# johannes-graeter/limo

Measured on AMD Instinct MI355X. Metric: keyframe-BA window solves/sec (5 KF, ~2k landmarks), higher is better.
Workload: dtype f64; 1 GPU; C2: KITTI-00-shaped windows, 5 keyframes x 2000 landmarks, LiDAR depth + ground plane, solveTrimmed schedule {2, trim 5%, <=100 LM iterations}; batch_windows_per_gpu=16384, distinct_windows_per_gpu=4096, observations_per_batch=144288124, depth_observations_per_batch=68405568, parallelism=single, converged=16328

## Files before the change

include/limo_hip.h:

```cpp
#ifndef LIMO_HIP_H_
#define LIMO_HIP_H_

#include <stddef.h>
#include <stdint.h>

#ifdef __cplusplus
extern "C" {
#endif

#define LIMO_ABI_VERSION 6

enum limo_fixation { LIMO_FIX_POSE = 0, LIMO_FIX_SCALE = 1, LIMO_FIX_NONE = 2 };

enum limo_status {
    LIMO_OK = 0,
    LIMO_ERR_INVALID = -1,
    LIMO_ERR_NOT_ENOUGH_KF = -2,
    LIMO_ERR_RUNTIME = -3,
    LIMO_ERR_NO_DEVICE = -4,
    LIMO_ERR_UNSUPPORTED = -5
};

enum limo_termination { LIMO_CONVERGENCE = 0, LIMO_NO_CONVERGENCE = 1, LIMO_FAILURE = 2 };

// ... 20 lines not shown
    const float* obs_u;
    const float* obs_v;
    const float* obs_d;
} limo_ba_window;

typedef struct limo_ba_options {
    double depth_thres;
    double reprojection_thres;
    double depth_quantile;
    double reprojection_quantile;
    int32_t num_trim_rounds;
    int32_t trim_solver_iterations;
    int32_t min_landmarks_for_trimming;
    int32_t minimum_number_residual_groups;
    int32_t max_num_iterations;
    double max_solver_time_sec;
    double function_tolerance;
    double gradient_tolerance;
    double parameter_tolerance;
    double initial_trust_region_radius;
    double max_trust_region_radius;
    double min_trust_region_radius;
    double min_lm_diagonal;
    double max_lm_diagonal;
    double min_relative_decrease;
    int32_t max_num_consecutive_invalid_steps;
    int32_t jacobi_scaling;
} limo_ba_options;

typedef struct limo_ba_report {
    int32_t termination;
    int32_t num_solves;
    int32_t iterations_total;
    int32_t iterations_final;
    int32_t successful_steps;
    int32_t n_depth_blocks;
    int32_t n_repr_blocks;
    int32_t n_gp_blocks;
    int32_t n_trimmed_landmarks;
    int32_t num_linearizations;
    double initial_cost;
    double final_cost;
    double time_sec;
} limo_ba_report;

typedef struct limo_ctx limo_ctx;
typedef struct limo_ba_batch limo_ba_batch;

int limo_abi_version(void);
int limo_ctx_create(int device, limo_ctx** out);
void limo_ctx_destroy(limo_ctx* ctx);
int limo_ctx_set_stream(limo_ctx* ctx, void* hip_stream);
const char* limo_last_error(const limo_ctx* ctx);
void* limo_host_alloc(size_t bytes);
void limo_host_free(void* p);

void limo_ba_default_options(limo_ba_options* out);

int limo_ba_solve(limo_ctx* ctx, limo_ba_window* window, const limo_ba_options* opts, limo_ba_report* report);

int limo_ba_batch_create(limo_ctx* ctx, int32_t n_windows, const limo_ba_window* windows, limo_ba_batch** out);
int limo_ba_batch_solve(limo_ba_batch* batch, const limo_ba_options* opts);
int limo_ba_batch_reset(limo_ba_batch* batch);
int limo_ba_batch_download(limo_ba_batch* batch, limo_ba_window* windows_out, limo_ba_report* reports);
void limo_ba_batch_destroy(limo_ba_batch* batch);
int limo_ba_batch_trimmed(limo_ba_batch* batch, int32_t window, uint8_t* removed);
int limo_ba_batch_kernel_stats(limo_ba_batch* batch, int reset, double* linearize_ms, int64_t* linearize_launches,
                               double* total_ms);
#define LIMO_KERNEL_LINEARIZE 0
#define LIMO_KERNEL_SCHUR 1
int limo_ba_batch_kernel_time(limo_ba_batch* batch, int kernel, double* ms, int64_t* launches);

#define LIMO_COMM_ID_BYTES 128
int limo_comm_unique_id(unsigned char id[LIMO_COMM_ID_BYTES]);
int limo_ctx_comm_init(limo_ctx* ctx, const unsigned char id[LIMO_COMM_ID_BYTES], int rank, int world);
typedef void (*limo_exchange_fn)(const double* send, double* recv, long long count, int kind, void* user);
int limo_ctx_comm_init_host(limo_ctx* ctx, limo_exchange_fn fn, void* user, int rank, int world);
int limo_ba_solve_sharded(limo_ctx* ctx, limo_ba_window* window, const limo_ba_options* opts, int n_shards,
                          limo_ba_report* report);
int limo_ctx_exchange_stats(limo_ctx* ctx, int64_t* stats3);
int64_t limo_ctx_coop_fallbacks(const limo_ctx* ctx);
int limo_ctx_last_solve_info(const limo_ctx* ctx, int64_t info[8]);
int limo_ctx_last_schur_gp_info(const limo_ctx* ctx, int64_t info[4]);

typedef struct limo_ba_iteration {
    int32_t solve;
    int32_t solve_kind;
    int32_t iteration;
    uint8_t step_is_valid, step_is_successful, pad[2];
    double cost;
    double cost_change, gradient_max_norm, step_norm, relative_decrease, trust_region_radius;
} limo_ba_iteration;
int limo_ctx_set_iteration_log(limo_ctx* ctx, int32_t on);
int limo_ba_batch_iteration_log(limo_ba_batch* batch, int32_t window, int32_t cap, limo_ba_iteration* out, int32_t* n);
int limo_ctx_last_iteration_log(limo_ctx* ctx, int32_t window, int32_t cap, limo_ba_iteration* out, int32_t* n);

int limo_ba_evaluate(limo_ctx* ctx, const limo_ba_window* window, const limo_ba_options* opts, int apply_loss,
                     double* cost, double* residuals, double* jac_pose, double* jac_lm, uint8_t* valid);

int limo_ba_evaluate_batch_time(limo_ctx* ctx, int32_t n_windows, const limo_ba_window* windows, const limo_ba_options* opts,
                                int32_t reps, double* device_ms);

typedef struct limo_speed_prior {
    double speed_weight;
    double dt_cur;
    double vel_prev[3];
    double pose_before[7];
} limo_speed_prior;
int limo_ba_adjust_pose_only(limo_ctx* ctx, limo_ba_window* window, const limo_speed_prior* prior,
                             const limo_ba_options* opts, limo_ba_report* report);

int limo_ba_batch_create_pose_only(limo_ctx* ctx, int32_t n_windows, const limo_ba_window* windows,
                                   const limo_speed_prior* priors, limo_ba_batch** out);
int limo_ba_adjust_pose_only_batch(limo_ctx* ctx, int32_t n_windows, limo_ba_window* windows, const limo_speed_prior* priors,
                                   const limo_ba_options* opts, limo_ba_report* reports);

int limo_ba_solve_fixed_landmarks(limo_ctx* ctx, limo_ba_window* window, const uint8_t* lm_fixed, const limo_ba_options* opts,
                                  limo_ba_report* report);
int limo_ba_batch_create_fixed_landmarks(limo_ctx* ctx, int32_t n_windows, const limo_ba_window* windows, const uint8_t* const* lm_fixed,
                                         limo_ba_batch** out);

enum limo_row_kind {
    LIMO_ROW_GROUND_HEIGHT = 0,
    LIMO_ROW_SCALE = 1,
    LIMO_ROW_NORMAL_DIFF = 2,
    LIMO_ROW_DIST_DIFF = 3,
    LIMO_ROW_PLANE_MOTION = 4,
    LIMO_ROW_GLOBAL_NORMAL = 5,
    LIMO_ROW_SPEED = 6
};
typedef struct limo_ba_row {
    int32_t kind;
    int32_t sub;
    int32_t kf[2];
    int32_t lm;
    int32_t fixed;
    double r;
    double cost;
    double jac_kf[2][10];
    double jac_lm[3];
} limo_ba_row;
int limo_ba_evaluate_rows(limo_ctx* ctx, const limo_ba_window* window, const limo_speed_prior* prior, int pose_only,
                          const limo_ba_options* opts, int32_t cap, limo_ba_row* rows, int32_t* n_rows);

typedef struct limo_ray {
    double pose_cam_origin[7];
    double f, cx, cy;
    float u, v, d;
    float pad;
} limo_ray;
int limo_landmark_init(limo_ctx* ctx, int32_t n, const int32_t* ray_off , const limo_ray* rays,
                       const uint8_t* use_depth , double* pos_out , uint8_t* ok );

int limo_trim_quantile(int32_t n, const int64_t* ids, const double* values, double quantile, int64_t* outliers_out);

typedef struct limo_depth_params {
    int32_t pixelarea_search_width;
    int32_t pixelarea_search_height;
    int32_t pixelarea_search_offset_x;
    int32_t pixelarea_search_offset_y;
    int32_t neighbors_count_min;
    int32_t do_use_histogram_segmentation;
    double histogram_segmentation_bin_width;
    int32_t histogram_segmentation_min_pointcount;
    int32_t treshold_depth_enabled;
    double treshold_depth_max;
// ... 149 lines not shown
```

limo_amd/_ffi.py:

```python
import ctypes as C
import os

_HERE = os.path.dirname(os.path.abspath(__file__))
LIB_PATH = os.environ.get("LIMO_HIP_LIB") or os.path.join(_HERE, "lib", "liblimo_hip.so")

LIMO_FIX_POSE, LIMO_FIX_SCALE, LIMO_FIX_NONE = 0, 1, 2
LIMO_OK, LIMO_ERR_INVALID, LIMO_ERR_NOT_ENOUGH_KF, LIMO_ERR_RUNTIME, LIMO_ERR_NO_DEVICE, LIMO_ERR_UNSUPPORTED = 0, -1, -2, -3, -4, -5
LIMO_CONVERGENCE, LIMO_NO_CONVERGENCE, LIMO_FAILURE = 0, 1, 2

c_double_p = C.POINTER(C.c_double)
c_float_p = C.POINTER(C.c_float)
c_int32_p = C.POINTER(C.c_int32)
c_int64_p = C.POINTER(C.c_int64)
c_uint8_p = C.POINTER(C.c_uint8)


class BaWindow(C.Structure):
    _fields_ = [
        ("n_kf", C.c_int32),
        ("n_cam", C.c_int32),
        ("n_lm", C.c_int32),
        ("n_obs", C.c_int32),
        ("kf_pose", c_double_p),
        ("kf_plane_dir", c_double_p),
# ... 259 lines not shown
        ("do_use_triangle_size_maximation", C.c_int32),
        ("do_check_triangleplanar_condition", C.c_int32),
        ("triangleplanar_crossnorm_treshold", C.c_double),
        ("viewray_plane_orthoganality_treshold", C.c_double),
        ("do_use_ransac_plane", C.c_int32),
        ("ransac_plane_distance_treshold", C.c_double),
        ("ransac_plane_min_z", C.c_double),
        ("ransac_plane_max_z", C.c_double),
        ("ransac_plane_max_iterations", C.c_int32),
        ("ransac_plane_probability", C.c_double),
        ("ransac_plane_use_refinement", C.c_int32),
        ("ransac_plane_refinement_treshold", C.c_double),
        ("ransac_plane_point_distance_treshold", C.c_double),
        ("plane_estimator_use_mestimator", C.c_int32),
        ("ransac_seed", C.c_uint64),
        ("neighbor_search_mode", C.c_int32),
        ("do_use_nearestNeighborSearch", C.c_int32),
        ("nnSearch_count", C.c_int32),
        ("do_use_radiusSearch", C.c_int32),
        ("radiusSearch_radius", C.c_double),
        ("radiusSearch_count_min", C.c_int32),
        ("do_use_depth_segmentation", C.c_int32),
        ("depth_segmentation_max_treshold_gradient", C.c_double),
        ("depth_segmentation_max_neighbor_distance", C.c_double),
        ("depth_segmentation_max_neighbor_distance_gradient", C.c_double),
        ("depth_segmentation_max_seedpoint_to_seedpoint_distance", C.c_double),
        ("depth_segmentation_max_seedpoint_to_seedpoint_distance_gradient", C.c_double),
        ("depth_segmentation_max_neighbor_to_seedpoint_distance", C.c_double),
        ("depth_segmentation_max_neighbor_to_seedpoint_distance_gradient", C.c_double),
        ("depth_segmentation_max_pointcount", C.c_int32),
        ("treshold_depth_mode", C.c_int32),
        ("treshold_depth_local_mode", C.c_int32),
        ("do_use_PCA", C.c_int32),
        ("pca_debug", C.c_double),
        ("pca_treshold_3_abs_min", C.c_double),
        ("pca_treshold_3_2_rel_max", C.c_double),
        ("pca_treshold_2_1_rel_min", C.c_double),
        ("ransac_plane_use_camx_treshold", C.c_int32),
        ("ransac_plane_treshold_camx", C.c_double),
        ("plane_estimator_use_triangle_maximation", C.c_int32),
        ("plane_estimator_use_leastsquares", C.c_int32),
        ("plane_estimator_z_x_min_relation", C.c_double),
        ("do_debug_singleFeatures", C.c_int32),
        ("do_publish_points", C.c_int32),
        ("do_depth_calc_statistics", C.c_int32),
    ]


(DEPTH_OK, DEPTH_NEIGHBOURS, DEPTH_HISTOGRAM, DEPTH_SEGMENT3, DEPTH_PLANAR, DEPTH_PARALLEL, DEPTH_GLOBAL, DEPTH_LOCAL, DEPTH_PCA,
 DEPTH_DEGENERATE) = range(10)
DEPTH_REASON_NAMES = ["OK", "NEIGHBOURS", "HISTOGRAM", "SEGMENT3", "PLANAR", "PARALLEL", "GLOBAL", "LOCAL", "PCA", "DEGENERATE"]


EXCHANGE_FN = C.CFUNCTYPE(None, C.POINTER(C.c_double), C.POINTER(C.c_double), C.c_longlong, C.c_int, C.c_void_p)

ABI_VERSION = 6

ABI_SYMBOLS = [
    "limo_abi_version",
    "limo_ctx_create",
    "limo_ctx_destroy",
    "limo_ctx_set_stream",
    "limo_last_error",
    "limo_host_alloc",
    "limo_host_free",
    "limo_ba_default_options",
    "limo_ba_solve",
    "limo_ba_batch_create",
    "limo_ba_batch_solve",
    "limo_ba_batch_reset",
    "limo_ba_batch_download",
    "limo_ba_batch_destroy",
    "limo_ba_batch_trimmed",
    "limo_ba_batch_kernel_stats",
    "limo_ba_batch_kernel_time",
    "limo_comm_unique_id",
    "limo_ctx_comm_init",
    "limo_ctx_comm_init_host",
    "limo_ba_solve_sharded",
    "limo_ctx_exchange_stats",
    "limo_ctx_coop_fallbacks",
    "limo_ctx_last_solve_info",
    "limo_ctx_last_schur_gp_info",
    "limo_ctx_set_iteration_log",
    "limo_ba_batch_iteration_log",
    "limo_ctx_last_iteration_log",
    "limo_ba_evaluate",
    "limo_ba_evaluate_batch_time",
    "limo_ba_evaluate_rows",
    "limo_ba_adjust_pose_only",
    "limo_ba_batch_create_pose_only",
    "limo_ba_adjust_pose_only_batch",
    "limo_ba_solve_fixed_landmarks",
    "limo_ba_batch_create_fixed_landmarks",
    "limo_landmark_init",
    "limo_trim_quantile",
    "limo_depth_default_params",
    "limo_depth_estimate",
    "limo_depth_estimate_begin",
    "limo_depth_estimate_end",
    "limo_depth_estimate_batch",
    "limo_depth_last_ground_plane",
    "limo_depth_last_reasons",
    "limo_depth_set_timing",
    "limo_depth_last_kernel_ms",
    "limo_five_point_default_params",
    "limo_five_point",
    "limo_five_point_batch",
    "limo_select_default_params",
    "limo_landmark_select",
    "limo_landmark_select_batch",
    "limo_select_set_timing",
    "limo_select_last_kernel_ms",
]

_lib = None


def load():
    global _lib
    if _lib is not None:
        return _lib
    if not os.path.exists(LIB_PATH):
        raise RuntimeError(
            "limo_amd: %s not found - run `python -c 'import __graft_entry__ as g; g.build()'` first. "
            "There is no CPU fallback for the product path." % LIB_PATH
        )
    try:
        import torch
    except ImportError:
        pass
    lib = C.CDLL(LIB_PATH, mode=C.RTLD_GLOBAL)
    vp = C.c_void_p
    lib.limo_abi_version.restype = C.c_int
    older = os.environ.get("LIMO_ALLOW_OLDER_ABI") == "1" and lib.limo_abi_version() < ABI_VERSION
    if lib.limo_abi_version() != ABI_VERSION and not older:
        raise RuntimeError("limo_amd: %s has ABI version %d, this binding needs %d - rebuild it (__graft_entry__.build())" % (LIB_PATH, lib.limo_abi_version(), ABI_VERSION))
    lib.limo_ctx_create.argtypes = [C.c_int, C.POINTER(vp)]
    lib.limo_ctx_destroy.argtypes = [vp]
    lib.limo_ctx_destroy.restype = None
    lib.limo_ctx_set_stream.argtypes = [vp, vp]
    lib.limo_last_error.argtypes = [vp]
    lib.limo_last_error.restype = C.c_char_p
    lib.limo_ba_default_options.argtypes = [C.POINTER(BaOptions)]
    lib.limo_ba_default_options.restype = None
    lib.limo_ba_solve.argtypes = [vp, C.POINTER(BaWindow), C.POINTER(BaOptions), C.POINTER(BaReport)]
    lib.limo_ba_batch_create.argtypes = [vp, C.c_int32, C.POINTER(BaWindow), C.POINTER(vp)]
    lib.limo_ba_batch_solve.argtypes = [vp, C.POINTER(BaOptions)]
    lib.limo_ba_batch_reset.argtypes = [vp]
    lib.limo_ba_batch_download.argtypes = [vp, C.POINTER(BaWindow), C.POINTER(BaReport)]
    lib.limo_ba_batch_destroy.argtypes = [vp]
    lib.limo_ba_batch_destroy.restype = None
    lib.limo_ba_batch_trimmed.argtypes = [vp, C.c_int32, c_uint8_p]
    lib.limo_ba_batch_kernel_stats.argtypes = [vp, C.c_int, c_double_p, c_int64_p, c_double_p]
    lib.limo_ba_batch_kernel_time.argtypes = [vp, C.c_int, c_double_p, c_int64_p]
    lib.limo_comm_unique_id.argtypes = [C.c_char_p]
    lib.limo_ctx_comm_init.argtypes = [vp, C.c_char_p, C.c_int, C.c_int]
    if not older:
        lib.limo_ctx_comm_init_host.argtypes = [vp, EXCHANGE_FN, C.c_void_p, C.c_int, C.c_int]
    lib.limo_ba_solve_sharded.argtypes = [vp, C.POINTER(BaWindow), C.POINTER(BaOptions), C.c_int, C.POINTER(BaReport)]
    lib.limo_ba_evaluate_batch_time.argtypes = [vp, C.c_int32, C.POINTER(BaWindow), C.POINTER(BaOptions), C.c_int32, C.POINTER(C.c_double)]
    lib.limo_ba_evaluate.argtypes = [
        vp,
        C.POINTER(BaWindow),
        C.POINTER(BaOptions),
        C.c_int,
        c_double_p,
        c_double_p,
        c_double_p,
        c_double_p,
        c_uint8_p,
    ]
    lib.limo_ba_evaluate_rows.argtypes = [vp, C.POINTER(BaWindow), C.POINTER(SpeedPrior), C.c_int, C.POINTER(BaOptions), C.c_int32, C.POINTER(BaRow), c_int32_p]
    lib.limo_ba_adjust_pose_only.argtypes = [
        vp,
        C.POINTER(BaWindow),
        C.POINTER(SpeedPrior),
        C.POINTER(BaOptions),
        C.POINTER(BaReport),
    ]
    if hasattr(lib, "limo_ba_batch_create_pose_only"):
        lib.limo_ba_batch_create_pose_only.argtypes = [vp, C.c_int32, C.POINTER(BaWindow), C.POINTER(SpeedPrior), C.POINTER(vp)]
        lib.limo_ba_adjust_pose_only_batch.argtypes = [vp, C.c_int32, C.POINTER(BaWindow), C.POINTER(SpeedPrior), C.POINTER(BaOptions), C.POINTER(BaReport)]
    if hasattr(lib, "limo_ba_solve_fixed_landmarks"):
        lib.limo_ba_solve_fixed_landmarks.argtypes = [vp, C.POINTER(BaWindow), c_uint8_p, C.POINTER(BaOptions), C.POINTER(BaReport)]
        lib.limo_ba_batch_create_fixed_landmarks.argtypes = [vp, C.c_int32, C.POINTER(BaWindow), C.POINTER(c_uint8_p), C.POINTER(vp)]
    lib.limo_landmark_init.argtypes = [vp, C.c_int32, c_int32_p, C.POINTER(Ray), c_uint8_p, c_double_p, c_uint8_p]
    lib.limo_trim_quantile.argtypes = [C.c_int32, c_int64_p, c_double_p, C.c_double, c_int64_p]
    lib.limo_depth_default_params.argtypes = [C.POINTER(DepthParams)]
    lib.limo_depth_default_params.restype = None
    lib.limo_depth_estimate.argtypes = [
        vp,
        c_float_p,
        C.c_size_t,
        c_double_p,
        C.c_double,
        C.c_double,
        C.c_double,
        C.c_int32,
        C.c_int32,
        c_float_p,
        C.c_size_t,
        c_uint8_p,
        C.POINTER(DepthParams),
        c_float_p,
    ]
    lib.limo_depth_estimate_begin.argtypes = lib.limo_depth_estimate.argtypes[:-1]
    lib.limo_depth_estimate_end.argtypes = [vp, c_float_p, C.c_size_t]
    lib.limo_host_alloc.argtypes = [C.c_size_t]
    lib.limo_host_alloc.restype = C.c_void_p
    lib.limo_host_free.argtypes = [C.c_void_p]
    lib.limo_host_free.restype = None
    lib.limo_depth_estimate_batch.argtypes = [vp, C.c_int32, C.POINTER(DepthFrame), c_double_p, C.c_double, C.c_double, C.c_double, C.c_int32, C.c_int32,
                                              C.POINTER(DepthParams), C.c_uint32]
    lib.limo_ctx_exchange_stats.argtypes = [vp, c_int64_p]
    lib.limo_ctx_coop_fallbacks.argtypes = [vp]
    lib.limo_ctx_coop_fallbacks.restype = C.c_int64
    if hasattr(lib, "limo_ctx_last_solve_info"):
        lib.limo_ctx_last_solve_info.argtypes = [vp, c_int64_p]
    if hasattr(lib, "limo_ctx_last_schur_gp_info"):
        lib.limo_ctx_last_schur_gp_info.argtypes = [vp, c_int64_p]
    if hasattr(lib, "limo_ctx_set_iteration_log"):
        lib.limo_ctx_set_iteration_log.argtypes = [vp, C.c_int32]
        lib.limo_ba_batch_iteration_log.argtypes = [vp, C.c_int32, C.c_int32, C.POINTER(BaIteration), c_int32_p]
        lib.limo_ctx_last_iteration_log.argtypes = [vp, C.c_int32, C.c_int32, C.POINTER(BaIteration), c_int32_p]
    lib.limo_depth_set_timing.argtypes = [vp, C.c_int32]
    lib.limo_depth_last_kernel_ms.argtypes = [vp, c_double_p]
    lib.limo_depth_last_ground_plane.argtypes = [vp, C.c_int32, c_double_p, c_int32_p]
    if not older:
        lib.limo_depth_last_reasons.argtypes = [vp, C.c_int32, c_uint8_p, C.c_size_t]
    if hasattr(lib, "limo_five_point"):
        lib.limo_five_point_default_params.argtypes = [C.POINTER(FivePointParams)]
        lib.limo_five_point_default_params.restype = None
        lib.limo_five_point.argtypes = [vp, C.POINTER(FivePointFrame), C.c_double, C.c_double, C.c_double, C.POINTER(FivePointParams),
                                        C.POINTER(FivePointMotion), c_uint8_p]
        lib.limo_five_point_batch.argtypes = [vp, C.c_int32, C.POINTER(FivePointFrame), C.c_double, C.c_double, C.c_double, C.POINTER(FivePointParams),
                                              C.POINTER(FivePointMotion)]
    if hasattr(lib, "limo_landmark_select"):
        lib.limo_select_default_params.argtypes = [C.POINTER(SelectParams)]
        lib.limo_select_default_params.restype = None
        lib.limo_landmark_select.argtypes = [vp, C.POINTER(SelectPool), C.POINTER(SelectParams), c_uint8_p]
        lib.limo_landmark_select_batch.argtypes = [vp, C.c_int32, C.POINTER(SelectPool), C.POINTER(SelectParams), C.POINTER(c_uint8_p)]
        lib.limo_select_set_timing.argtypes = [vp, C.c_int32]
        lib.limo_select_last_kernel_ms.argtypes = [vp, c_double_p]
    _lib = lib
    return lib
```

limo_amd/ba.py:

```python
import ctypes as C

import numpy as np

from . import _ffi
from .window import struct_array


class LimoError(RuntimeError):
    pass


class NotEnoughKeyframes(LimoError):
    """BundleAdjusterKeyframes::NotEnoughKeyframesException (bundle_adjuster_keyframes.hpp:59-68)."""


def _check(rc, ctx=None, what=""):
    if rc == _ffi.LIMO_OK:
        return
    msg = ""
    if ctx is not None:
        msg = _ffi.load().limo_last_error(ctx).decode(errors="replace")
    if rc == _ffi.LIMO_ERR_NOT_ENOUGH_KF:
        raise NotEnoughKeyframes(msg or what)
    raise LimoError("%s failed: rc=%d %s" % (what, rc, msg))


class Context:
    def __init__(self, device=0, stream=None):
        self.lib = _ffi.load()
        self.device = device
        self.ptr = C.c_void_p()
        rc = self.lib.limo_ctx_create(device, C.byref(self.ptr))
        if rc != 0:
            raise LimoError("limo_ctx_create(device=%d) failed rc=%d (no gfx950 device? the product path has no CPU fallback)" % (device, rc))
        if stream is not None:
            self.set_stream(stream)

    def set_stream(self, stream):
        _check(self.lib.limo_ctx_set_stream(self.ptr, C.c_void_p(stream)), self.ptr, "limo_ctx_set_stream")

    def close(self):
        if self.ptr:
            self.lib.limo_ctx_destroy(self.ptr)
            self.ptr = C.c_void_p()

    def __del__(self):
        try:
            self.close()
        except Exception:
            pass

    def solve(self, window, opts, lm_fixed=None):
        s = window.as_struct()
        rep = _ffi.BaReport()
        if lm_fixed is not None:
            flags = fixed_flags(lm_fixed, window.n_lm)
            rc = self.lib.limo_ba_solve_fixed_landmarks(self.ptr, C.byref(s), flags.ctypes.data_as(_ffi.c_uint8_p), C.byref(opts), C.byref(rep))
            _check(rc, self.ptr, "limo_ba_solve_fixed_landmarks")
            return rep.as_dict()
        _check(self.lib.limo_ba_solve(self.ptr, C.byref(s), C.byref(opts), C.byref(rep)), self.ptr, "limo_ba_solve")
        return rep.as_dict()

    def solve_sharded(self, window, opts, n_shards):
        s = window.as_struct()
        rep = _ffi.BaReport()
        _check(self.lib.limo_ba_solve_sharded(self.ptr, C.byref(s), C.byref(opts), int(n_shards), C.byref(rep)), self.ptr, "limo_ba_solve_sharded")
        return rep.as_dict()

    def exchange_stats(self):
        st = (C.c_int64 * 3)()
        _check(self.lib.limo_ctx_exchange_stats(self.ptr, st), self.ptr, "limo_ctx_exchange_stats")
        return {"exchanges": int(st[0]), "bytes": int(st[1]), "iterations": int(st[2])}

    def coop_fallbacks(self):
        return int(self.lib.limo_ctx_coop_fallbacks(self.ptr))

    SOLVE_PATHS = {1: "WG", 2: "COOP", 3: "STREAMING", 4: "LOCKSTEP"}

    def last_solve_info(self):
        v = (C.c_int64 * 8)()
        _check(self.lib.limo_ctx_last_solve_info(self.ptr, v), self.ptr, "limo_ctx_last_solve_info")
        keys = ("recovered", "coop_G", "groups", "slots", "rounds", "pair_launches", "lin_variant")
        return dict({"path": self.SOLVE_PATHS.get(int(v[0]), "NONE")}, **{k: int(v[1 + i]) for i, k in enumerate(keys)})

    def last_schur_gp_info(self):
        v = (C.c_int64 * 4)()
        _check(self.lib.limo_ctx_last_schur_gp_info(self.ptr, v), self.ptr, "limo_ctx_last_schur_gp_info")
        return dict(zip(("narrow_groups", "wide_groups", "narrow_launches", "wide_launches"), (int(x) for x in v)))

    def set_iteration_log(self, on):
        _check(self.lib.limo_ctx_set_iteration_log(self.ptr, int(bool(on))), self.ptr, "limo_ctx_set_iteration_log")

    def last_iteration_log(self, window=0):
        return _read_iteration_log(lambda cap, out, n: self.lib.limo_ctx_last_iteration_log(self.ptr, int(window), cap, out, n), self.ptr,
                                   "limo_ctx_last_iteration_log")

    def comm_init(self, unique_id, rank, world):
        _check(self.lib.limo_ctx_comm_init(self.ptr, unique_id, int(rank), int(world)), self.ptr, "limo_ctx_comm_init")

    def comm_init_host(self, rank, world, allgather, allreduce):
        import numpy as np

        def _cb(send, recv, count, kind, _user):
            s = np.ctypeslib.as_array(send, shape=(count,))
            if kind == 0:
                allgather(s, np.ctypeslib.as_array(recv, shape=(world, count)))
            else:
                allreduce(s, np.ctypeslib.as_array(recv, shape=(count,)))

        self._xfn = _ffi.EXCHANGE_FN(_cb)
        _check(self.lib.limo_ctx_comm_init_host(self.ptr, self._xfn, None, int(rank), int(world)), self.ptr, "limo_ctx_comm_init_host")

    def comm_unique_id(self):
        buf = C.create_string_buffer(128)
        _check(self.lib.limo_comm_unique_id(buf), self.ptr, "limo_comm_unique_id")
        return buf.raw

    def landmark_init(self, ray_off, rays, use_depth):
        ray_off = np.ascontiguousarray(ray_off, np.int32)
        use_depth = np.ascontiguousarray(use_depth, np.uint8)
        n = len(use_depth)
        pos = np.zeros((n, 3))
        ok = np.zeros(n, np.uint8)
        rc = self.lib.limo_landmark_init(self.ptr, n, ray_off.ctypes.data_as(_ffi.c_int32_p), rays, use_depth.ctypes.data_as(_ffi.c_uint8_p),
                                         pos.ctypes.data_as(_ffi.c_double_p), ok.ctypes.data_as(_ffi.c_uint8_p))
        _check(rc, self.ptr, "limo_landmark_init")
        return pos, ok

    def five_point_params(self, probability=None, threshold_px=None, max_samples=None, chunk=None):
        p = _ffi.FivePointParams()
        self.lib.limo_five_point_default_params(C.byref(p))
        for name, v in (("probability", probability), ("threshold_px", threshold_px), ("max_samples", max_samples), ("chunk", chunk)):
            if v is not None:
                setattr(p, name, v)
        return p

    def five_point(self, pts_a, pts_b, focal, cx, cy, seed=1, params=None, with_mask=False):
        a = np.ascontiguousarray(pts_a, np.float64).reshape(-1, 2)
        b = np.ascontiguousarray(pts_b, np.float64).reshape(-1, 2)
        if len(a) != len(b):
            raise ValueError("five_point: %d points in a, %d in b" % (len(a), len(b)))
        fr = _ffi.FivePointFrame(len(a), a.ctypes.data_as(_ffi.c_double_p), b.ctypes.data_as(_ffi.c_double_p), int(seed))
        p = params if params is not None else self.five_point_params()
        m = _ffi.FivePointMotion()
        mask = np.zeros(max(1, len(a)), np.uint8) if with_mask else None
        rc = self.lib.limo_five_point(self.ptr, C.byref(fr), float(focal), float(cx), float(cy), C.byref(p), C.byref(m),
                                      mask.ctypes.data_as(_ffi.c_uint8_p) if with_mask else None)
        _check(rc, self.ptr, "limo_five_point")
        out = m.as_dict()
        out["raw"] = bytes(m)
        if with_mask:
            out["inlier"] = mask[: len(a)]
        return out

    def five_point_batch(self, frames, focal, cx, cy, params=None):
        keep = [(np.ascontiguousarray(a, np.float64).reshape(-1, 2), np.ascontiguousarray(b, np.float64).reshape(-1, 2), int(s)) for a, b, s in frames]
        n = len(keep)
        arr = (_ffi.FivePointFrame * max(1, n))()
        for i, (a, b, s) in enumerate(keep):
            if len(a) != len(b):
                raise ValueError("five_point_batch: frame %d: %d points in a, %d in b" % (i, len(a), len(b)))
            arr[i] = _ffi.FivePointFrame(len(a), a.ctypes.data_as(_ffi.c_double_p), b.ctypes.data_as(_ffi.c_double_p), s)
        p = params if params is not None else self.five_point_params()
        ms = (_ffi.FivePointMotion * max(1, n))()
        _check(self.lib.limo_five_point_batch(self.ptr, n, arr, float(focal), float(cx), float(cy), C.byref(p), ms), self.ptr, "limo_five_point_batch")
        out = []
        for i in range(n):
            d = ms[i].as_dict()
            d["raw"] = bytes(ms[i])
            out.append(d)
        return out
# ... 318 lines not shown
```

limo_amd/csrc/kba_batch_plan.hpp:

```cpp
#pragma once
#include <algorithm>
#include <cstdint>
#include <cstdlib>
#include <vector>

#include "kba_items.hpp"
#include "kba_pack.hpp"

namespace kba {

struct PlanKernelSizes {
    int (*lean_lds)(int ncol);
    int (*wide_lds)(int nfp, int nc, int n_view);
    int lin_lds;
    int wide_waves;
    int trim_max_sort;
};

struct BatchPlan {
    bool any_fast = false, any_gen = false;
    int plain_tm = 1, plain_wpe = 4, gp_tm = 1, gp_wpe = 3;
    bool pair_ok = false;
    int wide_npw = 0;
    int plain_lds = 0, leangp_lds = 0, wide_lds = 0;
// ... 11 lines not shown
        p.max_nc = std::max(p.max_nc, (int)d.nc);
        if (d.schur_fast) {
            p.any_fast = true;
            max_nfq = std::max(max_nfq, (int)d.nfq);
            max_nf = std::max(max_nf, (int)d.nf);
        } else if (d.n_sblk > 0) {
            p.any_gen = true;
            t_gen = std::max(t_gen, d.nf_pad / 16);
            nfp_gen = std::max(nfp_gen, (int)d.nf_pad);
            nc_gen = std::max(nc_gen, (int)d.nc);
            nv_gen = std::max(nv_gen, (int)d.n_view);
        }
    }
    if (p.any_fast) {
        p.plain_tm = (max_nfq + 16) / 16 <= 1 ? 1 : 2;
        p.plain_wpe = p.plain_tm == 1 ? 4 : 3;
        p.plain_lds = ks.lean_lds(max_nfq + 1);
        p.gp_tm = std::min(3, (max_nf + 16) / 16);
        p.gp_wpe = p.gp_tm == 1 ? 3 : 2;
        p.leangp_lds = ks.lean_lds(max_nf + 1);
        p.pair_ok = p.plain_tm == 2 && p.gp_tm == 3;
        p.narrow = p.gp_tm == 3 && P.n_sgrp_narrow > 0;
    }
    if (p.any_gen) {
        const int tiles = t_gen * (t_gen + 1) / 2, npw = (tiles + ks.wide_waves - 1) / ks.wide_waves;
        p.wide_npw = npw <= 1 ? 1 : npw <= 3 ? 3 : npw <= 6 ? 6 : npw <= 12 ? 12 : -1;
        p.wide_lds = ks.wide_lds(nfp_gen, nc_gen, nv_gen);
    }
    {
        int nc_lds = kCamSlots, nf_lds = 1, nv_lds = 1;
        for (const WinDesc& d : P.win)
            if (d.cam_scr_off < 0) {
                nc_lds = std::max(nc_lds, (int)d.nc);
                nf_lds = std::max(nf_lds, (int)d.nf);
                nv_lds = std::max(nv_lds, (int)d.n_view);
            }
        p.asm_bytes = cam_assemble_scratch(nc_lds, kBlock, nv_lds) * (int)sizeof(double);
        p.solve_bytes = cam_solve_scratch(nc_lds, kBlock, nf_lds) * (int)sizeof(double);
    }
    int max_lm = 1, np2 = 1;
    for (const WinDesc& d : P.win) max_lm = std::max(max_lm, (int)d.n_lm);
    while (np2 < max_lm) np2 <<= 1;
    p.trim_bytes = np2 <= ks.trim_max_sort ? np2 * 12 + max_lm + 16 : 16;
    p.schur_wave_lds = (std::max(p.plain_lds, p.leangp_lds) + 15) / 16 * 16;
    p.onelaunch_lds = std::max(std::max(p.asm_bytes, p.solve_bytes), std::max(p.trim_bytes, ks.lin_lds));
    return p;
}

inline void build_sblk_list(const PackedBatch& P, const std::vector<int32_t>* windows, int span, int span_gp, int owner, std::vector<int32_t>& v,
                            int& n_plain, int& n_fgp) {
    v.clear();
    n_plain = n_fgp = 0;
    const int nw = windows ? (int)windows->size() : P.n_win;
    for (int cls = 0; cls < 3; ++cls) {
        for (int q = 0; q < nw; ++q) {
            const int w = windows ? (*windows)[q] : q;
            const WinDesc& d = P.win[w];
            if ((cls < 2) != (d.schur_fast != 0)) continue;
            auto groups = [&](int i0, int i1, int sp) {
                for (int i = i0; i < i1; i += sp)
                    if (owner < 0 || P.sblk_owner[d.sblk0 + i] == owner) v.push_back(d.sblk0 + i);
            };
            if (cls != 1) groups(0, d.n_sblk_plain, span);
            if (cls != 0) groups(d.n_sblk_plain, d.n_sblk, span_gp);
        }
        if (cls == 0) n_plain = (int)v.size();
        if (cls == 1) n_fgp = (int)v.size() - n_plain;
    }
}

constexpr int kCoopMaxWg = 256, kCoopMaxWin = 64;
constexpr int kWgMaxLblk = 8;
constexpr int kCoopRetryAfter = 64;

struct SolveSwitches {
    bool stream_min_set = false;
    int stream_min = 16;
    int coop_max_win = kCoopMaxWin;
    bool no_wg = false;
    bool no_coop = false;
    double coop_timeout_ms = 50.0;
    bool groups_set = false;
    int groups = 0;
    bool gp_wide = false;
};

inline SolveSwitches read_solve_switches() {
    SolveSwitches s;
    auto on = [](const char* name) {
        const char* e = std::getenv(name);
        return e && std::atoi(e) != 0;
    };
    if (const char* e = std::getenv("KBA_STREAM_MIN")) {
        s.stream_min_set = true;
        s.stream_min = std::atoi(e);
    }
    if (const char* e = std::getenv("KBA_COOP_MAX_WIN")) s.coop_max_win = std::min(std::atoi(e), kCoopMaxWg);
    s.no_wg = on("KBA_NO_WG_SOLVE");
    s.no_coop = on("KBA_NO_COOP_SOLVE");
    if (const char* e = std::getenv("KBA_COOP_TIMEOUT_MS")) s.coop_timeout_ms = std::atof(e);
    if (const char* e = std::getenv("KBA_GROUPS")) {
        s.groups_set = true;
        s.groups = std::atoi(e);
    }
    s.gp_wide = on("KBA_SCHUR_GP_WIDE");
    return s;
}

enum SolvePath { PATH_NONE = 0, PATH_WG = 1, PATH_COOP = 2, PATH_STREAMING = 3, PATH_LOCKSTEP = 4 };

struct SolveFacts {
    double max_solver_time_sec = -1.0;
    int shard_P = 1;
    bool pose_batch = false;
    bool pristine = true;
    int coop_strikes = 0, coop_benched = 0;
};
struct CoopGeometry {
    int G = 0, grid = 0;
};
struct SolveChoice {
    SolvePath path = PATH_LOCKSTEP;
    SolvePath fallback = PATH_LOCKSTEP;
    bool benched = false;
    CoopGeometry coop;
};

inline int plain_groups(const WinDesc& d, int span) { return (d.n_sblk_plain + span - 1) / span; }
inline int gp_groups(const WinDesc& d, int span_gp) { return (d.n_sblk - d.n_sblk_plain + span_gp - 1) / span_gp; }

inline bool wg_solve_applies(const PackedBatch& P, const BatchPlan& plan, const SolveSwitches& sw, int shard_P) {
    if (shard_P != 1 || P.evaluate_only || P.n_sblk != 0 || P.n_win < 1 || sw.no_wg) return false;
    for (const WinDesc& d : P.win)
        if (d.n_lblk > kWgMaxLblk) return false;
    return plan.onelaunch_lds <= kCamLdsCapBytes;
}

inline int coop_lds_bytes(const BatchPlan& plan) { return std::max(plan.onelaunch_lds, (kBlock / 64) * plan.schur_wave_lds); }

inline bool coop_solve_applies(const PackedBatch& P, const BatchPlan& plan, const SolveSwitches& sw, int shard_P, CoopGeometry& geo) {
    if (shard_P != 1 || P.evaluate_only || P.n_win < 1 || sw.no_coop) return false;
    int G = 1;
    for (const WinDesc& d : P.win) {
        if (!d.schur_fast || d.cam_scr_off >= 0 || d.nf_pad * d.nf_pad > kCoopRedStride) return false;
        const int tasks = plain_groups(d, kSchurSpan) + gp_groups(d, kSchurSpanGp);
        G = std::max(G, std::max((int)d.n_lblk, tasks ? 1 + (tasks + kBlock / 64 - 1) / (kBlock / 64) : 1));
    }
    G = std::min(G, 32);
    if (P.n_win > kCoopMaxWg || coop_lds_bytes(plan) > kCamLdsCapBytes) return false;
    const int per8 = ((int)P.n_win + 7) / 8;
    geo.G = std::max(1, std::min(G, kCoopMaxWg / (8 * per8)));
    geo.grid = 8 * geo.G * per8;
    return true;
}

inline SolveChoice choose_solve_path(const PackedBatch& P, const BatchPlan& plan, const SolveSwitches& sw, const SolveFacts& f) {
    SolveChoice ch;
    const bool pose_multi = f.pose_batch && P.n_win > 1;
    const bool can_stream = f.shard_P == 1 && f.max_solver_time_sec <= 0.0 && P.n_win >= sw.stream_min && !P.evaluate_only && !pose_multi;
    const bool one_launch = pose_multi || (!(sw.stream_min_set && can_stream) && P.n_win <= sw.coop_max_win);
    ch.path = ch.fallback = can_stream ? PATH_STREAMING : PATH_LOCKSTEP;
    if (!one_launch) return ch;
    if (wg_solve_applies(P, plan, sw, f.shard_P)) {
        ch.path = PATH_WG;
    } else if (!pose_multi && f.pristine && coop_solve_applies(P, plan, sw, f.shard_P, ch.coop)) {
        ch.benched = f.coop_strikes >= 3;
        if (!ch.benched || f.coop_benched + 1 >= kCoopRetryAfter) ch.path = PATH_COOP;
    }
    return ch;
}

struct SchurSpans {
    int plain = kSchurSpan, gp = kSchurSpanGp;
};
struct StreamGeometry {
    int n_slots = 0, n_groups = 0;
    int group_slots[4] = {0, 0, 0, 0};
    int mx[SL_COUNT] = {0};
};
inline StreamGeometry stream_geometry(const PackedBatch& P, const SchurSpans& spans, const SolveSwitches& sw) {
    StreamGeometry g;
    g.n_slots = std::min((int)P.n_win, std::max(1024, std::min(kSchedMaxSlots, (int)P.n_win / 4)));
    g.n_groups = sw.groups_set ? std::max(1, std::min(4, sw.groups)) : g.n_slots >= 4096 ? 3 : P.n_win >= 512 ? 2 : 1;
    for (int gi = 0; gi < g.n_groups; ++gi) g.group_slots[gi] = g.n_slots / g.n_groups + (gi < g.n_slots % g.n_groups ? 1 : 0);
    for (const WinDesc& d : P.win) {
        const int plg = plain_groups(d, spans.plain), gpg = gp_groups(d, spans.gp);
        g.mx[SL_LBLK] = std::max(g.mx[SL_LBLK], (int)d.n_lblk);
        g.mx[SL_TBLK] = std::max(g.mx[SL_TBLK], (int)d.n_blk);
        g.mx[SL_SPLAIN] = std::max(g.mx[SL_SPLAIN], d.schur_fast ? plg : 0);
// ... 11 lines not shown
```

limo_amd/csrc/kba_items.hpp:

```cpp
#pragma once
#include "kba_layout.hpp"
#include "kba_lm.hpp"
#include "kba_math.hpp"

#ifndef KBA_SYNC
#define KBA_SYNC() ((void)0)
#endif
#if defined(KBA_PROFILE_TICKS) && defined(__HIPCC__)
__device__ long long kba_ticks[2][24];
#endif
#if defined(KBA_PROFILE_TICKS) && defined(__HIP_DEVICE_COMPILE__)
#define KBA_TICK(n)                                                                   \
    do {                                                                              \
        if (w == 0 && (tid == 0 || tid == nt - 1)) kba_ticks[tid != 0][n] = clock64(); \
    } while (0)
#else
#define KBA_TICK(n) ((void)0)
#endif

namespace kba {

struct LinLane {
    double e[kLinPartial];
    int fail;
// ... 938 lines not shown
                rel_translation(pose + 7 * (int64_t)(wd.kf0 + k0), pose + 7 * (int64_t)(wd.kf0 + k1), d, Ja, Jb, want_jac);
                const double z = d[0] * d[0] + d[1] * d[1] + d[2] * d[2];
                double dn[3] = {d[0], d[1], d[2]};
                double inv = 1.0;
                if (z > 0.0) {
                    inv = 1.0 / sqrt(z);
                    for (int k = 0; k < 3; ++k) dn[k] *= inv;
                }
                row.r = sw * (n0[0] * dn[0] + n0[1] * dn[1] + n0[2] * dn[2]);
                all_const = !blk_free(k0, 0) && !blk_free(k1, 0) && !blk_free(k0, 6);
                if (want_jac) {
                    double e[3];
                    if (z > 0.0) {
                        const double ndn = n0[0] * dn[0] + n0[1] * dn[1] + n0[2] * dn[2];
                        for (int k = 0; k < 3; ++k) e[k] = (n0[k] - ndn * dn[k]) * inv;
                    } else {
                        for (int k = 0; k < 3; ++k) e[k] = n0[k];
                    }
                    double P0[9];
                    unitvec_plus_jac(n0, P0);
                    for (int k = 0; k < 6; ++k) push(k0, k, sw * (e[0] * Ja[k] + e[1] * Ja[6 + k] + e[2] * Ja[12 + k]));
                    for (int k = 0; k < 6; ++k) push(k1, k, sw * (e[0] * Jb[k] + e[1] * Jb[6 + k] + e[2] * Jb[12 + k]));
                    for (int k = 0; k < 3; ++k)
                        push(k0, 6 + k, sw * (dn[0] * P0[0 + k] + dn[1] * P0[3 + k] + dn[2] * P0[6 + k]));
                }
            }
            return;
        }
        i -= npair * 5;
        if (i < wd.n_kf * 3) {
            const int k = i / 3, sub = i % 3;
            const double sw = sqrt(10.0);
            const double* n = pdir + 3 * (int64_t)(wd.kf0 + k);
            const double tgt[3] = {0.0, 0.0, 1.0};
            row.r = sw * (tgt[sub] - n[sub]);
            all_const = !blk_free(k, 6);
            if (want_jac) {
                double P[9];
                unitvec_plus_jac(n, P);
                for (int kk = 0; kk < 3; ++kk) push(k, 6 + kk, -sw * sel_row3(P, sub, kk));
            }
            return;
        }
        i -= wd.n_kf * 3;
    }
    if (wd.pose_only && wd.speed_w > 0.0 && i < 3) {
        const double sw = sqrt(wd.speed_w);
        const double* p = pose + 7 * (int64_t)wd.kf0;
        double u[3], R[9], Ru[3];
        for (int k = 0; k < 3; ++k)
            u[k] = -(wd.speed_Rb[0 + k] * wd.speed_tb[0] + wd.speed_Rb[3 + k] * wd.speed_tb[1] + wd.speed_Rb[6 + k] * wd.speed_tb[2]);
        quat_R(p, R);
        mat3_vec(R, u, Ru);
        const double Rui = i == 0 ? Ru[0] : (i == 1 ? Ru[1] : Ru[2]);
        row.r = sw * ((Rui + p[4 + i]) / wd.speed_dt - wd.speed_vel[i]);
        all_const = !blk_free(0, 0);
        if (want_jac) {
            double M[9];
            rot_tangent_jac(p, u, M);
            for (int k = 0; k < 3; ++k) push(0, k, sw * sel_row3(M, i, k) / wd.speed_dt);
            for (int k = 0; k < 3; ++k) push(0, 3 + k, sw * ((i == k) ? 1.0 : 0.0) / wd.speed_dt);
        }
        return;
    }
}

KBA_HD double block_grad_inf(int kind, const double* x, const double* g) {
    double out[7], d[6], m = 0.0;
    if (kind == 0) {
        for (int i = 0; i < 6; ++i) d[i] = -g[i];
        pose_plus(x, d, out);
        for (int i = 0; i < 7; ++i) m = fmax(m, fabs(x[i] - out[i]));
    } else if (kind == 1) {
        for (int i = 0; i < 3; ++i) d[i] = -g[i];
        unitvec_plus(x, d, out);
        for (int i = 0; i < 3; ++i) m = fmax(m, fabs(x[i] - out[i]));
    } else {
        m = fabs(g[0]);
    }
    return m;
}

template <int N, int NSUM>
KBA_HD void coop_reduce(double* v, int tid, int nt, double* red) {
#if defined(__HIP_DEVICE_COMPILE__)
    if (nt >= 64 && (nt & 63) == 0) {
        const int wave = tid >> 6, nw = nt >> 6;
        for (int q = 0; q < N; ++q) {
            double x = v[q];
            for (int off = 32; off > 0; off >>= 1) {
                const double o = __shfl_xor(x, off, 64);
                x = q < NSUM ? x + o : fmax(x, o);
            }
            if ((tid & 63) == 0) red[wave * N + q] = x;
        }
        KBA_SYNC();
        for (int q = 0; q < N; ++q) {
            double x = red[q];
            for (int u = 1; u < nw; ++u) x = q < NSUM ? x + red[u * N + q] : fmax(x, red[u * N + q]);
            v[q] = x;
        }
        KBA_SYNC();
        return;
    }
#endif
    for (int q = 0; q < N; ++q) red[q * nt + tid] = v[q];
    KBA_SYNC();
    for (int s = nt >> 1; s > 0; s >>= 1) {
        if (tid < s) {
            for (int q = 0; q < NSUM; ++q) red[q * nt + tid] += red[q * nt + tid + s];
            for (int q = NSUM; q < N; ++q) red[q * nt + tid] = fmax(red[q * nt + tid], red[q * nt + tid + s]);
        }
        KBA_SYNC();
    }
    for (int q = 0; q < N; ++q) v[q] = red[q * nt];
    KBA_SYNC();
}

KBA_HD int coop_red_doubles(int n, int nt) { return n * ((nt >= 64 && (nt & 63) == 0) ? nt >> 6 : nt); }

constexpr int kGpChunk = 128;
constexpr int kRegDense = 2 + 2 * kCamSlots;
KBA_HD int cam_max_reg_rows(int nc) {
    const int nkf = nc / kCamSlots;
    return 1 + (nkf > 0 ? (nkf - 1) * 5 + 3 * nkf : 0) + 3;
}
constexpr int kCamDiag = kCamSlots * (kCamSlots + 1) / 2, kCamOff = kCamSlots * kCamSlots;
KBA_HD int cam_bt_count(int nc) {
    const int nkf = nc / kCamSlots;
    return nkf > 0 ? kCamDiag * nkf + kCamOff * (nkf - 1) : 0;
}
KBA_HD int cam_bt_index(int nc, int a, int b) {
    if (a > b) {
        const int t = a;
        a = b;
        b = t;
    }
    const int ka = a / kCamSlots, kb = b / kCamSlots, ia = a - ka * kCamSlots, ib = b - kb * kCamSlots;
    if (ka == kb) return ka * kCamDiag + ia * kCamSlots - ia * (ia - 1) / 2 + (ib - ia);
    if (kb == ka + 1) return (nc / kCamSlots) * kCamDiag + ka * kCamOff + ia * kCamSlots + ib;
    return -1;
}
KBA_HD int cam_assemble_head(int nc) { return cam_bt_count(nc) + 2 * nc + (nc + 1) / 2; }
KBA_HD int cam_assemble_union(int nc) {
    const int rows = (int)((sizeof(RegRow) * cam_max_reg_rows(nc) + 7) / 8);
    const int gp = kGpChunk * 12;
    return rows > gp ? rows : gp;
}
KBA_HD int cam_assemble_scratch(int nc, int nt, int n_view) {
    const int dense = cam_max_reg_rows(nc) * kRegDense;
    const int red = coop_red_doubles(6, nt);
    const int raw = n_view * kLinPartial;
    const int third = red > dense ? red : dense;
    return cam_assemble_head(nc) + cam_assemble_union(nc) + (raw > third ? raw : third);
}
constexpr int kCamLdsCapBytes = 150 * 1024;
KBA_HD int cam_solve_scratch(int nc, int nt, int nf = -1) {
    if (nf < 0) nf = nc;
    return nf * (nf + 1) + nf + nc + coop_red_doubles(3, nt) + nf * (nf + 1) / 2 + nf;
}

KBA_HD void cam_assemble(const BatchView& bv, const SolveConsts& c, int w, int tid, int nt, double* scratch) {
    const WinDesc& wd = bv.win[w];
    const int nc = wd.nc, nbt = cam_bt_count(nc);
    double* H = scratch;
    double* gc = H + nbt;
    double* sc = gc + nc;
    int* fl = reinterpret_cast<int*>(sc + nc);
    double* gps = scratch + cam_assemble_head(nc);
    RegRow* rows = reinterpret_cast<RegRow*>(gps);
    double* dense = gps + cam_assemble_union(nc);
    double* red = dense;
    const uint8_t* cm = bv.cmask + (int64_t)wd.cam0;
    const bool compute_scale = bv.st[w].compute_scale != 0;
    KBA_TICK(0);
    for (int i = tid; i < nbt; i += nt) H[i] = 0.0;
    for (int i = tid; i < nc; i += nt) gc[i] = 0.0;
    auto gp_stage = [&](int g0) {
        const int ng = (wd.gp0 + wd.n_gp - g0) < kGpChunk ? (wd.gp0 + wd.n_gp - g0) : kGpChunk;
        for (int i = tid; i < ng * 12; i += nt) {
            const int q = i / ng, g = g0 + i % ng;
            double v;
            if (q < 10)
                v = bv.gp_F[q * bv.SG + g];
            else if (q == 10)
                v = bv.gp_r[g];
            else
                v = (double)(bv.gp_kf[g] - wd.kf0);
            gps[(i % ng) * 12 + q] = v;
        }
    };
    if (wd.n_gp > 0 && !bv.gp_red) gp_stage(wd.gp0);
    KBA_SYNC();
    double* raw = dense;
    const bool slots_once = nc <= nt;
    int ci0 = -1;
    double sc0 = 1.0;
    if (slots_once && tid < nc) {
        ci0 = bv.cslot[wd.cam0 + tid];
        if (!compute_scale) sc0 = bv.scale_c[wd.cam0 + tid];
    }
    for (int e = tid; e < wd.n_view * kLinPartial; e += nt) {
        const double* lp = bv.lv_part + wd.lvpart_off + e;
        const int64_t stride = (int64_t)wd.n_view * kLinPartial;
        double acc = 0.0;
        int b = 0;
        for (; b + 4 <= wd.n_lblk; b += 4) {
            const double v0 = lp[b * stride], v1 = lp[(b + 1) * stride], v2 = lp[(b + 2) * stride], v3 = lp[(b + 3) * stride];
            acc += v0;
            acc += v1;
            acc += v2;
            acc += v3;
        }
        for (; b < wd.n_lblk; ++b) acc += lp[b * stride];
        raw[e] = acc;
    }
    if (slots_once) {
        if (tid < nc) {
            if (ci0 >= 0) fl[ci0] = tid;
            if (!compute_scale) sc[tid] = sc0;
        }
    } else {
        for (int i = tid; i < nc; i += nt) {
            const int ci = bv.cslot[wd.cam0 + i];
            if (ci >= 0) fl[ci] = i;
            if (!compute_scale) sc[i] = bv.scale_c[wd.cam0 + i];
        }
    }
    KBA_SYNC();
    for (int e = tid; e < wd.n_kf * 27; e += nt) {
        const int kl = e / 27, q = e % 27;
        double acc = 0.0;
        for (int j = 0; j < wd.n_view; ++j) {
            if (bv.view_kf[wd.view0 + j] - wd.kf0 != kl) continue;
            acc += cam_raw_entry(q, raw + j * kLinPartial, bv.view_cam + 16 * (int64_t)(wd.view0 + j) + 4);
        }
        if (q < 21) {
            int a = 0, rem = q;
            while (rem >= 6 - a) {
                rem -= 6 - a;
                ++a;
            }
            const int bb = a + rem;
            H[cam_bt_index(nc, kl * kCamSlots + a, kl * kCamSlots + bb)] += acc;
        } else {
            gc[kl * kCamSlots + (q - 21)] += acc;
        }
    }
    KBA_SYNC();
    KBA_TICK(1);
    if (bv.gp_red) {
        for (int e = tid; e < wd.n_kf * 110; e += nt) {
            const int kl = e / 110, q = e % 110;
            const int a = q < 100 ? q / 10 : q - 100, bb = q < 100 ? q % 10 : 10;
            if (a > bb) continue;
            const int lo = a, hi = bb;
            const int idx = hi == 10 ? 55 + lo : lo * 10 - lo * (lo - 1) / 2 + (hi - lo);
            double acc = 0.0;
            for (int sh = 0; sh < bv.gp_red_P; ++sh) acc += bv.gp_red[((int64_t)sh * bv.TK + wd.kf0 + kl) * kGpRed + idx];
            if (bb < 10)
                H[cam_bt_index(nc, kl * kCamSlots + a, kl * kCamSlots + bb)] += acc;
            else
                gc[kl * kCamSlots + a] += acc;
        }
        KBA_SYNC();
    }
    for (int g0 = wd.gp0; !bv.gp_red && g0 < wd.gp0 + wd.n_gp; g0 += kGpChunk) {
        const int ng = (wd.gp0 + wd.n_gp - g0) < kGpChunk ? (wd.gp0 + wd.n_gp - g0) : kGpChunk;
        if (g0 != wd.gp0) {
            gp_stage(g0);
            KBA_SYNC();
        }
#if defined(__HIP_DEVICE_COMPILE__)
        if (nt == 256) {
            typedef double v4d_t __attribute__((ext_vector_type(4)));
            const int lane = tid & 63, li = lane & 15, kq = lane >> 4;
            for (int kl = tid >> 6; kl < wd.n_kf; kl += 4) {
                int lo = bv.kf_gp0[wd.kf0 + kl] - g0, hi = lo + bv.kf_ngp[wd.kf0 + kl];
                lo = lo < 0 ? 0 : lo;
                hi = hi > ng ? ng : hi;
                if (hi <= lo) continue;
                v4d_t acc = {0.0, 0.0, 0.0, 0.0};
                for (int g = lo; g < hi; g += 8) {
                    const int r0 = g + kq, r1 = g + 4 + kq;
                    const double z0 = (r0 < hi && li < 11) ? gps[r0 * 12 + li] : 0.0;
                    const double z1 = (r1 < hi && li < 11) ? gps[r1 * 12 + li] : 0.0;
                    acc = __builtin_amdgcn_mfma_f64_16x16x4f64(z0, z0, acc, 0, 0, 0);
                    acc = __builtin_amdgcn_mfma_f64_16x16x4f64(z1, z1, acc, 0, 0, 0);
                }
#pragma unroll
                for (int r = 0; r < 4; ++r) {
                    const int a = kq + 4 * r;
                    if (a < 10 && li < 10) {
                        if (a <= li) H[cam_bt_index(nc, kl * kCamSlots + a, kl * kCamSlots + li)] += acc[r];
                    } else if (a < 10 && li == 10)
                        gc[kl * kCamSlots + a] += acc[r];
                }
            }
        } else
#endif
        for (int e = tid; e < wd.n_kf * 110; e += nt) {
            const int kl = e / 110, q = e % 110;
            const int a = q < 100 ? q / 10 : q - 100, bb = q < 100 ? q % 10 : 10;
            if (a > bb) continue;
            int lo = bv.kf_gp0[wd.kf0 + kl] - g0, hi = lo + bv.kf_ngp[wd.kf0 + kl];
            lo = lo < 0 ? 0 : lo;
            hi = hi > ng ? ng : hi;
            double acc = 0.0;
            for (int g = lo; g < hi; ++g) acc += gps[g * 12 + a] * gps[g * 12 + bb];
            if (bb < 10)
                H[cam_bt_index(nc, kl * kCamSlots + a, kl * kCamSlots + bb)] += acc;
            else
                gc[kl * kCamSlots + a] += acc;
        }
        KBA_SYNC();
    }
    KBA_TICK(2);
    const int nrows = reg_row_count(wd);
    const int reg_base = wd.has_scale_reg ? 1 : 0, reg_npair = wd.has_gp_reg ? wd.n_kf - 1 : 0;
    for (int i0 = tid; i0 < (nt >= 256 ? nt : nrows); i0 += nt) {
        int i = i0;
        if (nt >= 256) {
            const int wv = tid >> 6, ln = tid & 63;
            i = -1;
            if (wv == 0) {
                if (ln < reg_npair) i = reg_base + ln * 5 + 4;
            } else if (wv == 1) {
                if (ln < reg_npair * 3) i = reg_base + (ln / 3) * 5 + ln % 3;
            } else if (wv == 2) {
                if (ln < reg_npair)
                    i = reg_base + ln * 5 + 3;
                else if (ln == 63 && wd.has_scale_reg)
                    i = 0;
            } else if (wv == 3) {
                if (reg_base + reg_npair * 5 + ln < nrows) i = reg_base + reg_npair * 5 + ln;
            }
            if (i < 0) continue;
        }
        int all_const;
        reg_row_eval(wd, bv.cmask, bv.pose, bv.pdir, bv.pdist, i, true, rows[i], all_const);
        if (all_const) rows[i].n = -1;
        const RegRow& row = rows[i];
        double* dd = dense + i * kRegDense;
        int klo = 1 << 20;
        for (int p = 0; p < row.n; ++p) klo = row.col[p] / kCamSlots < klo ? row.col[p] / kCamSlots : klo;
        if (row.n <= 0) klo = -(1 << 20);
        for (int q = 0; q < 2 * kCamSlots; ++q) dd[2 + q] = 0.0;
        for (int p = 0; p < row.n; ++p) dd[2 + row.col[p] - klo * kCamSlots] = row.val[p];
        dd[0] = row.r;
        dd[1] = (double)klo;
    }
    KBA_SYNC();
    KBA_TICK(3);
    for (int e = tid; e < (2 * wd.n_kf - 1) * kCamSlots * kCamSlots; e += nt) {
        const int blk = e / (kCamSlots * kCamSlots), q = e % (kCamSlots * kCamSlots);
        const int ka = blk < wd.n_kf ? blk : blk - wd.n_kf, kb = blk < wd.n_kf ? blk : ka + 1;
        const int a = ka * kCamSlots + q / kCamSlots, b = kb * kCamSlots + q % kCamSlots;
        if (a > b) continue;
        const int at = cam_bt_index(nc, a, b);
        double acc = H[at];
        reg_rows_of_block(wd, ka, kb, [&](int lo, int cnt, int base) {
            const double* da = dense + lo * kRegDense + 2 + a - base * kCamSlots;
            const double* db = dense + lo * kRegDense + 2 + b - base * kCamSlots;
            for (int i = 0; i < cnt; ++i) acc += da[i * kRegDense] * db[i * kRegDense];
        });
        H[at] = acc;
    }
    for (int a = tid; a < nc; a += nt) {
        double acc = gc[a];
        reg_rows_of_block(wd, a / kCamSlots, a / kCamSlots, [&](int lo, int cnt, int base) {
            const double* da = dense + lo * kRegDense + 2 + a - base * kCamSlots;
            const double* dr = dense + lo * kRegDense;
            for (int i = 0; i < cnt; ++i) acc += da[i * kRegDense] * dr[i * kRegDense];
        });
        gc[a] = acc;
    }
    KBA_SYNC();
    KBA_TICK(4);
    for (int i = tid; i < nc; i += nt) {
        const double g = cm[i] ? gc[i] : 0.0;
        gc[i] = g;
        bv.gc[wd.cam0 + i] = g;
        if (compute_scale) {
            const double s = (cm[i] && c.jacobi_scaling) ? 1.0 / (1.0 + sqrt(H[cam_bt_index(nc, i, i)])) : 1.0;
            sc[i] = s;
            bv.scale_c[wd.cam0 + i] = s;
        }
    }
    KBA_SYNC();
    {
        double* Hg = bv.Hcc + wd.hcc_off;
        const int nf = wd.nf, n_need = schur_need_count(nf);
        for (int i = tid; i < n_need; i += nt) {
            int ca, cb;
            schur_need_decode(i, nf, ca, cb);
            const int a = fl[ca];
            double v;
            if (cb < nf) {
                const int b = fl[cb], e = cam_bt_index(nc, a, b);
                v = e >= 0 ? sc[a] * sc[b] * H[e] : 0.0;
            } else {
                v = sc[a] * gc[a];
            }
            Hg[i] = v;
        }
    }
    KBA_TICK(5);
    double cost = 0.0, failf = 0.0, gmax = 0.0, xn2 = 0.0, reg_free = 0.0, reg_fixed = 0.0;
    for (int i = tid; i < wd.n_lblk * wd.n_view; i += nt) cost += bv.lv_part[wd.lvpart_off + (int64_t)i * kLinPartial];
    for (int b = wd.lblk0 + tid; b < wd.lblk0 + wd.n_lblk; b += nt)
        if (bv.lblk_linfail[b] != 0.0) failf = 1.0;
    if (wd.n_lm_const) {
        for (int i = tid; i < wd.n_lblk * wd.n_view_fixed0; i += nt)
            reg_fixed += bv.lv_part[wd.lvpart_off + ((int64_t)(i / wd.n_view_fixed0) * wd.n_view + i % wd.n_view_fixed0) * kLinPartial + kLinFixedCost];
        for (int g = wd.gp0 + tid; g < wd.gp0 + wd.n_gp; g += nt) {
            const double v = bv.gp_cost[g];
            const bool fixed = gp_row_fixed(bv, g);
            cost += fixed ? 0.0 : v;
            reg_fixed += fixed ? v : 0.0;
        }
    } else {
        for (int g = wd.gp0 + tid; g < wd.gp0 + wd.n_gp; g += nt) cost += bv.gp_cost[g];
    }
    for (int i = tid; i < nrows; i += nt) {
        if (rows[i].n < 0)
            reg_fixed += 0.5 * rows[i].r * rows[i].r;
        else
            reg_free += 0.5 * rows[i].r * rows[i].r;
    }
    for (int b = wd.lblk0 + tid; b < wd.lblk0 + wd.n_lblk; b += nt) {
        gmax = fmax(gmax, bv.lblk_part[(int64_t)b * 8 + 0]);
        xn2 += bv.lblk_part[(int64_t)b * 8 + 1];
    }
    for (int k = tid; k < wd.n_kf; k += nt) {
        const int gk = wd.kf0 + k;
        if (cm[k * kCamSlots + 0]) {
            const double* x = bv.pose + 7 * (int64_t)gk;
            gmax = fmax(gmax, block_grad_inf(0, x, gc + k * kCamSlots));
            for (int i = 0; i < 7; ++i) xn2 += x[i] * x[i];
        }
        if (cm[k * kCamSlots + 6]) {
            const double* x = bv.pdir + 3 * (int64_t)gk;
            gmax = fmax(gmax, block_grad_inf(1, x, gc + k * kCamSlots + 6));
            for (int i = 0; i < 3; ++i) xn2 += x[i] * x[i];
        }
        if (cm[k * kCamSlots + 9]) {
            gmax = fmax(gmax, block_grad_inf(2, bv.pdist + gk, gc + k * kCamSlots + 9));
            xn2 += bv.pdist[gk] * bv.pdist[gk];
        }
    }
    {
        double v[6] = {reg_free, reg_fixed, cost, xn2, failf, gmax};
        coop_reduce<6, 4>(v, tid, nt, red);
        reg_free = v[0];
        reg_fixed = v[1];
        cost = v[2] + reg_free;
        xn2 = v[3];
        failf = v[4];
        gmax = v[5];
    }
    if (tid == 0) {
        WinRed& r = bv.red[w];
        r.lin_cost = cost;
        r.lin_fail = failf != 0.0;
        r.gmax = gmax;
        r.xnorm2 = xn2;
        r.no_variable = wd.nf == 0 && wd.n_lm_const > 0 && wd.n_lm_const == wd.n_lm;
        bv.reg_cost[2 * w] = reg_free;
        bv.reg_cost[2 * w + 1] = reg_fixed;
    }
    KBA_TICK(6);
}

KBA_HD void cam_solve(const BatchView& bv, const SolveConsts& c, int w, int tid, int nt, double* scratch, int* flag) {
    const WinDesc& wd = bv.win[w];
    const int nc = wd.nc, nf = wd.nf, nfp = wd.nf_pad, lda = nf + 1;
    double* A = scratch;
    double* y = A + nf * lda;
    double* dl = y + nf;
    double* red = dl + nc;
    double* Hs = red + coop_red_doubles(3, nt);
    const double radius = bv.st[w].radius;
    const double* Hg = bv.Hcc + wd.hcc_off;
    const double* sc = bv.scale_c + wd.cam0;
    const int32_t* cs = bv.cslot + wd.cam0;
    double* yc = bv.yc + wd.cam0;
    double* dc = bv.delta_c + wd.cam0;
    const int slab = c.schur_packed ? schur_need_pad(nf) : nfp * nfp;
    const int nfq = wd.nfq;
    KBA_TICK(8);
    const double* sp = c.schur_nslab > 0 ? bv.S_red + wd.sred_off : bv.S_part + wd.spart_off;
    const int n_need = nf * (nf + 1) / 2 + nf;
    const int n_slab = c.schur_nslab > 0 ? c.schur_nslab : schur_slabs(wd, c.schur_span, c.schur_span_gp);
    const int q_gp = c.schur_nslab > 0 ? 0 : (schur_plain_slabs(wd, c.schur_span) & ~3);
    const bool pk = c.slab_packed && wd.schur_fast && c.schur_nslab == 0;
    const int n_pk = pk ? schur_plain_slabs(wd, c.schur_span) : 0;
    const int64_t stride_pl = pk ? schur_need_pad(nfq) : 0, stride_gp = pk ? schur_need_pad(nf) : slab;
    const int64_t skip_base = pk ? (n_slab > n_pk ? slab_packed_base(n_slab - 1, n_pk, nf, nfq) : 0) : (int64_t)(n_slab - 1) * slab;
    constexpr int kE = 4;
    for (int i0 = tid; i0 < n_need; i0 += kE * nt) {
        double acc[kE][4];
        int off[kE], off_pl[kE];
        int dst[kE], qs[kE];
        for (int e = 0; e < kE; ++e) {
            const int i = i0 + e * nt;
            dst[e] = -1;
            off[e] = 0;
            off_pl[e] = -1;
            qs[e] = n_slab;
            for (int r = 0; r < 4; ++r) acc[e][r] = 0.0;
            if (i >= n_need) continue;
            int ca, cb;
            schur_need_decode(i, nf, ca, cb);
            double s_e = Hg[i];
            Hs[i] = s_e;
            if (ca == cb) s_e += fmin(fmax(s_e, c.min_lm_diagonal), c.max_lm_diagonal) / radius;
            off[e] = (c.schur_packed || pk) ? i : (int)schur_need_offset(ca, cb, nf, nfq, nfp);
            if (pk) off_pl[e] = slab_packed_read(false, ca, cb, nf, nfq);
            dst[e] = ca * lda + cb;
            A[dst[e]] = s_e;
            qs[e] = (ca >= nfq || (cb >= nfq && cb < nf)) ? q_gp : 0;
        }
        int q = 0;
        for (; q + 4 <= n_slab; q += 4)
            for (int e = 0; e < kE; ++e)
                for (int r = 0; r < 4; ++r) {
                    const bool plain = q + r < n_pk;
                    const int64_t base = plain ? (int64_t)(q + r) * stride_pl : n_pk * stride_pl + (int64_t)(q + r - n_pk) * stride_gp;
                    const int o = plain ? off_pl[e] : off[e];
                    const bool on = q >= qs[e] && o >= 0;
                    const double v = sp[on ? base + o : skip_base + off[e]];
                    acc[e][r] += on ? v : 0.0;
                }
        for (; q < n_slab; ++q)
            for (int e = 0; e < kE; ++e) {
                const bool plain = q < n_pk;
                const int64_t base = plain ? (int64_t)q * stride_pl : n_pk * stride_pl + (int64_t)(q - n_pk) * stride_gp;
                const int o = plain ? off_pl[e] : off[e];
                const bool on = q >= qs[e] && o >= 0;
                const double v = sp[on ? base + o : skip_base + off[e]];
                acc[e][0] += on ? v : 0.0;
            }
        for (int e = 0; e < kE; ++e)
            if (dst[e] >= 0) A[dst[e]] = A[dst[e]] - ((acc[e][0] + acc[e][1]) + (acc[e][2] + acc[e][3]));
    }
    KBA_SYNC();
    KBA_TICK(9);
    bool failed = false;
    (void)flag;
    const int tw = nt >= 16 ? 16 : 1, th = nt / tw, tx = tid % tw;
    const int ty = nt == 256 ? ((tid >> 4) & 3) * 4 + (tid >> 6) : tid / tw;
#if defined(__HIP_DEVICE_COMPILE__)
    if (nt == 256) {
        typedef double v4d_t __attribute__((ext_vector_type(4)));
        const int lane = tid & 63, wave = tid >> 6, li = lane & 15, kq = lane >> 4;
        double* invd = y;
        if (tid == 0) *flag = 0;
        KBA_SYNC();
        for (int kb = 0; kb < nf; kb += 4) {
            const int kbe = kb + 4 < nf ? kb + 4 : nf;
            if (wave == 0 && nf < 64) {
                auto bcast = [](double v, int from) {
                    return __hiloint2double(__builtin_amdgcn_readlane(__double2hiint(v), from), __builtin_amdgcn_readlane(__double2loint(v), from));
                };
                double rw[4];
#pragma unroll
                for (int q = 0; q < 4; ++q) rw[q] = (kb + q < kbe && lane <= nf) ? A[(kb + q) * lda + lane] : 0.0;
                bool bad = false;
#pragma unroll
                for (int q = 0; q < 4; ++q) {
                    if (kb + q < kbe && !bad) {
                        const double d = bcast(rw[q], kb + q);
                        if (!(d > 0.0)) {
                            bad = true;
                        } else {
                            const double inv_d = 1.0 / d;
                            if (lane == 0) invd[q] = inv_d;
#pragma unroll
                            for (int pr = q + 1; pr < 4; ++pr) {
                                if (kb + pr < kbe) {
                                    const double aki = bcast(rw[q], kb + pr) * inv_d;
                                    if (lane >= kb + pr) rw[pr] -= aki * rw[q];
                                }
                            }
                        }
                    }
                }
                if (bad && lane == 0) *flag = 1;
#pragma unroll
                for (int q = 1; q < 4; ++q)
                    if (kb + q < kbe && lane >= kb + q && lane <= nf) A[(kb + q) * lda + lane] = rw[q];
            } else if (wave == 0) {
                for (int k = kb; k < kbe; ++k) {
                    const double d = A[k * lda + k];
                    if (!(d > 0.0)) {
                        if (lane == 0) *flag = 1;
                        break;
                    }
                    const double inv_d = 1.0 / d;
                    if (lane == 0) invd[k - kb] = inv_d;
                    for (int i = k + 1; i < kbe; ++i) {
                        const double aki = A[k * lda + i] * inv_d;
                        for (int j = i + lane; j <= nf; j += 64) A[i * lda + j] -= aki * A[k * lda + j];
                    }
                    __builtin_amdgcn_fence(__ATOMIC_RELEASE, "workgroup");
                    __builtin_amdgcn_wave_barrier();
                    __builtin_amdgcn_fence(__ATOMIC_ACQUIRE, "workgroup");
                }
            }
            KBA_SYNC();
            if (*flag) break;
            const int n_tr = nf - kbe;
            if (n_tr > 0) {
                const int Ti = (n_tr + 15) / 16, Tj = (n_tr + 1 + 15) / 16;
                const int kp = kb + kq;
                const bool kin = kp < kbe;
                const double ivd = kin ? invd[kq] : 0.0;
                int t = 0;
                for (int ti = 0; ti < Ti; ++ti)
                    for (int tj = ti; tj < Tj; ++tj, ++t) {
                        if ((t & 3) != wave) continue;
                        const int i_op = kbe + 16 * ti + li, j_op = kbe + 16 * tj + li;
                        const double wv = kin && i_op < nf ? -(A[kp * lda + i_op] * ivd) : 0.0;
                        const double pv = kin && j_op <= nf ? A[kp * lda + j_op] : 0.0;
                        v4d_t cacc;
                        const int jc = kbe + 16 * tj + li;
#pragma unroll
                        for (int r = 0; r < 4; ++r) {
                            const int ic = kbe + 16 * ti + kq + 4 * r;
                            cacc[r] = (ic < nf && jc <= nf && jc >= ic) ? A[ic * lda + jc] : 0.0;
                        }
                        cacc = __builtin_amdgcn_mfma_f64_16x16x4f64(wv, pv, cacc, 0, 0, 0);
#pragma unroll
                        for (int r = 0; r < 4; ++r) {
                            const int ic = kbe + 16 * ti + kq + 4 * r;
                            if (ic < nf && jc <= nf && jc >= ic) A[ic * lda + jc] = cacc[r];
                        }
                    }
            }
            KBA_SYNC();
        }
        failed = *flag != 0;
    } else
#endif
    for (int k = 0; k < nf; ++k) {
        const double d = A[k * lda + k];
        if (!(d > 0.0)) {
            failed = true;
            break;
        }
        const double inv_d = 1.0 / d;
        for (int i = k + 1 + ty; i < nf; i += th) {
            const double aki = A[k * lda + i] * inv_d;
            for (int j = i + tx; j <= nf; j += tw) A[i * lda + j] -= aki * A[k * lda + j];
        }
        KBA_SYNC();
    }
    if (failed) {
        if (tid == 0) {
            WinRed& r = bv.red[w];
            r.chol_fail = 1;
            r.mcc = 0.0;
            r.step2 = 0.0;
            r.cand2 = 0.0;
        }
        for (int a = tid; a < nc; a += nt) dc[a] = 0.0;
        return;
    }
    for (int k = tid; k < nf; k += nt) y[k] = sqrt(A[k * lda + k]);
    KBA_SYNC();
    for (int k = ty; k < nf; k += th) {
        const double dp = y[k];
        for (int j = k + tx; j <= nf; j += tw) A[k * lda + j] = j == k ? dp : A[k * lda + j] / dp;
    }
    KBA_SYNC();
    KBA_TICK(10);
#if defined(__HIP_DEVICE_COMPILE__)
    if (nt >= 64 && nf <= 64) {
        if (tid < 64) {
            const bool mine = tid < nf;
            double yv = mine ? A[tid * lda + nf] : 0.0;
            const double diag = mine ? A[tid * lda + tid] : 1.0;
            for (int i = nf - 1; i >= 0; --i) {
                const double xi = __hiloint2double(__builtin_amdgcn_readlane(__double2hiint(yv), i), __builtin_amdgcn_readlane(__double2loint(yv), i)) /
                                  __hiloint2double(__builtin_amdgcn_readlane(__double2hiint(diag), i), __builtin_amdgcn_readlane(__double2loint(diag), i));
                if (tid < i)
                    yv -= A[tid * lda + i] * xi;
                else if (tid == i)
                    yv = xi;
            }
            if (mine) y[tid] = yv;
        }
    } else
#endif
    {
        for (int i = tid; i < nf; i += nt) y[i] = A[i * lda + nf];
        KBA_SYNC();
        for (int i = nf - 1; i >= 0; --i) {
            const double xi = y[i] / A[i * lda + i];
            for (int j = tid; j < i; j += nt) y[j] -= A[j * lda + i] * xi;
            KBA_SYNC();
            if (tid == 0) y[i] = xi;
        }
    }
    KBA_SYNC();
    KBA_TICK(11);
    for (int a = tid; a < nc; a += nt) {
        const int ca = cs[a];
        const double yv = ca >= 0 ? y[ca] : 0.0;
        yc[a] = yv;
        const double d = ca >= 0 ? -sc[a] * yv : 0.0;
        dc[a] = d;
        dl[a] = d;
    }
    KBA_SYNC();
    double part = 0.0;
    for (int i = tid; i < n_need; i += nt) {
        int ca, cb;
        schur_need_decode(i, nf, ca, cb);
        if (cb < nf)
            part -= (ca == cb ? 0.5 : 1.0) * (Hs[i] * y[ca] * y[cb]);
        else
            part += Hs[i] * y[ca];
    }
    KBA_TICK(14);
    const uint8_t* cm = bv.cmask + (int64_t)wd.cam0;
    double step2 = 0.0, cand2 = 0.0;
    for (int k = tid; k < wd.n_kf; k += nt) {
        const int gk = wd.kf0 + k;
        const double* d = dl + k * kCamSlots;
        const double* x = bv.pose + 7 * (int64_t)gk;
        double* xc = bv.pose_c + 7 * (int64_t)gk;
        double pc[7];
        if (cm[k * kCamSlots + 0]) {
            pose_plus(x, d, pc);
            for (int i = 0; i < 7; ++i) {
                step2 += (x[i] - pc[i]) * (x[i] - pc[i]);
                cand2 += pc[i] * pc[i];
            }
        } else {
            for (int i = 0; i < 7; ++i) pc[i] = x[i];
        }
        for (int i = 0; i < 7; ++i) xc[i] = pc[i];
        const double* n = bv.pdir + 3 * (int64_t)gk;
        double* ncand = bv.pdir_c + 3 * (int64_t)gk;
        if (cm[k * kCamSlots + 6]) {
            unitvec_plus(n, d + 6, ncand);
            for (int i = 0; i < 3; ++i) {
                step2 += (n[i] - ncand[i]) * (n[i] - ncand[i]);
                cand2 += ncand[i] * ncand[i];
            }
        } else {
            for (int i = 0; i < 3; ++i) ncand[i] = n[i];
        }
        if (cm[k * kCamSlots + 9]) {
            bv.pdist_c[gk] = bv.pdist[gk] + d[9];
            step2 += d[9] * d[9];
            cand2 += bv.pdist_c[gk] * bv.pdist_c[gk];
        } else {
            bv.pdist_c[gk] = bv.pdist[gk];
        }
    }
    for (int j = nt - 1 - tid; j < wd.n_view; j += nt) {
        const int view = wd.view0 + j, gk = bv.view_kf[view], k = gk - wd.kf0;
        const double* cam = bv.view_cam + 16 * (int64_t)view;
        const double* x = bv.pose + 7 * (int64_t)gk;
        double pc[7];
        if (cm[k * kCamSlots + 0]) {
            pose_plus(x, dl + k * kCamSlots, pc);
        } else {
            for (int i = 0; i < 7; ++i) pc[i] = x[i];
        }
        double Rk[9];
        quat_R(pc, Rk);
        double* vl = bv.view_lin_c + (int64_t)kViewLin * view;
        mat3_mul(cam + 4, Rk, vl);
        for (int i = 0; i < 3; ++i)
            vl[9 + i] = cam[4 + 3 * i] * pc[4] + cam[4 + 3 * i + 1] * pc[5] + cam[4 + 3 * i + 2] * pc[6] + cam[13 + i];
        vl[25] = cam[0];
        vl[26] = cam[1];
        vl[27] = cam[2];
        {
            const bool fr = cm[k * kCamSlots] != 0;
            const double* dk = dl + k * kCamSlots;
            const double dz[6] = {fr ? dk[0] : 0.0, fr ? dk[1] : 0.0, fr ? dk[2] : 0.0, fr ? dk[3] : 0.0, fr ? dk[4] : 0.0, fr ? dk[5] : 0.0};
            double dR[9];
            quat_dR(x, dz, dR);
            mat3_mul(cam + 4, dR, vl + 28);
            mat3_vec(cam + 4, dz + 3, vl + 37);
        }
    }
    KBA_TICK(12);
    double v3[3] = {part, step2, cand2};
    coop_reduce<3, 3>(v3, tid, nt, red);
    if (tid == 0) {
        WinRed& r = bv.red[w];
        r.chol_fail = 0;
        r.mcc = v3[0];
        r.step2 = v3[1];
        r.cand2 = v3[2];
    }
    KBA_TICK(13);
}


KBA_HD void reduce_step(const BatchView& bv, int w, int tid, int nt, double* red, int n_work = -1) {
    const WinDesc& wd = bv.win[w];
    if (n_work < 0) n_work = nt;
    double mcc = 0.0, s2 = 0.0, c2 = 0.0, lfail = 0.0, cost = 0.0, cfail = 0.0;
    const int t0 = tid < n_work ? tid : (1 << 28);
    for (int b = wd.lblk0 + t0; b < wd.lblk0 + wd.n_lblk; b += n_work) {
        mcc += bv.lblk_part[(int64_t)b * 8 + 2];
        s2 += bv.lblk_part[(int64_t)b * 8 + 3];
        c2 += bv.lblk_part[(int64_t)b * 8 + 4];
        if (bv.lblk_part[(int64_t)b * 8 + 5] != 0.0) lfail = 1.0;
    }
    for (int b = wd.lblk0 + t0; b < wd.lblk0 + wd.n_lblk; b += n_work) {
        cost += bv.lblk_part[(int64_t)b * 8 + 6];
        if (bv.lblk_part[(int64_t)b * 8 + 7] != 0.0) cfail = 1.0;
    }
    {
        int g = wd.gp0 + t0;
        const int g_end = wd.gp0 + wd.n_gp;
        for (; g + 3 * n_work < g_end; g += 4 * n_work) {
            const double v0 = bv.gp_cost_c[g], v1 = bv.gp_cost_c[g + n_work], v2 = bv.gp_cost_c[g + 2 * n_work], v3 = bv.gp_cost_c[g + 3 * n_work];
            cost += v0;
            cost += v1;
            cost += v2;
            cost += v3;
        }
        for (; g < g_end; g += n_work) cost += bv.gp_cost_c[g];
    }
    const int nrows = reg_row_count(wd);
    for (int i = t0; i < nrows; i += n_work) {
        RegRow row;
        int all_const;
        reg_row_eval(wd, bv.cmask, bv.pose_c, bv.pdir_c, bv.pdist_c, i, false, row, all_const);
        if (!all_const) cost += 0.5 * row.r * row.r;
    }
    double v[6] = {mcc, s2, c2, cost, lfail, cfail};
    coop_reduce<6, 4>(v, tid, nt, red);
    mcc = v[0];
    s2 = v[1];
    c2 = v[2];
    cost = v[3];
    lfail = v[4];
    cfail = v[5];
    if (tid == 0) {
        WinRed& r = bv.red[w];
        r.mcc += mcc;
        r.step2 += s2;
        r.cand2 += c2;
        if (lfail != 0.0) r.chol_fail = 1;
        r.cand_cost = cost;
        r.cand_fail = cfail != 0.0;
    }
}

KBA_HD void shard_reduce_lin(const BatchView& bv, int w, int shard, int tid, int nt) {
    const WinDesc& wd = bv.win[w];
    const int n_e = wd.n_view * kLinPartial;
    for (int e = tid; e < n_e; e += nt) {
        double acc = 0.0;
        for (int b = 0; b < wd.n_lblk; ++b)
            if (bv.lblk_owner[wd.lblk0 + b] == shard) acc += bv.lv_part[wd.lvpart_off + (int64_t)b * n_e + e];
        bv.x_lv[wd.xlv_off + e] = acc;
    }
    for (int e = tid; e < wd.n_kf * kGpRed; e += nt) {
        const int kl = e / kGpRed, idx = e % kGpRed;
        int a, bb;
        if (idx >= 55) {
            a = idx - 55;
            bb = 10;
        } else {
            a = 0;
            int rem = idx;
            while (rem >= 10 - a) {
// ... 123 lines not shown
```

limo_amd/csrc/kba_kernels.hip:

```cpp
#include <hip/hip_runtime.h>

#include <type_traits>

#define KBA_SYNC() __syncthreads()
#include "kba_items.hpp"

namespace kba {

__device__ __forceinline__ double wave_sum(double v) {
#pragma unroll
    for (int off = 32; off > 0; off >>= 1) v += __shfl_down(v, off, 64);
    return v;
}
__device__ __forceinline__ double wave_max(double v) {
#pragma unroll
    for (int off = 32; off > 0; off >>= 1) v = fmax(v, __shfl_down(v, off, 64));
    return v;
}

template <int N>
__device__ __forceinline__ void block_sum(const double* vals, double* lds , double* out_global) {
    const int lane = threadIdx.x & 63, wave = threadIdx.x >> 6;
#pragma unroll
    for (int i = 0; i < N; ++i) {
// ... 987 lines not shown
#pragma unroll
                for (int r = 0; r < 4; ++r) {
                    const int row = tr * 16 + kq + 4 * r, col = tc * 16 + li;
                    out[row * nfp + col] = St[row * 32 + col];
                }
            }
        return;
    }
    if constexpr (kTT) {
#pragma unroll
        for (int r = 0; r < 4; ++r) {
            const int row = kq + 4 * r, col = li;
            if (packed) {
                const int k = slab_packed_write(false, row, col, g.nf, nfq);
                if (k >= 0) out[k] = acc[0][r];
            } else {
                out[row * nfp + col] = (row < ncol && col < ncol) ? acc[0][r] : 0.0;
            }
        }
    } else {
        int idx = 0;
#pragma unroll
        for (int tr = 0; tr < TM; ++tr)
#pragma unroll
            for (int tc = tr; tc < TM; ++tc) {
                if (tc < T) {
#pragma unroll
                    for (int r = 0; r < 4; ++r) {
                        const int row = tr * 16 + kq + 4 * r, col = tc * 16 + li;
                        if (packed) {
                            const int k = slab_packed_write(GP, row, col, g.nf, nfq);
                            if (k >= 0) out[k] = acc[idx][r];
                        } else {
                            out[row * nfp + col] = (row < ncol && col < ncol) ? acc[idx][r] : 0.0;
                        }
                    }
                }
                ++idx;
            }
        if constexpr (GP) {
            if (!packed)
                for (int tc = TM; tc < T; ++tc)
                    for (int tr = 0; tr <= tc; ++tr) {
#pragma unroll
                        for (int r = 0; r < 4; ++r) out[(tr * 16 + kq + 4 * r) * nfp + tc * 16 + li] = 0.0;
                    }
        }
    }
}
template <int TM, bool GP, int WAVES>
__global__ __launch_bounds__(64) __attribute__((amdgpu_waves_per_eu(WAVES, WAVES))) void k_schur_lean(
    BatchView bv, const int32_t* wl, int span, int span_gp, int slab_packed) {
    const int sb = wl_at(bv, wl, blockIdx.x);
    if (sb < 0) return;
    extern __shared__ __attribute__((aligned(16))) double smem[];
    schur_lean_group<TM, GP, false>(bv, sb, span, span_gp, slab_packed, smem);
}
__global__ __launch_bounds__(64) __attribute__((amdgpu_waves_per_eu(2, 2))) void k_schur_lean_gp(BatchView bv, const int32_t* wl) {
    const int sb = wl_at(bv, wl, blockIdx.x);
    if (sb < 0) return;
    extern __shared__ __attribute__((aligned(16))) double smem[];
    if (bv.sgrp[sb].gp_class != kSchurGpWide)
        schur_lean_group<2, true, false, true>(bv, sb, kSchurSpan, kSchurSpanGp, 1, smem);
    else
        schur_lean_group<3, true, false>(bv, sb, kSchurSpan, kSchurSpanGp, 1, smem);
}

template <int TMP, int TMG, bool NARROW = false>
__global__ __launch_bounds__(64) void k_schur_lean_pair(BatchView bv, const int32_t* wl_plain, int n_plain_cap, const int32_t* wl_gp, int span, int span_gp, int slab_packed) {
    extern __shared__ __attribute__((aligned(16))) double smem[];
    if ((int)blockIdx.x < n_plain_cap) {
        const int sb = wl_at(bv, wl_plain, blockIdx.x);
        if (sb >= 0) schur_lean_group<TMP, false, false>(bv, sb, span, span_gp, slab_packed, smem);
    } else {
        const int sb = wl_at(bv, wl_gp, blockIdx.x - n_plain_cap);
        if (sb < 0) return;
        if (NARROW && bv.sgrp[sb].gp_class != kSchurGpWide)
            schur_lean_group<2, true, false, true>(bv, sb, span, span_gp, slab_packed, smem);
        else
            schur_lean_group<TMG, true, false>(bv, sb, span, span_gp, slab_packed, smem);
    }
}

__global__ __launch_bounds__(kBlock) __attribute__((amdgpu_waves_per_eu(3, 3))) void k_cam_assemble(BatchView bv, SolveConsts c, const int32_t* wl) {
    const int w = wl_at(bv, wl, blockIdx.x);
    if (w < 0) return;
    WinState& st = bv.st[w];
    extern __shared__ __attribute__((aligned(16))) double smem[];
    if (st.active && st.need_lin) {
        const int64_t so = bv.win[w].cam_scr_off;
        if (so >= 0)
            cam_assemble(bv, c, w, threadIdx.x, blockDim.x, bv.cam_scratch + so);
        else
            cam_assemble(bv, c, w, threadIdx.x, blockDim.x, smem);
        __syncthreads();
#ifdef KBA_PROFILE_TICKS
        if (w == 0 && threadIdx.x == 0)
            for (int l = 0; l < 2; ++l)
                printf("[ticks cam_assemble %s lane] observation blocks %lld, ground-plane rows %lld, regulariser rows %lld, their sums %lld, scale + hand-over %lld, reductions %lld\n",
                       l ? "last" : "first", kba_ticks[l][1] - kba_ticks[l][0], kba_ticks[l][2] - kba_ticks[l][1], kba_ticks[l][3] - kba_ticks[l][2],
                       kba_ticks[l][4] - kba_ticks[l][3], kba_ticks[l][5] - kba_ticks[l][4], kba_ticks[l][6] - kba_ticks[l][5]);
#endif
        if (threadIdx.x == 0) lm_decide_lin(st, bv.red[w], bv.reg_cost[2 * w + 1], c);
    }
    __syncthreads();
    if (threadIdx.x == 0 && !bv.counted) {
        if (st.active) atomicAdd(bv.n_active, 1);
        __threadfence();
        if (atomicAdd(bv.n_active + 1, 1) == (int)gridDim.x - 1) {
            __threadfence();
            const int total = atomicAdd(bv.n_active, 0);
            bv.n_active[0] = 0;
            bv.n_active[1] = 0;
            *(volatile int32_t*)bv.n_active_host = total;
            __threadfence_system();
        }
    }
}

__global__ __launch_bounds__(kBlock) void k_cam_solve(BatchView bv, SolveConsts c, const int32_t* wl) {
    const int w = wl_at(bv, wl, blockIdx.x);
    if (w < 0) return;
    if (!bv.st[w].active) return;
    extern __shared__ __attribute__((aligned(16))) double smem[];
    __shared__ int flag;
    const int64_t so = bv.win[w].cam_scr_off;
    if (so >= 0)
        cam_solve(bv, c, w, threadIdx.x, blockDim.x, bv.cam_scratch + so, &flag);
    else
        cam_solve(bv, c, w, threadIdx.x, blockDim.x, smem, &flag);
#ifdef KBA_PROFILE_TICKS
    __syncthreads();
    if (w == 0 && threadIdx.x == 0)
        for (int l = 0; l < 2; ++l)
            printf("[ticks cam_solve %s lane] slab sum %lld, cholesky %lld, back-substitution %lld, step %lld, reduction %lld\n", l ? "last" : "first",
                   kba_ticks[l][9] - kba_ticks[l][8], kba_ticks[l][10] - kba_ticks[l][9], kba_ticks[l][11] - kba_ticks[l][10],
                   kba_ticks[l][12] - kba_ticks[l][11], kba_ticks[l][13] - kba_ticks[l][12]);
#endif
}

__global__ __launch_bounds__(64) void k_step_decide(BatchView bv, SolveConsts c, const int32_t* wl) {
    const int w = wl_at(bv, wl, blockIdx.x);
    if (w < 0) return;
    if (!bv.st[w].active) return;
    __shared__ double red[64];
    reduce_step(bv, w, threadIdx.x, blockDim.x, red);
    __syncthreads();
    if (threadIdx.x == 0) lm_decide_step(bv.st[w], bv.red[w], c);
    __syncthreads();
    if (bv.st[w].accept) accept_keyframes(bv, bv.win[w], threadIdx.x, blockDim.x);
}

__global__ __launch_bounds__(kBlock) void k_after_step(BatchView bv, SolveConsts c, const int32_t* wl) {
    const int b = wl_at(bv, wl, blockIdx.x);
    if (b < 0) return;
    lm_damp_block(bv, c, b);
}

__global__ __launch_bounds__(kBlock) void k_trim_residual(BatchView bv, double* plane_rep, double* plane_dep, const int32_t* wl) {
    const int b = wl_at(bv, wl, blockIdx.x);
    if (b < 0) return;
    const int w = bv.view_win[bv.blk_view[b]];
    if (!bv.win[w].do_trim) return;
    for (int q = 0; q < kObsPerLane; ++q) trim_residual_lane(bv, b, threadIdx.x + q * kBlock, plane_rep, plane_dep);
}

__global__ void k_trim_max(BatchView bv, const double* plane_rep, const double* plane_dep, int shard, int n_shards) {
    int gl;
    if (bv.counted) {
        const int32_t* wl = bv.sched_lists + bv.sched_off[SL_TLBLK] + 1;
        if ((int)blockIdx.x >= wl[-1]) return;
        const int b = wl[blockIdx.x];
        if ((int)threadIdx.x >= bv.lblk_n[b]) return;
        gl = bv.lblk_lm0[b] + threadIdx.x;
    } else {
        gl = blockIdx.x * blockDim.x + threadIdx.x;
    }
    if (gl >= bv.TL) return;
    if (n_shards > 1 && bv.lm_id[gl] % n_shards != shard) return;
    if (!bv.win[bv.lm_win[gl]].do_trim) return;
    trim_max_lane(bv, gl, plane_rep, plane_dep);
}

constexpr int kTrimMaxSort = 8192;

__device__ __forceinline__ bool trim_less(double ka, int ia, double kb, int ib) {
    return ka < kb || (ka == kb && ia < ib);
}

__device__ __forceinline__ void trim_select_win(const BatchView& bv, const SolveConsts& c, int w) {
    const WinDesc& wd = bv.win[w];
    if (!wd.do_trim) return;
    const int n = wd.n_lm;
    extern __shared__ __attribute__((aligned(16))) double smem[];
    __shared__ int n_valid;
    int np2 = 1;
    while (np2 < n) np2 <<= 1;
    int removed = 0;
    if (np2 <= kTrimMaxSort) {
        unsigned long long* keys = reinterpret_cast<unsigned long long*>(smem);
        unsigned* ids = reinterpret_cast<unsigned*>(smem + np2);
        unsigned char* flags = reinterpret_cast<unsigned char*>(ids + np2);
        __shared__ int hist[256];
        __shared__ int s_bin, s_k, s_cnt;
        __shared__ unsigned long long s_thr_hi;
        __shared__ unsigned s_thr_lo;
        for (int i = threadIdx.x; i < n; i += kBlock) flags[i] = 0;
        for (int list = 0; list < 2; ++list) {
            const double* vals = (list == 0 ? bv.trim_dep : bv.trim_rep) + wd.lm0;
            const int32_t* lid = bv.lm_id + wd.lm0;
            const double q = list == 0 ? c.depth_quantile : c.reprojection_quantile;
            if (threadIdx.x == 0) n_valid = 0;
            __syncthreads();
// ... 634 lines not shown
```

limo_amd/csrc/kba_layout.hpp:

```cpp
#pragma once
#include <stddef.h>
#include <stdint.h>

#include "../../include/limo_hip.h"

namespace kba {

constexpr int kMaxKf = 20;
constexpr int kMaxViews = 64;
constexpr int kViewLin = 64;
constexpr int kCamSlots = 10;
constexpr int kMaxNc = kMaxKf * kCamSlots;
constexpr int kBlock = 256;
constexpr int kObsPerLane = 4;
constexpr int kObsBlock = kBlock * kObsPerLane;
constexpr int kSchurLm = 16;
constexpr int kSchurLmPerBlock = 64;
constexpr int kSchurSpan = 2, kSchurSpanGp = 1;
constexpr int kMaxRegRows = 1 + (kMaxKf - 1) * 5 + 3 * kMaxKf;

constexpr int kGpRed = 65;
constexpr int kLinPartial = 28;
constexpr int kLinFixedCost = 26;
constexpr int kLinWaves = 4;

struct EvalChunk {
    int32_t base, view, o0, o1, dep0, pad;
};

struct WinDesc {
    int32_t kf0, n_kf;
    int32_t lm0, n_lm;
    int32_t view0, n_view;
    int32_t obs0, n_obs;
    int32_t blk0, n_blk;
    int32_t lblk0, n_lblk;
    int32_t gp0, n_gp;
    int32_t sblk0, n_sblk;
    int32_t n_sblk_plain;
    int32_t schur_fast, n_fk;
    int32_t fk[4];
    int32_t fk_view[4];
    int32_t nc, nc_pad;
    int32_t nf, nf_pad;
    int32_t nfq;
    int32_t lm_gp0;
    int32_t cam0;
    int32_t reg0;
    int32_t has_scale_reg, has_gp_reg;
    int32_t n_depth, n_repr;
    int32_t do_trim;
    int32_t pose_only;
    int32_t n_view_fixed0;
    int32_t n_lm_const;
    double scale_w, scale_s0;
    double speed_w, speed_dt, speed_vel[3], speed_Rb[9], speed_tb[3];
    int64_t hcc_off;
    int64_t spart_off;
    int64_t sred_off;
    int64_t xlv_off;
    int64_t lvpart_off;
    int64_t cam_scr_off;
};

struct alignas(128) SchurGroup {
    int32_t w;
    int32_t lm_first, n_lm;
    int32_t n_fk;
    int32_t nf, nfq, nf_pad;
    int32_t kf0, view0, cam0;
    int32_t q_slab;
    int32_t gp_class;
    int32_t kl[4];
    int32_t view[4];
    int32_t col0[4];
    int64_t off_tile;
    int64_t off_packed;
    int32_t gp_ci0, gp_ns;
    int32_t pad2[2];
};
static_assert(sizeof(SchurGroup) == 128, "one cache line per record");
constexpr int kSchurGpNoPlane = -1, kSchurGpWide = -2;

struct WinState {
    int32_t active, need_lin, first, accept;
    int32_t iter, max_iter, term, invalid_run;
    int32_t in_phase;
    int32_t compute_scale;
    int32_t n_success, n_unsuccess;
    int32_t acc_solves, acc_iters, acc_success, last_iters;
    int32_t n_trimmed, acc_lin;
    int32_t phase, trim_round;
    int32_t redamp;
    int32_t log_kind;
    double radius, decrease_factor;
    double x_cost, x_norm, fixed_cost;
// ... 160 lines not shown
```

limo_amd/csrc/kba_pack.cpp:

```cpp
#include "kba_pack.hpp"

#include <algorithm>
#include <atomic>
#include <chrono>
#include <cmath>
#include <cstdio>
#include <cstdlib>
#include <cstring>
#include <condition_variable>
#include <functional>
#include <limits>
#include <mutex>
#include <numeric>
#include <thread>
#include <pthread.h>
#include <unistd.h>
#include <exception>

#include "kba_items.hpp"

namespace kba {

namespace {
thread_local PackArena* t_pack_arena = nullptr;
// ... 618 lines not shown
            }
        d.n_lblk = (int)L.lblk_win.size() - d.lblk0;
        d.sblk0 = (int)L.sblk_win.size();
        d.n_sblk_plain = 0;
        if (!po.pose_only && !po.evaluate_only && d.nf > 0) {
            const int per = kSchurLmPerBlock;
            const int n_plain = n_var - n_gp_var;
            std::vector<int> cuts;
            for (int v : seg)
                if (v < n_var) cuts.push_back(v);
            cuts.push_back(n_plain);
            cuts.push_back(n_var);
            std::sort(cuts.begin(), cuts.end());
            cuts.erase(std::unique(cuts.begin(), cuts.end()), cuts.end());
            for (size_t si = 0; si + 1 < cuts.size(); ++si)
                for (int l0 = cuts[si]; l0 < cuts[si + 1]; l0 += per) {
                    L.sblk_win.push_back(w);
                    L.sblk_lm0.push_back(d.lm0 + l0);
                    L.sblk_n.push_back(std::min(per, cuts[si + 1] - l0));
                    L.sblk_owner.push_back(P.lm_id[d.lm0 + l0] % NS);
                    if (l0 < n_plain) d.n_sblk_plain++;
                }
        }
        d.n_sblk = (int)L.sblk_win.size() - d.sblk0;
        d.schur_fast = 1;
        d.n_fk = 0;
        for (int q = 0; q < 4; ++q) d.fk[q] = d.fk_view[q] = -1;
        for (int k = 0; k < W.n_kf; ++k) {
            int nv = 0, view = -1;
            for (int v = 0; v < d.n_view; ++v)
                if (views[w][v].kf == k) {
                    ++nv;
                    view = d.view0 + v;
                }
            if (nv > 1) d.schur_fast = 0;
            if (freem[k * kCamSlots] || freem[k * kCamSlots + 6]) {
                if (d.n_fk < 4) {
                    d.fk[d.n_fk] = k;
                    d.fk_view[d.n_fk] = view;
                }
                d.n_fk++;
            }
        }
        if (d.n_fk > 4) d.schur_fast = 0;
        d.n_view_fixed0 = 0;
        while (d.n_view_fixed0 < d.n_view && !freem[views[w][d.n_view_fixed0].kf * kCamSlots]) d.n_view_fixed0++;
        if (po.evaluate_only) d.n_view_fixed0 = 0;
        };
    for_windows(pack_one);
    const auto t_p2 = std::chrono::steady_clock::now();
    struct Base {
        int blk, lblk, sblk, gp;
    };
    std::vector<Base> base(n);
    {
        Base run{0, 0, 0, 0};
        for (int w = 0; w < n; ++w) {
            Local& L = locals[w];
            if (L.rc != LIMO_OK) {
                err = po.per_window_prior ? "window " + std::to_string(w) + ": " + L.err : L.err;
                return L.rc;
            }
            base[w] = run;
            run.blk += (int)L.blk_view.size();
            run.lblk += (int)L.lblk_win.size();
            run.sblk += (int)L.sblk_win.size();
            run.gp += (int)L.gp_lm.size();
            WinDesc& d = P.win[w];
            d.blk0 += base[w].blk;
            d.lblk0 += base[w].lblk;
            d.sblk0 += base[w].sblk;
            d.gp0 += base[w].gp;
            d.hcc_off = P.hcc_total;
            P.hcc_total += (int64_t)d.nc * d.nc;
            d.spart_off = P.spart_total;
            P.spart_total += (int64_t)d.n_sblk * ((int64_t)d.nf_pad * d.nf_pad);
            d.sred_off = P.sred_total;
            if (P.n_shards > 1) P.sred_total += (int64_t)P.n_shards * schur_need_pad(d.nf);
            d.xlv_off = P.xlv_total;
            P.xlv_total += (int64_t)d.n_view * kLinPartial;
            d.lvpart_off = P.lvpart_total;
            P.lvpart_total += (int64_t)d.n_lblk * d.n_view * kLinPartial;
            {
                const int need = std::max(cam_assemble_scratch(d.nc, kBlock, d.n_view), cam_solve_scratch(d.nc, kBlock));
                d.cam_scr_off = -1;
                if (need * (int)sizeof(double) > kCamLdsCapBytes) {
                    d.cam_scr_off = P.camscr_total;
                    P.camscr_total += need;
                }
            }
        }
        for (auto* v : {&P.blk_view, &P.blk_obs0, &P.blk_n, &P.blk_owner}) v->resize(run.blk);
        for (auto* v : {&P.lblk_win, &P.lblk_lm0, &P.lblk_n, &P.lblk_owner}) v->resize(run.lblk);
        for (auto* v : {&P.sblk_win, &P.sblk_lm0, &P.sblk_n, &P.sblk_owner}) v->resize(run.sblk);
        for (auto* v : {&P.gp_lm, &P.gp_kf, &P.gp_owner}) v->resize(run.gp);
        P.gp_w.resize(run.gp);
    }
    for_windows([&](int w) {
        Local& L = locals[w];
        const WinDesc& d = P.win[w];
        const Base& bs = base[w];
        for (int k = d.kf0; k < d.kf0 + d.n_kf; ++k) {
            if (P.kf_nblk[k]) P.kf_blk0[k] += bs.blk;
            if (P.kf_ngp[k]) P.kf_gp0[k] += bs.gp;
        }
        for (int l = d.lm0; l < d.lm0 + d.n_lm; ++l)
            if (P.lm_gp[l] >= 0) P.lm_gp[l] += bs.gp;
        auto put = [](auto& dst, const auto& src, int at) { std::copy(src.begin(), src.end(), dst.begin() + at); };
        put(P.blk_view, L.blk_view, bs.blk);
        put(P.blk_obs0, L.blk_obs0, bs.blk);
        put(P.blk_n, L.blk_n, bs.blk);
        put(P.blk_owner, L.blk_owner, bs.blk);
        put(P.lblk_win, L.lblk_win, bs.lblk);
        put(P.lblk_lm0, L.lblk_lm0, bs.lblk);
        put(P.lblk_n, L.lblk_n, bs.lblk);
        put(P.lblk_owner, L.lblk_owner, bs.lblk);
        put(P.sblk_win, L.sblk_win, bs.sblk);
        put(P.sblk_lm0, L.sblk_lm0, bs.sblk);
        put(P.sblk_n, L.sblk_n, bs.sblk);
        put(P.sblk_owner, L.sblk_owner, bs.sblk);
        put(P.gp_lm, L.gp_lm, bs.gp);
        put(P.gp_kf, L.gp_kf, bs.gp);
        put(P.gp_w, L.gp_w, bs.gp);
        put(P.gp_owner, L.gp_owner, bs.gp);
        L = Local();
    });
    if (std::getenv("KBA_PACK_TRACE"))
        std::fprintf(stderr, "[kba] pack: views + sizes %.1f ms, arrays %.1f ms, fill %.1f ms, merge %.1f ms\n", std::chrono::duration<double, std::milli>(t_p0b - t_p0).count(),
                     std::chrono::duration<double, std::milli>(t_p1 - t_p0b).count(), std::chrono::duration<double, std::milli>(t_p2 - t_p1).count(),
                     std::chrono::duration<double, std::milli>(std::chrono::steady_clock::now() - t_p2).count());
    P.TG = (int)P.gp_lm.size();
    P.SG = pad64(std::max(1, P.TG));
    P.n_blk = (int)P.blk_view.size();
    P.n_lblk = (int)P.lblk_win.size();
    P.n_sblk = (int)P.sblk_win.size();
    P.sgrp.assign((size_t)P.n_sblk, SchurGroup{});
    const bool classify = schur_gp_panels(P.win) >= 3;
    for_windows([&](int w) {
        const WinDesc& d = P.win[w];
        if (!d.schur_fast) return;
        for (int sb = d.sblk0; sb < d.sblk0 + d.n_sblk; ++sb)
            P.sgrp[sb] = schur_group_make(d, w, sb, kSchurSpan, kSchurSpanGp, P.sblk_lm0.data(), P.sblk_n.data(), P.cslot.data(),
                                          classify ? P.lm_gp.data() : nullptr, classify ? P.gp_kf.data() : nullptr);
    });
    P.n_sgrp_narrow = P.n_sgrp_wide = 0;
    if (classify)
        for (const WinDesc& d : P.win) {
            if (!d.schur_fast) continue;
            for (int i = d.n_sblk_plain; i < d.n_sblk; i += kSchurSpanGp) (P.sgrp[d.sblk0 + i].gp_class == kSchurGpWide ? P.n_sgrp_wide : P.n_sgrp_narrow)++;
        }
    if (P.evaluate_only) {
        P.echunk.clear();
        P.obs_rank.assign((size_t)std::max(1, P.TO), -1);
        std::vector<int32_t> before((size_t)P.TO + 1, 0);
        for (int o = 0; o < P.TO; ++o) {
            const bool dep = P.obs_d[o] > 0.0f;
            if (dep) P.obs_rank[o] = before[o];
            before[o + 1] = before[o] + (dep ? 1 : 0);
        }
        P.TD = before[P.TO];
        P.SD = pad64(std::max(1, P.TD)) + 64;
        for (int b = 0; b < P.n_blk; ++b) {
            const int o0 = P.blk_obs0[b], o1 = o0 + P.blk_n[b];
            for (int a = o0; a < o1; a += 64) {
                EvalChunk ch;
                ch.base = a;
                ch.view = P.blk_view[b];
// ... 38 lines not shown
```

limo_amd/csrc/limo_ctx.hpp:

```cpp
#pragma once
#include <hip/hip_runtime.h>

#include <algorithm>
#include <cstdlib>
#include <map>
#include <string>
#include <vector>

#include "kba_pack.hpp"

struct PinnedBuf {
    void* p = nullptr;
    size_t cap = 0;
    hipError_t ensure(size_t bytes, size_t min_bytes = 0, size_t max_bytes = ~size_t(0)) {
        if (cap >= bytes) return hipSuccess;
        release();
        const size_t want = std::min(max_bytes, std::max(bytes, min_bytes));
        const hipError_t e = hipHostMalloc(&p, want);
        if (e == hipSuccess)
            cap = want;
        else
            p = nullptr;
        return e;
    }
    void release() {
        if (p) (void)hipHostFree(p);
        p = nullptr;
        cap = 0;
    }
};

struct limo_ctx {
    int device = 0;
    hipStream_t stream = nullptr;
    hipStream_t own = nullptr;
    std::string err;
    void* depth_ws = nullptr;
    void (*depth_ws_free)(void*) = nullptr;
    void* comm = nullptr;
    int comm_rank = 0, comm_world = 1;
    void (*xfn)(const double* send, double* recv, long long count, int kind, void* user) = nullptr;
    void* xuser = nullptr;
    PinnedBuf xhost;
    bool has_transport() const { return comm != nullptr || xfn != nullptr; }
    long long exchange_stats[3] = {0, 0, 0};
    long long coop_fallbacks = 0;
    int coop_strikes = 0;
    int coop_benched = 0;
    long long last_solve_info[8] = {0, 0, 0, 0, 0, 0, 0, 0};
    long long last_schur_gp_info[4] = {0, 0, 0, 0};
    bool iteration_log = false;
    std::vector<limo_ba_iteration> last_log;
    std::vector<int32_t> last_log_n;
    std::vector<size_t> last_log_off;
    bool select_timing = false;
    double select_last_ms = 0.;
    static constexpr int kPoolPerClass = 4;
    static constexpr size_t kPoolMaxBlock = 32u << 20;
    std::map<size_t, std::vector<void*>> pool, host_pool;
    PinnedBuf staging;
    PinnedBuf pack_arena;
    size_t pack_arena_wanted = 0;
    bool pack_arena_busy = false;
    static constexpr size_t kPackArenaMax = size_t(1) << 30;
    PinnedBuf staging_big;
    static constexpr size_t kBigStageMax = 512u << 20;

    static constexpr size_t kLargeStep = 64u << 20;
    static constexpr size_t kPoolLargeBytes = size_t(16) << 30;
    size_t pooled_large = 0;
    static size_t size_class(size_t bytes) {
        if (bytes > kPoolMaxBlock) return (bytes + kLargeStep - 1) / kLargeStep * kLargeStep;
        size_t c = 256;
        while (c < bytes) c <<= 1;
        return c;
    }
    hipError_t pool_alloc(void** p, size_t bytes) {
        const size_t c = size_class(bytes);
        static const bool no_reuse = std::getenv("KBA_NO_POOL") != nullptr;
        if (no_reuse) return hipMalloc(p, c);
        auto it = pool.find(c);
        if (it != pool.end() && !it->second.empty()) {
            *p = it->second.back();
            it->second.pop_back();
            if (bytes > kPoolMaxBlock) pooled_large -= c;
            return hipSuccess;
        }
        hipError_t e = hipMalloc(p, c);
        while (e == hipErrorOutOfMemory && trim_largest()) {
            (void)hipGetLastError();
            e = hipMalloc(p, c);
        }
        return e;
    }
    bool trim_largest() {
        for (auto it = pool.rbegin(); it != pool.rend(); ++it) {
            if (it->second.empty()) continue;
            (void)hipFree(it->second.back());
            it->second.pop_back();
            if (it->first > kPoolMaxBlock) pooled_large -= it->first;
            return true;
        }
        return false;
    }
    void pool_free(void* p, size_t bytes) {
        const size_t c = size_class(bytes);
        auto& v = pool[c];
        static const bool no_reuse = std::getenv("KBA_NO_POOL") != nullptr;
        const bool large = bytes > kPoolMaxBlock;
        if (!no_reuse && (large ? (v.empty() && pooled_large + c <= kPoolLargeBytes) : (int)v.size() < kPoolPerClass)) {
            v.push_back(p);
            if (large) pooled_large += c;
        } else {
            (void)hipFree(p);
        }
    }
    hipError_t host_alloc(void** p, size_t bytes) {
        const size_t c = size_class(bytes);
        auto it = host_pool.find(c);
        if (it != host_pool.end() && !it->second.empty()) {
            *p = it->second.back();
            it->second.pop_back();
            return hipSuccess;
        }
        return hipHostMalloc(p, c);
    }
    void host_free(void* p, size_t bytes) {
        auto& v = host_pool[size_class(bytes)];
        if ((int)v.size() < kPoolPerClass && bytes <= kPoolMaxBlock)
            v.push_back(p);
        else
            (void)hipHostFree(p);
    }
// ... 16 lines not shown
```

limo_amd/csrc/limo_hip.hip:

```cpp
#include <hip/hip_runtime.h>
#include <rccl/rccl.h>

#include <algorithm>
#include <chrono>
#include <cmath>
#include <cstdio>
#include <cstring>
#include <atomic>
#include <memory>
#include <new>
#include <string>
#include <thread>
#include <vector>

#include "kba_kernels.hip"

#include "kba_batch_plan.hpp"
#include "kba_buffers.hpp"
#include "kba_rows.hpp"

using namespace kba;

#include "limo_ctx.hpp"

// ... 1 lines not shown
    do {                                                                                         \
        hipError_t e__ = (expr);                                                                 \
        if (e__ != hipSuccess) {                                                                 \
            (ctx)->err = std::string(#expr) + ": " + hipGetErrorString(e__);                     \
            return LIMO_ERR_RUNTIME;                                                             \
        }                                                                                        \
    } while (0)

namespace {

inline int cdiv(int64_t a, int64_t b) {
    return (int)((a + b - 1) / b);
}

struct EventPair {
    hipEvent_t a, b;
    int kernel;
};

}

struct limo_ba_batch : Executor {
    limo_ctx* ctx = nullptr;
    PackedBatch P;
    bool holds_pack_arena = false;
    bool pose_batch = false;
    BatchView bv;
    SolveConsts c;
    limo_ba_options opts;
    std::vector<std::pair<void*, size_t>> allocs;
    double *d_plane_rep = nullptr, *d_plane_dep = nullptr;
    double *d_pose0 = nullptr, *d_pdir0 = nullptr, *d_pdist0 = nullptr, *d_lm0 = nullptr;
    uint8_t* d_lm_state0 = nullptr;
    std::vector<WinState> st0;
    int32_t* h_active = nullptr;
    int32_t* d_h_active = nullptr;
    size_t h_flags_bytes = 0;
    hipEvent_t act_ev[4] = {nullptr, nullptr, nullptr, nullptr};
    int it_no = 0;
    struct WorkLists {
        const int32_t *blk = nullptr, *lblk = nullptr, *sblk = nullptr, *win = nullptr;
        int n_blk = 0, n_lblk = 0, n_sblk_plain = 0, n_sblk_fgp = 0, n_sblk = 0, n_win = 0;
    };
    struct ViewLists {
        WorkLists full, cur;
        int owner = -1;
    };
    std::vector<ViewLists> wl;
    int32_t *d_act_blk = nullptr, *d_act_lblk = nullptr, *d_act_sblk = nullptr, *d_act_win = nullptr;
    int32_t* d_flags = nullptr;
    BatchPlan plan;
    const void *schur_fn_plain = nullptr, *schur_fn_leangp = nullptr, *schur_fn_gen = nullptr;
    const void* schur_fn_narrow = nullptr;
    bool gp_wide = false;
    bool schur_pair_ok = false;
    static constexpr int kSchurPairBound = 384;
    int32_t* h_flags = nullptr;
    int rc = LIMO_OK;
    int n_slots = 0;
    int32_t* d_sched_ctl = nullptr;
    int shard_P = 1, shard_rank = 0;
    bool shard_virtual = true;
    std::vector<int> local_shards;
    std::vector<BatchView> pv;
    ExchangeLayout xl;
    double* arena_c = nullptr;
    std::vector<double*> blocks;
    std::vector<double*> trims;
    double* d_gather = nullptr;
    WinDesc* d_win_orig = nullptr;
    bool first_lin = false, assemble_pending = false;
    int64_t n_exchanges = 0, exchange_bytes = 0;
    double* d_lm_tmp = nullptr;
    std::vector<EventPair> ev_pool;
    size_t ev_used = 0;
    double k_ms_acc[2] = {0.0, 0.0};
    int64_t k_launches[2] = {0, 0};
    hipEvent_t ev_total_a = nullptr, ev_total_b = nullptr;
    double total_ms_acc = 0.0;
    double last_solve_sec = 0.0;
    int64_t n_rounds = 0, n_pair_launches = 0;
    int64_t n_narrow_launches = 0, n_widegp_launches = 0;
    int lin_variant = 1;

    ~limo_ba_batch() override {
        if (holds_pack_arena) ctx->pack_arena_busy = false;
        for (auto& a : allocs) ctx->pool_free(a.first, a.second);
        if (h_active) ctx->host_free(h_active, 64);
        if (h_flags) ctx->host_free(h_flags, h_flags_bytes);
        stream_teardown();
        for (auto& e : ev_pool) {
            (void)hipEventDestroy(e.a);
            (void)hipEventDestroy(e.b);
        }
        for (auto& e : act_ev)
            if (e) (void)hipEventDestroy(e);
        if (ev_total_a) (void)hipEventDestroy(ev_total_a);
        if (ev_total_b) (void)hipEventDestroy(ev_total_b);
    }

    int dmalloc(void** p, size_t bytes) {
        bytes = bytes ? bytes : 8;
        HIP_TRY(ctx, ctx->pool_alloc(p, bytes));
        allocs.push_back({*p, bytes});
        static const bool poison = std::getenv("KBA_POISON") != nullptr;
        if (poison) {
            HIP_TRY(ctx, hipMemsetAsync(*p, 0xFF, bytes, ctx->stream));
            HIP_TRY(ctx, hipStreamSynchronize(ctx->stream));
        }
        return LIMO_OK;
    }

    static const void* schur_kernel(int cls, int a, int b) {
        switch (cls * 100 + a * 10 + b) {
            case 14: return (const void*)k_schur_lean<1, false, 4>;
            case 23: return (const void*)k_schur_lean<2, false, 3>;
            case 113: return (const void*)k_schur_lean<1, true, 3>;
            case 122: return (const void*)k_schur_lean<2, true, 2>;
            case 132: return (const void*)k_schur_lean<3, true, 2>;
            case 210: return (const void*)k_schur_wide<1>;
            case 230: return (const void*)k_schur_wide<3>;
            case 260: return (const void*)k_schur_wide<6>;
            case 320: return (const void*)k_schur_wide<12>;
        }
        return nullptr;
    }

    int upload_list(const std::vector<int32_t>& v, const int32_t** out) {
        int32_t* d = nullptr;
        if (dmalloc((void**)&d, sizeof(int32_t) * std::max<size_t>(1, v.size()))) return LIMO_ERR_RUNTIME;
        if (!v.empty()) HIP_TRY(ctx, hipMemcpy(d, v.data(), sizeof(int32_t) * v.size(), hipMemcpyHostToDevice));
        *out = d;
        return LIMO_OK;
    }
    int build_full_sblk(size_t i) {
        WorkLists& f = wl[i].full;
        std::vector<int32_t> v;
        build_sblk_list(P, nullptr, c.schur_span, c.schur_span_gp, wl[i].owner, v, f.n_sblk_plain, f.n_sblk_fgp);
        f.n_sblk = (int)v.size();
        return upload_list(v, &f.sblk);
    }

    int upload() {
        std::memset(&bv, 0, sizeof(bv));
        int status = LIMO_OK;
        struct Ent {
            void** slot;
            size_t bytes, off;
            const void* init;
        };
        std::vector<Ent> ents;
        for_each_buffer(P, bv, [&](void** slot, size_t bytes, const void* init) { ents.push_back({slot, bytes ? bytes : 8, 0, init}); });
        st0.assign(P.n_win, WinState());
        std::memset(st0.data(), 0, sizeof(WinState) * st0.size());
        for (auto& q : st0) q.term = -1;
        for (Ent& e : ents)
            if (e.slot == (void**)&bv.st) e.init = st0.data();
        ents.push_back({(void**)&d_pose0, sizeof(double) * 7 * std::max(1, P.TK), 0, P.pose.empty() ? nullptr : P.pose.data()});
        ents.push_back({(void**)&d_pdir0, sizeof(double) * 3 * std::max(1, P.TK), 0, P.pdir.empty() ? nullptr : P.pdir.data()});
        ents.push_back({(void**)&d_pdist0, sizeof(double) * std::max(1, P.TK), 0, P.pdist.empty() ? nullptr : P.pdist.data()});
        ents.push_back({(void**)&d_lm0, sizeof(double) * 3 * std::max(1, P.TL), 0, P.lm.empty() ? nullptr : P.lm.data()});
        ents.push_back({(void**)&d_lm_state0, (size_t)std::max(1, P.TL), 0, P.lm_state.empty() ? nullptr : P.lm_state.data()});
        auto align = [](size_t x) { return (x + 255) / 256 * 256; };
        size_t init_total = 0, zero_total = 0;
        for (Ent& e : ents)
            if (e.init) {
// ... 38 lines not shown
        pv.assign(1, bv);
        if (shard_P > 1) {
            xl = exchange_layout(P);
            d_win_orig = const_cast<WinDesc*>(bv.win);
            pv.assign(local_shards.size(), bv);
            auto zeros = [&](double** out, size_t n) -> int {
                if (dmalloc((void**)out, sizeof(double) * std::max<size_t>(1, n))) return LIMO_ERR_RUNTIME;
                HIP_TRY(ctx, hipMemsetAsync(*out, 0, sizeof(double) * std::max<size_t>(1, n), ctx->stream));
                return LIMO_OK;
            };
            if (zeros(&arena_c, xl.c_total)) return LIMO_ERR_RUNTIME;
            trims.assign(1 + local_shards.size(), nullptr);
            for (double*& t : trims)
                if (zeros(&t, xl.trim_count)) return LIMO_ERR_RUNTIME;
            blocks.assign(local_shards.size(), nullptr);
            if (!shard_virtual && zeros(&d_gather, (size_t)ctx->comm_world * xl.b_total)) return LIMO_ERR_RUNTIME;
            {
                std::vector<WinDesc> wc = exchange_consumer_windows(P);
                WinDesc* d_wc = nullptr;
                if (dmalloc((void**)&d_wc, sizeof(WinDesc) * wc.size())) return LIMO_ERR_RUNTIME;
                HIP_TRY(ctx, hipMemcpy(d_wc, wc.data(), sizeof(WinDesc) * wc.size(), hipMemcpyHostToDevice));
                exchange_bind_consumer(xl, bv, arena_c, trims[0], d_wc);
            }
            for (size_t i = 0; i < local_shards.size(); ++i) {
                if (zeros(&blocks[i], xl.b_total)) return LIMO_ERR_RUNTIME;
                exchange_bind_producer(xl, pv[i], blocks[i], trims[1 + i]);
                if (zeros(&pv[i].S_part, xl.spart_count)) return LIMO_ERR_RUNTIME;
            }
            if (!shard_virtual && dmalloc((void**)&d_lm_tmp, sizeof(double) * 3 * std::max(1, P.TL))) return LIMO_ERR_RUNTIME;
        }
        if (dmalloc((void**)&d_plane_rep, sizeof(double) * P.SO)) return LIMO_ERR_RUNTIME;
        if (dmalloc((void**)&d_plane_dep, sizeof(double) * P.SO)) return LIMO_ERR_RUNTIME;
        HIP_TRY(ctx, ctx->host_alloc((void**)&h_active, 64));
        HIP_TRY(ctx, hipHostGetDevicePointer((void**)&d_h_active, h_active, 0));
        bv.n_active_host = nullptr;
        h_flags_bytes = sizeof(int32_t) * std::max(1, P.n_win);
        HIP_TRY(ctx, ctx->host_alloc((void**)&h_flags, h_flags_bytes));
        if (dmalloc((void**)&d_act_blk, sizeof(int32_t) * std::max(1, P.n_blk))) return LIMO_ERR_RUNTIME;
        if (dmalloc((void**)&d_act_lblk, sizeof(int32_t) * std::max(1, P.n_lblk))) return LIMO_ERR_RUNTIME;
        if (dmalloc((void**)&d_act_sblk, sizeof(int32_t) * std::max(1, P.n_sblk))) return LIMO_ERR_RUNTIME;
        if (dmalloc((void**)&d_act_win, sizeof(int32_t) * std::max(1, P.n_win))) return LIMO_ERR_RUNTIME;
        if (dmalloc((void**)&d_flags, sizeof(int32_t) * std::max(1, P.n_win))) return LIMO_ERR_RUNTIME;
        wl.assign(pv.size(), ViewLists());
        for (size_t i = 0; i < wl.size(); ++i) {
            WorkLists& f = wl[i].full;
            f.n_blk = P.n_blk;
            f.n_lblk = P.n_lblk;
            f.n_win = P.n_win;
            if (shard_P == 1) continue;
            const int r = wl[i].owner = local_shards[i];
            auto owned = [&](const std::vector<int32_t>& owner, const int32_t** list, int* n) -> int {
                std::vector<int32_t> v;
                for (size_t k = 0; k < owner.size(); ++k)
                    if (owner[k] == r) v.push_back((int32_t)k);
                *n = (int)v.size();
                return upload_list(v, list);
            };
            if (owned(P.blk_owner, &f.blk, &f.n_blk) || owned(P.lblk_owner, &f.lblk, &f.n_lblk) || build_full_sblk(i)) return LIMO_ERR_RUNTIME;
        }
        plan = plan_batch(P, {schur_lean_lds_bytes, schur_wide_lds_bytes, lin_lm_lds_bytes(P.Vmax, true), kWideWaves, kTrimMaxSort});
        if (plan.wide_npw < 0) {
            ctx->err = "window with too many free camera slots for k_schur_wide";
            return LIMO_ERR_INVALID;
        }
        if (plan.any_fast) {
            schur_fn_plain = schur_kernel(0, plan.plain_tm, plan.plain_wpe);
            HIP_TRY(ctx, hipFuncSetAttribute(schur_fn_plain, hipFuncAttributeMaxDynamicSharedMemorySize, plan.plain_lds));
            schur_fn_leangp = schur_kernel(1, plan.gp_tm, plan.gp_wpe);
            HIP_TRY(ctx, hipFuncSetAttribute(schur_fn_leangp, hipFuncAttributeMaxDynamicSharedMemorySize, plan.leangp_lds));
            schur_pair_ok = plan.pair_ok && !(std::getenv("KBA_NO_SCHUR_PAIR") && std::atoi(std::getenv("KBA_NO_SCHUR_PAIR")) != 0);
            if (schur_pair_ok)
                HIP_TRY(ctx, hipFuncSetAttribute((const void*)k_schur_lean_pair<2, 3>, hipFuncAttributeMaxDynamicSharedMemorySize, std::max(plan.plain_lds, plan.leangp_lds)));
            if (plan.narrow) {
                schur_fn_narrow = (const void*)k_schur_lean_gp;
                HIP_TRY(ctx, hipFuncSetAttribute(schur_fn_narrow, hipFuncAttributeMaxDynamicSharedMemorySize, plan.leangp_lds));
                if (schur_pair_ok)
                    HIP_TRY(ctx, hipFuncSetAttribute((const void*)k_schur_lean_pair<2, 3, true>, hipFuncAttributeMaxDynamicSharedMemorySize, std::max(plan.plain_lds, plan.leangp_lds)));
            }
        }
        if (plan.any_gen) {
            schur_fn_gen = schur_kernel(2, plan.wide_npw, 0);
            HIP_TRY(ctx, hipFuncSetAttribute(schur_fn_gen, hipFuncAttributeMaxDynamicSharedMemorySize, plan.wide_lds));
        }
        HIP_TRY(ctx, hipFuncSetAttribute((const void*)k_cam_assemble, hipFuncAttributeMaxDynamicSharedMemorySize, plan.asm_bytes));
        HIP_TRY(ctx, hipFuncSetAttribute((const void*)k_cam_solve, hipFuncAttributeMaxDynamicSharedMemorySize, plan.solve_bytes));
        HIP_TRY(ctx, hipFuncSetAttribute((const void*)k_trim_select, hipFuncAttributeMaxDynamicSharedMemorySize, plan.trim_bytes));
        for (auto& e : act_ev) HIP_TRY(ctx, hipEventCreateWithFlags(&e, hipEventDisableTiming));
        HIP_TRY(ctx, hipEventCreate(&ev_total_a));
        HIP_TRY(ctx, hipEventCreate(&ev_total_b));
        return LIMO_OK;
    }

    bool spart_has_packed = false;
    bool pristine = true;
    int reset_state() {
        pristine = true;
        HIP_TRY(ctx, hipMemcpyAsync(bv.st, st0.data(), sizeof(WinState) * st0.size(), hipMemcpyHostToDevice, ctx->stream));
        HIP_TRY(ctx, hipMemcpyAsync(bv.pose, d_pose0, sizeof(double) * 7 * P.TK, hipMemcpyDeviceToDevice, ctx->stream));
        HIP_TRY(ctx, hipMemcpyAsync(bv.pdir, d_pdir0, sizeof(double) * 3 * P.TK, hipMemcpyDeviceToDevice, ctx->stream));
        HIP_TRY(ctx, hipMemcpyAsync(bv.pdist, d_pdist0, sizeof(double) * P.TK, hipMemcpyDeviceToDevice, ctx->stream));
        HIP_TRY(ctx, hipMemcpyAsync(bv.lm, d_lm0, sizeof(double) * 3 * P.TL, hipMemcpyDeviceToDevice, ctx->stream));
        HIP_TRY(ctx, hipMemcpyAsync(bv.lm_state, d_lm_state0, P.TL, hipMemcpyDeviceToDevice, ctx->stream));
        return LIMO_OK;
    }

    limo_ba_iteration* d_log = nullptr;
    int log_cap = 0;
    int log_alloc = 0;
    static int log_bound(const limo_ba_options& o) {
        const int64_t t = std::max(0, o.trim_solver_iterations), r = std::max(0, o.num_trim_rounds), m = std::max(0, o.max_num_iterations);
        return (int)std::min<int64_t>(r * ((t + 1) + (3 * t + 1)) + (m + 1), 1 << 24);
    }
    int bind_log(bool on) {
        const int cap = on ? log_bound(opts) : 0;
        if (!on && !log_cap) return LIMO_OK;
        if (cap > log_alloc) {
            if (dmalloc((void**)&d_log, sizeof(limo_ba_iteration) * (size_t)cap * (size_t)std::max(1, P.n_win))) return LIMO_ERR_RUNTIME;
            log_alloc = cap;
        }
        if (cap != log_cap) {
            HIP_TRY(ctx, hipStreamSynchronize(ctx->stream));
            for (int w = 0; w < P.n_win; ++w) {
                st0[w].log = on ? d_log + (size_t)w * cap : nullptr;
                st0[w].log_cap = cap;
            }
            log_cap = cap;
        }
        hipLaunchKernelGGL(k_log_bind, dim3(cdiv(P.n_win, 256)), dim3(256), 0, ctx->stream, bv, on ? d_log : (limo_ba_iteration*)nullptr, cap);
        HIP_TRY(ctx, hipGetLastError());
        return LIMO_OK;
    }
    int read_log(int w, int cap, limo_ba_iteration* out, int32_t* n) {
        *n = 0;
        if (!log_cap) return LIMO_OK;
        WinState s;
        HIP_TRY(ctx, hipMemcpyAsync(&s, bv.st + w, sizeof(WinState), hipMemcpyDeviceToHost, ctx->stream));
        HIP_TRY(ctx, hipStreamSynchronize(ctx->stream));
        const int have = std::max(0, std::min(s.log_n, log_cap)), m = std::min(have, cap);
        *n = have;
        if (m > 0) {
            HIP_TRY(ctx, hipMemcpyAsync(out, d_log + (size_t)w * log_cap, sizeof(limo_ba_iteration) * m, hipMemcpyDeviceToHost, ctx->stream));
            HIP_TRY(ctx, hipStreamSynchronize(ctx->stream));
        }
        return LIMO_OK;
    }
    int export_log() {
        ctx->last_log.clear();
        ctx->last_log_n.clear();
        ctx->last_log_off.clear();
        if (!log_cap) return LIMO_OK;
        std::vector<WinState> sv(P.n_win);
        HIP_TRY(ctx, hipMemcpyAsync(sv.data(), bv.st, sizeof(WinState) * sv.size(), hipMemcpyDeviceToHost, ctx->stream));
        HIP_TRY(ctx, hipStreamSynchronize(ctx->stream));
        size_t total = 0;
        for (int w = 0; w < P.n_win; ++w) {
            const int have = std::max(0, std::min(sv[w].log_n, log_cap));
            ctx->last_log_n.push_back(have);
            ctx->last_log_off.push_back(total);
            total += (size_t)have;
        }
        ctx->last_log.resize(total);
        for (int w = 0; w < P.n_win; ++w)
            if (ctx->last_log_n[w])
                HIP_TRY(ctx, hipMemcpyAsync(ctx->last_log.data() + ctx->last_log_off[w], d_log + (size_t)w * log_cap,
                                            sizeof(limo_ba_iteration) * ctx->last_log_n[w], hipMemcpyDeviceToHost, ctx->stream));
        HIP_TRY(ctx, hipStreamSynchronize(ctx->stream));
        return LIMO_OK;
    }
// ... 185 lines not shown
                    LAUNCH_CHECK("k_shard_reduce");
                }
            if (!first_lin) {
                assemble_pending = true;
                return;
            }
            first_lin = false;
            exchange(1);
        }
        assemble(it_no);
    }

    void assemble(int iter) {
        hipStream_t s = ctx->stream;
        const int slot = iter & 3;
        BatchView bvs = bv;
        bvs.n_active = bv.n_active + 2 * slot;
        bvs.n_active_host = d_h_active + slot;
        const WorkLists& a = wl[0].cur;
        launch_cam_assemble(bvs, a.win, a.n_win, s);
        LAUNCH_CHECK("k_cam_assemble");
        note(hipEventRecord(act_ev[slot], s), "record n_active");
    }

    int active_count() override {
        if (rc != LIMO_OK) return 0;
        const int cur = it_no++;
        if (cur == 0) return P.n_win;
        const int slot = (cur - 1) & 3;
        note(hipEventSynchronize(act_ev[slot]), "sync n_active");
        if (rc != LIMO_OK) return 0;
        const int a = h_active[slot], listed = wl[0].cur.n_win;
        static const bool trace = std::getenv("KBA_TRACE_ACTIVE") != nullptr;
        if (trace) std::fprintf(stderr, "[kba] iteration %d: active %d, listed %d, span %d\n", cur - 1, a, listed, c.schur_span);
        if (a > 0 && listed >= 8 && 2 * a <= listed) rebatch();
        return a;
    }

    void expire(int) override {
        if (assemble_pending) {
            assemble_pending = false;
            exchange(1);
            assemble(it_no - 1);
        }
        hipLaunchKernelGGL(k_expire, dim3(cdiv(P.n_win, 256)), dim3(256), 0, ctx->stream, bv);
        LAUNCH_CHECK("k_expire");
    }

    void launch_schur(const BatchView& v, const int32_t* wl_plain, int n_plain, const int32_t* wl_fgp, int n_fgp, const int32_t* wl_gen, int n_gen, bool pair,
                      hipStream_t s) {
        int span = c.schur_span, span_gp = c.schur_span_gp, packed = c.slab_packed;
        const bool narrow = plan.narrow && !gp_wide && packed && span == kSchurSpan && span_gp == kSchurSpanGp;
        const bool wide = !narrow || P.n_sgrp_wide > 0;
        if (pair) {
            void* args[] = {(void*)&v, (void*)&wl_plain, (void*)&n_plain, (void*)&wl_fgp, (void*)&span, (void*)&span_gp, (void*)&packed};
            note(hipLaunchKernel(narrow ? (const void*)k_schur_lean_pair<2, 3, true> : (const void*)k_schur_lean_pair<2, 3>, dim3(n_plain + n_fgp), dim3(64), args,
                                 std::max(plan.plain_lds, plan.leangp_lds), s),
                 "launch k_schur_lean_pair");
            ++n_pair_launches;
        }
        if (!pair && n_plain) {
            void* args[] = {(void*)&v, (void*)&wl_plain, (void*)&span, (void*)&span_gp, (void*)&packed};
            note(hipLaunchKernel(schur_fn_plain, dim3(n_plain), dim3(64), args, plan.plain_lds, s), "launch k_schur_lean");
        }
        if (!pair && n_fgp && narrow) {
            void* args[] = {(void*)&v, (void*)&wl_fgp};
            note(hipLaunchKernel(schur_fn_narrow, dim3(n_fgp), dim3(64), args, plan.leangp_lds, s), "launch k_schur_lean_gp");
        }
        if (!pair && n_fgp && !narrow) {
            void* args[] = {(void*)&v, (void*)&wl_fgp, (void*)&span, (void*)&span_gp, (void*)&packed};
            note(hipLaunchKernel(schur_fn_leangp, dim3(n_fgp), dim3(64), args, plan.leangp_lds, s), "launch k_schur_lean (gp)");
        }
        if (pair || n_fgp) {
            n_narrow_launches += narrow ? 1 : 0;
            n_widegp_launches += wide ? 1 : 0;
        }
        if (n_gen) {
            void* args[] = {(void*)&v, (void*)&wl_gen, (void*)&span, (void*)&span_gp};
            note(hipLaunchKernel(schur_fn_gen, dim3(n_gen), dim3(64 * kWideWaves), args, plan.wide_lds, s), "launch k_schur_wide");
        }
    }

    void launch_cam_assemble(const BatchView& v, const int32_t* list, int grid, hipStream_t s) {
        if (grid) hipLaunchKernelGGL(k_cam_assemble, dim3(grid), dim3(kBlock), plan.asm_bytes, s, v, c, list);
    }
    void launch_cam_solve(const BatchView& v, const int32_t* list, int grid, hipStream_t s) {
        if (grid) hipLaunchKernelGGL(k_cam_solve, dim3(grid), dim3(kBlock), plan.solve_bytes, s, v, c, list);
    }
    void launch_backsub(const BatchView& v, const int32_t* list, int grid, hipStream_t s) {
        if (grid) hipLaunchKernelGGL(k_backsub, dim3(grid), dim3(kBlock), 0, s, v, c, list);
    }
    void launch_step_decide(const BatchView& v, const int32_t* list, int grid, hipStream_t s) {
        if (grid) hipLaunchKernelGGL(k_step_decide, dim3(grid), dim3(64), 0, s, v, c, list);
    }
    void launch_after_step(const BatchView& v, const int32_t* list, int grid, hipStream_t s) {
        if (grid) hipLaunchKernelGGL(k_after_step, dim3(grid), dim3(kBlock), 0, s, v, c, list);
    }
    void launch_trim_residual(const BatchView& v, const int32_t* list, int grid, hipStream_t s) {
        if (grid) hipLaunchKernelGGL(k_trim_residual, dim3(grid), dim3(kBlock), 0, s, v, d_plane_rep, d_plane_dep, list);
    }
    void launch_trim_max(const BatchView& v, int shard, int grid, hipStream_t s) {
        if (grid) hipLaunchKernelGGL(k_trim_max, dim3(grid), dim3(kBlock), 0, s, v, (const double*)d_plane_rep, (const double*)d_plane_dep, shard, shard_P);
    }
    void launch_trim_select(const BatchView& v, int grid, hipStream_t s) {
        if (grid) hipLaunchKernelGGL(k_trim_select, dim3(grid), dim3(kBlock), plan.trim_bytes, s, v, c);
    }

    void step() override {
        hipStream_t s = ctx->stream;
        if (c.slab_packed) spart_has_packed = true;
        const WorkLists& a = wl[0].cur;
        {
            int n_schur = 0;
            for (size_t i = 0; i < pv.size(); ++i) n_schur += wl[i].cur.n_sblk;
            EventPair* ep = n_schur ? timed(LIMO_KERNEL_SCHUR) : nullptr;
            for (size_t i = 0; i < pv.size(); ++i) {
                const WorkLists& l = wl[i].cur;
                launch_schur(pv[i], l.sblk, l.n_sblk_plain, l.sblk + l.n_sblk_plain, l.n_sblk_fgp, l.sblk + l.n_sblk_plain + l.n_sblk_fgp,
                             l.n_sblk - l.n_sblk_plain - l.n_sblk_fgp, false, s);
                LAUNCH_CHECK("Schur kernels");
            }
            if (ep) note(hipEventRecord(ep->b, s), "hipEventRecord");
        }
        if (shard_P > 1) {
            if (a.n_win)
                for (size_t i = 0; i < pv.size(); ++i) {
                    hipLaunchKernelGGL(k_shard_reduce, dim3(a.n_win), dim3(kBlock), 0, s, pv[i], a.win, local_shards[i], 1);
                    hipLaunchKernelGGL(k_slab_reduce, dim3(a.n_win, 8), dim3(kBlock), 0, s, pv[i], a.win, shard_P);
                    LAUNCH_CHECK("k_slab_reduce");
                }
            if (assemble_pending) {
                assemble_pending = false;
                exchange(3);
                assemble(it_no - 1);
            } else {
                exchange(2);
            }
        }
        launch_cam_solve(bv, a.win, a.n_win, s);
        LAUNCH_CHECK("k_cam_solve");
        for (size_t i = 0; i < pv.size(); ++i) {
            launch_backsub(pv[i], wl[i].cur.lblk, wl[i].cur.n_lblk, s);
            LAUNCH_CHECK("k_backsub");
        }
        if (shard_P > 1 && a.n_win)
            for (size_t i = 0; i < pv.size(); ++i) {
                hipLaunchKernelGGL(k_shard_reduce, dim3(a.n_win), dim3(kBlock), 0, s, pv[i], a.win, local_shards[i], 2);
                LAUNCH_CHECK("k_shard_reduce");
            }
        exchange(4);
        launch_step_decide(bv, a.win, a.n_win, s);
        LAUNCH_CHECK("k_step_decide");
        for (size_t i = 0; i < pv.size(); ++i) {
            launch_after_step(pv[i], wl[i].cur.lblk, wl[i].cur.n_lblk, s);
            LAUNCH_CHECK("k_after_step");
        }
    }

    void trim() override {
        hipStream_t s = ctx->stream;
        bool any = false;
        for (const WinDesc& d : P.win) any = any || d.do_trim;
        if (!any) return;
        for (size_t i = 0; i < pv.size(); ++i) {
            launch_trim_residual(pv[i], wl[i].full.blk, wl[i].full.n_blk, s);
            LAUNCH_CHECK("k_trim_residual");
        }
        for (size_t i = 0; i < pv.size(); ++i) {
            launch_trim_max(pv[i], local_shards[i], cdiv(P.TL, kBlock), s);
            LAUNCH_CHECK("k_trim_max");
// ... 378 lines not shown
        ctx->err = "pack_windows: out of host memory";
        return LIMO_ERR_RUNTIME;
    } catch (const std::exception& e) {
        ctx->err = std::string("pack_windows: ") + e.what();
        return LIMO_ERR_RUNTIME;
    }
    if (lending) {
        ctx->pack_arena_wanted = std::max(ctx->pack_arena_wanted, lend.wanted);
        if (lend.used > 0) {
            ctx->pack_arena_busy = true;
            b->holds_pack_arena = true;
        } else if (!ctx->pack_arena.p && lend.wanted > 0) {
            arena_resize(lend.wanted);
        }
    }
    const auto t_c1 = std::chrono::steady_clock::now();
    if (rc == LIMO_OK) {
        if (hipSetDevice(ctx->device) != hipSuccess) rc = LIMO_ERR_NO_DEVICE;
    }
    b->pose_batch = po.per_window_prior;
    b->shard_P = b->P.n_shards;
    b->shard_virtual = !shards_are_ranks;
    b->shard_rank = shards_are_ranks ? ctx->comm_rank : 0;
    if (b->shard_P > 1) {
        const int world = shards_are_ranks ? ctx->comm_world : 1, me = shards_are_ranks ? ctx->comm_rank : 0;
        for (int r = 0; r < b->shard_P; ++r)
            if (r % world == me) b->local_shards.push_back(r);
        if (b->local_shards.size() > 8) {
            ctx->err = "at most 8 shards per GPU";
            return LIMO_ERR_INVALID;
        }
    } else {
        b->local_shards.push_back(0);
    }
    b->c = b->consts_for(o);
    if (rc == LIMO_OK) rc = b->upload();
    if (std::getenv("KBA_PACK_TRACE"))
        std::fprintf(stderr, "[kba] create: pack %.1f ms, upload %.1f ms\n", std::chrono::duration<double, std::milli>(t_c1 - t_c0).count(),
                     std::chrono::duration<double, std::milli>(std::chrono::steady_clock::now() - t_c1).count());
    if (rc != LIMO_OK) return rc;
    *out = b.release();
    return LIMO_OK;
}

int limo_ba_batch_create(limo_ctx* ctx, int32_t n_windows, const limo_ba_window* windows, limo_ba_batch** out) {
    return batch_create_impl(ctx, n_windows, windows, nullptr, PackOptions(), out);
}

int limo_ba_batch_solve(limo_ba_batch* b, const limo_ba_options* opts) {
    if (!b) return LIMO_ERR_INVALID;
    limo_ctx* ctx = b->ctx;
    if (hipSetDevice(ctx->device) != hipSuccess) return LIMO_ERR_NO_DEVICE;
    if (opts) {
        if (opts->min_landmarks_for_trimming != b->opts.min_landmarks_for_trimming) {
            for (int w = 0; w < b->P.n_win; ++w) b->P.win[w].do_trim = b->P.win[w].n_lm > opts->min_landmarks_for_trimming;
            if (b->shard_P > 1) {
                const std::vector<WinDesc> wc = exchange_consumer_windows(b->P);
                HIP_TRY(ctx, hipMemcpy((void*)b->d_win_orig, b->P.win.data(), sizeof(WinDesc) * b->P.n_win, hipMemcpyHostToDevice));
                HIP_TRY(ctx, hipMemcpy((void*)b->bv.win, wc.data(), sizeof(WinDesc) * b->P.n_win, hipMemcpyHostToDevice));
            } else {
                HIP_TRY(ctx, hipMemcpyAsync((void*)b->bv.win, b->P.win.data(), sizeof(WinDesc) * b->P.n_win, hipMemcpyHostToDevice,
                                            ctx->stream));
            }
        }
        b->opts = *opts;
        b->c = b->consts_for(*opts);
    }
    b->rc = LIMO_OK;
    if (b->bind_log(ctx->iteration_log && b->shard_P == 1) != LIMO_OK) return LIMO_ERR_RUNTIME;
    const auto t0 = std::chrono::steady_clock::now();
    HIP_TRY(ctx, hipEventRecord(b->ev_total_a, ctx->stream));
    const SolveSwitches sw = read_solve_switches();
    SolveFacts facts;
    facts.max_solver_time_sec = b->opts.max_solver_time_sec;
    facts.shard_P = b->shard_P;
    facts.pose_batch = b->pose_batch;
    facts.pristine = b->pristine;
    facts.coop_strikes = ctx->coop_strikes;
    facts.coop_benched = ctx->coop_benched;
    const SolveChoice ch = choose_solve_path(b->P, b->plan, sw, facts);
    if (ch.benched) ++ctx->coop_benched;
    b->n_rounds = b->n_pair_launches = b->n_narrow_launches = b->n_widegp_launches = 0;
    b->gp_wide = sw.gp_wide;
    b->lin_variant = 1;
    long long* info = ctx->last_solve_info;
    std::fill(info, info + 8, 0ll);
    auto launch_sequence = [&]() {
        info[0] = ch.fallback;
        if (ch.fallback == PATH_STREAMING)
            b->solve_streaming(sw);
        else
            run_schedule(*b, b->opts);
    };
    switch (ch.path) {
        case PATH_WG:
            info[0] = PATH_WG;
            b->solve_wg();
            break;
        case PATH_COOP:
            if (b->solve_coop(ch.coop, sw)) {
                info[0] = PATH_COOP;
                info[2] = ch.coop.G;
                ctx->coop_benched = 0;
                break;
            }
            [[fallthrough]];
        default:
            launch_sequence();
    }
    b->pristine = false;
    if (b->coop_launched) {
        b->coop_launched = false;
        HIP_TRY(ctx, hipStreamSynchronize(ctx->stream));
        if (b->h_active[8] == 0) ctx->coop_strikes = 0;
        if (b->h_active[8] != 0) {
            b->h_active[8] = 0;
            info[1] = 1;
            ++ctx->coop_fallbacks;
            ++ctx->coop_strikes;
            if (b->reset_state() != LIMO_OK) return LIMO_ERR_RUNTIME;
            b->rc = LIMO_OK;
            launch_sequence();
            b->pristine = false;
        }
    }
    if (b->shard_P > 1 && !b->shard_virtual) {
        hipLaunchKernelGGL(k_lm_owned, dim3(cdiv(b->P.TL, 256)), dim3(256), 0, ctx->stream, b->bv, b->d_lm_tmp, b->shard_rank, b->shard_P,
                           ctx->comm_world);
        if (ctx->xfn) {
            b->host_exchange(b->d_lm_tmp, b->bv.lm, (size_t)3 * b->P.TL, 1);
            if (b->rc != LIMO_OK) return b->rc;
        } else {
            const ncclResult_t r = ncclAllReduce(b->d_lm_tmp, b->bv.lm, (size_t)3 * b->P.TL, ncclDouble, ncclSum, (ncclComm_t)ctx->comm, ctx->stream);
            b->note_nccl(r, "ncclAllReduce(landmarks)");
            if (r != ncclSuccess) return b->rc;
        }
        ++b->n_exchanges;
        b->exchange_bytes += (int64_t)sizeof(double) * 3 * b->P.TL;
    }
    if (info[0] == PATH_STREAMING) {
        info[3] = (long long)b->groups.size();
        info[4] = b->n_slots;
    }
    info[5] = b->n_rounds;
    info[6] = b->n_pair_launches;
    info[7] = b->lin_variant;
    ctx->last_schur_gp_info[0] = b->P.n_sgrp_narrow;
    ctx->last_schur_gp_info[1] = b->P.n_sgrp_wide;
    ctx->last_schur_gp_info[2] = b->n_narrow_launches;
    ctx->last_schur_gp_info[3] = b->n_widegp_launches;
    HIP_TRY(ctx, hipEventRecord(b->ev_total_b, ctx->stream));
    HIP_TRY(ctx, hipStreamSynchronize(ctx->stream));
    float ms = 0.f;
    HIP_TRY(ctx, hipEventElapsedTime(&ms, b->ev_total_a, b->ev_total_b));
    b->total_ms_acc += ms;
    b->last_solve_sec = std::chrono::duration<double>(std::chrono::steady_clock::now() - t0).count();
    return b->rc;
}

int limo_ba_batch_reset(limo_ba_batch* b) {
    if (!b) return LIMO_ERR_INVALID;
    if (hipSetDevice(b->ctx->device) != hipSuccess) return LIMO_ERR_NO_DEVICE;
    return b->reset_state();
}

int limo_ba_batch_download(limo_ba_batch* b, limo_ba_window* windows_out, limo_ba_report* reports) {
    if (!b) return LIMO_ERR_INVALID;
    limo_ctx* ctx = b->ctx;
    const PackedBatch& P = b->P;
    std::vector<double> pose_v, pdir_v, pdist_v, lm_v;
    std::vector<WinState> st_v;
    const double *pose = nullptr, *pdir = nullptr, *pdist = nullptr, *lm = nullptr;
    const WinState* st = nullptr;
    {
        const char* lo = reinterpret_cast<const char*>(b->bv.st);
        const char* hi = reinterpret_cast<const char*>(b->bv.lm) + sizeof(double) * 3 * (size_t)P.TL;
        auto inside = [&](const void* q) { return reinterpret_cast<const char*>(q) >= lo && reinterpret_cast<const char*>(q) < hi; };
        const bool neighbours = hi > lo && inside(b->bv.pose) && inside(b->bv.pdir) && inside(b->bv.pdist) && (P.TL == 0 || inside(b->bv.lm));
        const size_t span = neighbours ? (size_t)(hi - lo) : 0;
        void* hbuf = nullptr;
        if (neighbours && span <= ctx->staging.cap && ctx->staging.p) {
            hbuf = ctx->staging.p;
        } else if (neighbours && span <= limo_ctx::kBigStageMax) {
            if (ctx->staging_big.ensure(span, span + span / 4, limo_ctx::kBigStageMax) == hipSuccess)
                hbuf = ctx->staging_big.p;
            else
                (void)hipGetLastError();
        }
        if (hbuf) {
            HIP_TRY(ctx, hipMemcpyAsync(hbuf, lo, span, hipMemcpyDeviceToHost, ctx->stream));
            HIP_TRY(ctx, hipStreamSynchronize(ctx->stream));
            const char* h = static_cast<const char*>(hbuf);
            auto at = [&](const void* q) { return h + (reinterpret_cast<const char*>(q) - lo); };
            st = reinterpret_cast<const WinState*>(at(b->bv.st));
            pose = reinterpret_cast<const double*>(at(b->bv.pose));
            pdir = reinterpret_cast<const double*>(at(b->bv.pdir));
            pdist = reinterpret_cast<const double*>(at(b->bv.pdist));
            lm = reinterpret_cast<const double*>(at(b->bv.lm));
        } else {
            pose_v.resize((size_t)P.TK * 7);
            pdir_v.resize((size_t)P.TK * 3);
            pdist_v.resize(P.TK);
            lm_v.resize((size_t)P.TL * 3);
            st_v.resize(P.n_win);
            HIP_TRY(ctx, hipMemcpyAsync(pose_v.data(), b->bv.pose, sizeof(double) * pose_v.size(), hipMemcpyDeviceToHost, ctx->stream));
            HIP_TRY(ctx, hipMemcpyAsync(pdir_v.data(), b->bv.pdir, sizeof(double) * pdir_v.size(), hipMemcpyDeviceToHost, ctx->stream));
            HIP_TRY(ctx, hipMemcpyAsync(pdist_v.data(), b->bv.pdist, sizeof(double) * pdist_v.size(), hipMemcpyDeviceToHost, ctx->stream));
            if (P.TL) HIP_TRY(ctx, hipMemcpyAsync(lm_v.data(), b->bv.lm, sizeof(double) * lm_v.size(), hipMemcpyDeviceToHost, ctx->stream));
            HIP_TRY(ctx, hipMemcpyAsync(st_v.data(), b->bv.st, sizeof(WinState) * st_v.size(), hipMemcpyDeviceToHost, ctx->stream));
            HIP_TRY(ctx, hipStreamSynchronize(ctx->stream));
            pose = pose_v.data();
            pdir = pdir_v.data();
            pdist = pdist_v.data();
            lm = lm_v.data();
            st = st_v.data();
        }
    }
    if (windows_out)
        for (int w = 0; w < P.n_win; ++w)
            if (windows_out[w].n_kf != P.win[w].n_kf || windows_out[w].n_lm != P.win[w].n_lm) {
                ctx->err = "download: window shape differs from create()";
                return LIMO_ERR_INVALID;
            }
    auto one_window = [&](int w) {
        const WinDesc& d = P.win[w];
        if (windows_out) {
            limo_ba_window& W = windows_out[w];
            std::memcpy(W.kf_pose, pose + 7 * (size_t)d.kf0, sizeof(double) * 7 * d.n_kf);
            std::memcpy(W.kf_plane_dir, pdir + 3 * (size_t)d.kf0, sizeof(double) * 3 * d.n_kf);
            std::memcpy(W.kf_plane_dist, pdist + d.kf0, sizeof(double) * d.n_kf);
            for (int l = 0; l < d.n_lm; ++l)
                std::memcpy(W.lm_pos + 3 * (size_t)P.lm_id[d.lm0 + l], lm + 3 * (size_t)(d.lm0 + l), sizeof(double) * 3);
        }
// ... 113 lines not shown
    ctx->comm_world = world;
    return LIMO_OK;
}

int limo_ctx_comm_init_host(limo_ctx* ctx, limo_exchange_fn fn, void* user, int rank, int world) {
    if (!ctx || (fn && (world < 1 || rank < 0 || rank >= world))) return LIMO_ERR_INVALID;
    if (ctx->comm) {
        (void)ncclCommDestroy((ncclComm_t)ctx->comm);
        ctx->comm = nullptr;
    }
    ctx->xfn = fn;
    ctx->xuser = user;
    ctx->comm_rank = fn ? rank : 0;
    ctx->comm_world = fn ? world : 1;
    return LIMO_OK;
}

int limo_ba_solve_sharded(limo_ctx* ctx, limo_ba_window* window, const limo_ba_options* opts, int n_shards,
                          limo_ba_report* report) {
    if (!ctx || !window) return LIMO_ERR_INVALID;
    const bool ranks = ctx->has_transport();
    if (n_shards < 1 || (ranks && n_shards % ctx->comm_world != 0) || n_shards > 8 * (ranks ? ctx->comm_world : 1)) {
        ctx->err = "limo_ba_solve_sharded: n_shards must be a multiple of the communicator size, at most 8 shards per GPU";
        return LIMO_ERR_INVALID;
    }
    PackOptions po;
    po.shards = n_shards;
    limo_ba_batch* b = nullptr;
    ctx->last_log.clear();
    ctx->last_log_n.clear();
    ctx->last_log_off.clear();
    int rc = batch_create_impl(ctx, 1, window, opts, po, &b, ranks);
    if (rc != LIMO_OK) return rc;
    rc = limo_ba_batch_solve(b, opts);
    limo_ba_report rep;
    if (rc == LIMO_OK) rc = limo_ba_batch_download(b, window, &rep);
    if (rc == LIMO_OK && report) *report = rep;
    ctx->exchange_stats[0] = b->n_exchanges;
    ctx->exchange_stats[1] = b->exchange_bytes;
    ctx->exchange_stats[2] = rc == LIMO_OK ? rep.iterations_total : 0;
    limo_ba_batch_destroy(b);
    return rc;
}

static int solve_n(limo_ctx* ctx, int32_t n, limo_ba_window* windows, const limo_ba_options* opts, const PackOptions& po, limo_ba_report* reports,
                   const char* what) {
    using Clock = std::chrono::steady_clock;
    static const bool trace = std::getenv("KBA_HOST_TRACE") != nullptr;
    const auto t_a = Clock::now();
    limo_ba_batch* b = nullptr;
    int rc = batch_create_impl(ctx, n, windows, opts, po, &b);
    if (rc != LIMO_OK) return rc;
    const auto t0 = Clock::now();
    rc = limo_ba_batch_solve(b, nullptr);
    const auto t1 = Clock::now();
    if (rc == LIMO_OK) rc = limo_ba_batch_download(b, windows, reports);
    {
        const int lrc = b->export_log();
        if (rc == LIMO_OK) rc = lrc;
    }
    const auto t2 = Clock::now();
    if (reports)
        for (int w = 0; w < n; ++w) reports[w].time_sec = std::chrono::duration<double>(t2 - t0).count();
    limo_ba_batch_destroy(b);
    if (trace) {
        auto us = [](Clock::time_point a, Clock::time_point c) { return std::chrono::duration<double, std::micro>(c - a).count(); };
        std::fprintf(stderr, "[kba] %s (%d windows): create %.0f us, solve %.0f us, download %.0f us, destroy %.0f us\n", what, (int)n, us(t_a, t0), us(t0, t1),
                     us(t1, t2), us(t2, Clock::now()));
    }
    return rc;
}

int64_t limo_ctx_coop_fallbacks(const limo_ctx* ctx) { return ctx ? (int64_t)ctx->coop_fallbacks : 0; }

int limo_ctx_exchange_stats(limo_ctx* ctx, int64_t* stats3) {
    if (!ctx || !stats3) return LIMO_ERR_INVALID;
    for (int i = 0; i < 3; ++i) stats3[i] = ctx->exchange_stats[i];
    return LIMO_OK;
}

int limo_ctx_last_solve_info(const limo_ctx* ctx, int64_t info[8]) {
    if (!ctx || !info) return LIMO_ERR_INVALID;
    for (int i = 0; i < 8; ++i) info[i] = ctx->last_solve_info[i];
    return LIMO_OK;
}

int limo_ctx_last_schur_gp_info(const limo_ctx* ctx, int64_t info[4]) {
    if (!ctx || !info) return LIMO_ERR_INVALID;
    for (int i = 0; i < 4; ++i) info[i] = ctx->last_schur_gp_info[i];
    return LIMO_OK;
}

int limo_ctx_set_iteration_log(limo_ctx* ctx, int32_t on) {
    if (!ctx) return LIMO_ERR_INVALID;
    ctx->iteration_log = on != 0;
    return LIMO_OK;
}

static const char* iteration_log_args(int32_t window, int32_t n_win, int32_t cap, const limo_ba_iteration* out, const int32_t* n) {
    if (!n) return "n is NULL";
    if (cap < 0) return "cap < 0";
    if (cap > 0 && !out) return "out is NULL with cap > 0";
    if (window < 0 || (n_win >= 0 && window >= n_win)) return "window out of range";
    return nullptr;
}

int limo_ba_batch_iteration_log(limo_ba_batch* b, int32_t window, int32_t cap, limo_ba_iteration* out, int32_t* n) {
    if (!b) return LIMO_ERR_INVALID;
    limo_ctx* ctx = b->ctx;
    if (const char* bad = iteration_log_args(window, b->P.n_win, cap, out, n)) {
        ctx->err = std::string("limo_ba_batch_iteration_log: ") + bad;
        return LIMO_ERR_INVALID;
    }
    if (hipSetDevice(ctx->device) != hipSuccess) return LIMO_ERR_NO_DEVICE;
    return b->read_log(window, cap, out, n);
}

int limo_ctx_last_iteration_log(limo_ctx* ctx, int32_t window, int32_t cap, limo_ba_iteration* out, int32_t* n) {
    if (!ctx) return LIMO_ERR_INVALID;
    const int32_t n_win = ctx->last_log_n.empty() ? -1 : (int32_t)ctx->last_log_n.size();
    if (const char* bad = iteration_log_args(window, n_win, cap, out, n)) {
        ctx->err = std::string("limo_ctx_last_iteration_log: ") + bad;
        return LIMO_ERR_INVALID;
    }
    *n = 0;
    if (n_win < 0) return LIMO_OK;
    *n = ctx->last_log_n[window];
    const int m = std::min(*n, cap);
    if (m > 0) std::memcpy(out, ctx->last_log.data() + ctx->last_log_off[window], sizeof(limo_ba_iteration) * m);
    return LIMO_OK;
}

int limo_ba_solve(limo_ctx* ctx, limo_ba_window* window, const limo_ba_options* opts, limo_ba_report* report) {
    if (!ctx || !window) return LIMO_ERR_INVALID;
    return solve_n(ctx, 1, window, opts, PackOptions(), report, "limo_ba_solve");
}

int limo_ba_solve_fixed_landmarks(limo_ctx* ctx, limo_ba_window* window, const uint8_t* lm_fixed, const limo_ba_options* opts,
                                  limo_ba_report* report) {
    if (!ctx || !window) return LIMO_ERR_INVALID;
    PackOptions po;
    po.lm_fixed = lm_fixed ? &lm_fixed : nullptr;
    return solve_n(ctx, 1, window, opts, po, report, "limo_ba_solve_fixed_landmarks");
}

int limo_ba_batch_create_fixed_landmarks(limo_ctx* ctx, int32_t n_windows, const limo_ba_window* windows, const uint8_t* const* lm_fixed,
                                         limo_ba_batch** out) {
    PackOptions po;
    po.lm_fixed = lm_fixed;
    return batch_create_impl(ctx, n_windows, windows, nullptr, po, out);
}

int limo_ba_adjust_pose_only(limo_ctx* ctx, limo_ba_window* window, const limo_speed_prior* prior,
                             const limo_ba_options* opts, limo_ba_report* report) {
    if (!ctx || !window) return LIMO_ERR_INVALID;
    PackOptions po;
    po.pose_only = true;
    po.prior = prior;
    return solve_n(ctx, 1, window, opts, po, report, "limo_ba_adjust_pose_only");
}

int limo_ba_batch_create_pose_only(limo_ctx* ctx, int32_t n_windows, const limo_ba_window* windows, const limo_speed_prior* priors,
                                   limo_ba_batch** out) {
    PackOptions po;
    po.pose_only = true;
    po.per_window_prior = true;
// ... 154 lines not shown
```

Before: 40390 windows/s.

## Add half-width 128-thread camera assemble/solve kernels selected by occupancy

```diff
diff --git a/include/limo_hip.h b/include/limo_hip.h
--- a/include/limo_hip.h
+++ b/include/limo_hip.h
@@ -126,6 +126,7 @@
 int64_t limo_ctx_coop_fallbacks(const limo_ctx* ctx);
 int limo_ctx_last_solve_info(const limo_ctx* ctx, int64_t info[8]);
 int limo_ctx_last_schur_gp_info(const limo_ctx* ctx, int64_t info[4]);
+int limo_ctx_last_cam_lanes_info(const limo_ctx* ctx, int64_t info[9]);
 
 typedef struct limo_ba_iteration {
     int32_t solve;
diff --git a/limo_amd/_ffi.py b/limo_amd/_ffi.py
--- a/limo_amd/_ffi.py
+++ b/limo_amd/_ffi.py
@@ -365,6 +365,7 @@
     "limo_ctx_coop_fallbacks",
     "limo_ctx_last_solve_info",
     "limo_ctx_last_schur_gp_info",
+    "limo_ctx_last_cam_lanes_info",
     "limo_ctx_set_iteration_log",
     "limo_ba_batch_iteration_log",
     "limo_ctx_last_iteration_log",
@@ -503,6 +504,8 @@
         lib.limo_ctx_last_solve_info.argtypes = [vp, c_int64_p]
     if hasattr(lib, "limo_ctx_last_schur_gp_info"):
         lib.limo_ctx_last_schur_gp_info.argtypes = [vp, c_int64_p]
+    if hasattr(lib, "limo_ctx_last_cam_lanes_info"):
+        lib.limo_ctx_last_cam_lanes_info.argtypes = [vp, c_int64_p]
     if hasattr(lib, "limo_ctx_set_iteration_log"):
         lib.limo_ctx_set_iteration_log.argtypes = [vp, C.c_int32]
         lib.limo_ba_batch_iteration_log.argtypes = [vp, C.c_int32, C.c_int32, C.POINTER(BaIteration), c_int32_p]
diff --git a/limo_amd/ba.py b/limo_amd/ba.py
--- a/limo_amd/ba.py
+++ b/limo_amd/ba.py
@@ -87,6 +87,13 @@
         v = (C.c_int64 * 4)()
         _check(self.lib.limo_ctx_last_schur_gp_info(self.ptr, v), self.ptr, "limo_ctx_last_schur_gp_info")
         return dict(zip(("narrow_groups", "wide_groups", "narrow_launches", "wide_launches"), (int(x) for x in v)))
+
+    def last_cam_lanes_info(self):
+        v = (C.c_int64 * 9)()
+        _check(self.lib.limo_ctx_last_cam_lanes_info(self.ptr, v), self.ptr, "limo_ctx_last_cam_lanes_info")
+        keys = ("assemble_128", "assemble_256", "solve_128", "solve_256", "wg_per_cu_assemble_128", "wg_per_cu_assemble_256",
+                "wg_per_cu_solve_128", "wg_per_cu_solve_256", "global_class_windows")
+        return dict(zip(keys, (int(x) for x in v)))
 
     def set_iteration_log(self, on):
         _check(self.lib.limo_ctx_set_iteration_log(self.ptr, int(bool(on))), self.ptr, "limo_ctx_set_iteration_log")
diff --git a/limo_amd/csrc/kba_batch_plan.hpp b/limo_amd/csrc/kba_batch_plan.hpp
--- a/limo_amd/csrc/kba_batch_plan.hpp
+++ b/limo_amd/csrc/kba_batch_plan.hpp
@@ -117,6 +117,7 @@
     double coop_timeout_ms = 50.0;
     bool groups_set = false;
     int groups = 0;
+    int cam_lanes = 0;
     bool gp_wide = false;
 };
 
@@ -138,8 +139,37 @@
         s.groups_set = true;
         s.groups = std::atoi(e);
     }
+    if (const char* e = std::getenv("KBA_CAM_LANES")) {
+        const int v = std::atoi(e);
+        s.cam_lanes = v == kCamLanesHalf || v == kBlock ? v : 0;
+    }
     s.gp_wide = on("KBA_SCHUR_GP_WIDE");
     return s;
+}
+
+struct CamOccupancy {
+    int n_cu = 0;
+    int asm_full = 0, asm_half = 0, solve_full = 0, solve_half = 0;
+};
+struct CamLanesPlan {
+    bool asm_half_ok = false, solve_half_ok = false;
+    int asm_resident = 0, solve_resident = 0;
+};
+inline CamLanesPlan plan_cam_lanes(const PackedBatch& P, const CamOccupancy& occ, bool plain) {
+    CamLanesPlan p;
+    p.asm_resident = occ.n_cu * occ.asm_full;
+    p.solve_resident = occ.n_cu * occ.solve_full;
+    bool ok = plain && P.n_win > 0;
+    for (const WinDesc& d : P.win) ok = ok && d.cam_scr_off < 0 && d.nc <= kCamLanesHalf;
+    p.asm_half_ok = ok && occ.asm_full > 0 && occ.asm_half >= 2 * occ.asm_full;
+    p.solve_half_ok = ok && occ.solve_full > 0 && occ.solve_half >= 2 * occ.solve_full;
+    return p;
+}
+constexpr int kCamLanesFactor = 1;
+inline int cam_lanes_for_launch(bool half_ok, int resident_full, int n_listed, int forced) {
+    if (!half_ok || forced == kBlock) return kBlock;
+    if (forced == kCamLanesHalf) return kCamLanesHalf;
+    return n_listed > kCamLanesFactor * resident_full ? kCamLanesHalf : kBlock;
 }
 
 enum SolvePath { PATH_NONE = 0, PATH_WG = 1, PATH_COOP = 2, PATH_STREAMING = 3, PATH_LOCKSTEP = 4 };
diff --git a/limo_amd/csrc/kba_items.hpp b/limo_amd/csrc/kba_items.hpp
--- a/limo_amd/csrc/kba_items.hpp
+++ b/limo_amd/csrc/kba_items.hpp
@@ -1044,42 +1044,49 @@
 }
 
 template <int N, int NSUM>
-KBA_HD void coop_reduce(double* v, int tid, int nt, double* red) {
+KBA_HD void coop_reduce(double* v, int tid, int nt, double* red, int vrep = 1) {
 #if defined(__HIP_DEVICE_COMPILE__)
     if (nt >= 64 && (nt & 63) == 0) {
         const int wave = tid >> 6, nw = nt >> 6;
-        for (int q = 0; q < N; ++q) {
-            double x = v[q];
-            for (int off = 32; off > 0; off >>= 1) {
-                const double o = __shfl_xor(x, off, 64);
-                x = q < NSUM ? x + o : fmax(x, o);
-            }
-            if ((tid & 63) == 0) red[wave * N + q] = x;
-        }
+        for (int u = 0; u < vrep; ++u)
+            for (int q = 0; q < N; ++q) {
+                double x = v[u * N + q];
+                for (int off = 32; off > 0; off >>= 1) {
+                    const double o = __shfl_xor(x, off, 64);
+                    x = q < NSUM ? x + o : fmax(x, o);
+                }
+                if ((tid & 63) == 0) red[(u * nw + wave) * N + q] = x;
+            }
         KBA_SYNC();
         for (int q = 0; q < N; ++q) {
             double x = red[q];
-            for (int u = 1; u < nw; ++u) x = q < NSUM ? x + red[u * N + q] : fmax(x, red[u * N + q]);
+            for (int u = 1; u < nw * vrep; ++u) x = q < NSUM ? x + red[u * N + q] : fmax(x, red[u * N + q]);
             v[q] = x;
         }
         KBA_SYNC();
         return;
     }
 #endif
-    for (int q = 0; q < N; ++q) red[q * nt + tid] = v[q];
+    const int nvl = nt * vrep;
+    for (int u = 0; u < vrep; ++u)
+        for (int q = 0; q < N; ++q) red[q * nvl + tid + u * nt] = v[u * N + q];
     KBA_SYNC();
-    for (int s = nt >> 1; s > 0; s >>= 1) {
-        if (tid < s) {
-            for (int q = 0; q < NSUM; ++q) red[q * nt + tid] += red[q * nt + tid + s];
-            for (int q = NSUM; q < N; ++q) red[q * nt + tid] = fmax(red[q * nt + tid], red[q * nt + tid + s]);
+    for (int s = nvl >> 1; s > 0; s >>= 1) {
+        for (int t = tid; t < s; t += nt) {
+            for (int q = 0; q < NSUM; ++q) red[q * nvl + t] += red[q * nvl + t + s];
+            for (int q = NSUM; q < N; ++q) red[q * nvl + t] = fmax(red[q * nvl + t], red[q * nvl + t + s]);
         }
         KBA_SYNC();
     }
-    for (int q = 0; q < N; ++q) v[q] = red[q * nt];
+    for (int q = 0; q < N; ++q) v[q] = red[q * nvl];
     KBA_SYNC();
 }
 
+#if defined(KBA_HOST_LANES)
+KBA_HD int coop_red_doubles(int n, int nt) { return n * nt; }
+#else
 KBA_HD int coop_red_doubles(int n, int nt) { return n * ((nt >= 64 && (nt & 63) == 0) ? nt >> 6 : nt); }
+#endif
 
 constexpr int kGpChunk = 128;
 constexpr int kRegDense = 2 + 2 * kCamSlots;
@@ -1119,12 +1126,19 @@
 constexpr int kCamLdsCapBytes = 150 * 1024;
 KBA_HD int cam_solve_scratch(int nc, int nt, int nf = -1) {
     if (nf < 0) nf = nc;
-    return nf * (nf + 1) + nf + nc + coop_red_doubles(3, nt) + nf * (nf + 1) / 2 + nf;
-}
-
-KBA_HD void cam_assemble(const BatchView& bv, const SolveConsts& c, int w, int tid, int nt, double* scratch) {
+    return nf * (nf + 1) + nf + nc + coop_red_doubles(3, nt) + 2 * nf;
+}
+KBA_HD int cam_class_doubles(int nc, int n_view) {
+    const int solve = cam_solve_scratch(nc, kBlock) - 2 * nc + nc * (nc + 1) / 2 + nc;
+    const int assemble = cam_assemble_scratch(nc, kBlock, n_view);
+    return assemble > solve ? assemble : solve;
+}
+
+KBA_HD void cam_assemble(const BatchView& bv, const SolveConsts& c, int w, int tid, int nt, double* scratch, int nvl = 0) {
     const WinDesc& wd = bv.win[w];
     const int nc = wd.nc, nbt = cam_bt_count(nc);
+    if (nvl <= 0) nvl = nt;
+    const int vrep = nvl / nt;
     double* H = scratch;
     double* gc = H + nbt;
     double* sc = gc + nc;
@@ -1234,10 +1248,10 @@
             KBA_SYNC();
         }
 #if defined(__HIP_DEVICE_COMPILE__)
-        if (nt == 256) {
+        if (nvl == 256) {
             typedef double v4d_t __attribute__((ext_vector_type(4)));
             const int lane = tid & 63, li = lane & 15, kq = lane >> 4;
-            for (int kl = tid >> 6; kl < wd.n_kf; kl += 4) {
+            for (int kl = tid >> 6; kl < wd.n_kf; kl += nt >> 6) {
                 int lo = bv.kf_gp0[wd.kf0 + kl] - g0, hi = lo + bv.kf_ngp[wd.kf0 + kl];
                 lo = lo < 0 ? 0 : lo;
                 hi = hi > ng ? ng : hi;
@@ -1280,10 +1294,10 @@
     KBA_TICK(2);
     const int nrows = reg_row_count(wd);
     const int reg_base = wd.has_scale_reg ? 1 : 0, reg_npair = wd.has_gp_reg ? wd.n_kf - 1 : 0;
-    for (int i0 = tid; i0 < (nt >= 256 ? nt : nrows); i0 += nt) {
+    for (int i0 = tid; i0 < (nvl >= 256 ? nvl : nrows); i0 += nt) {
         int i = i0;
-        if (nt >= 256) {
-            const int wv = tid >> 6, ln = tid & 63;
+        if (nvl >= 256) {
+            const int wv = i0 >> 6, ln = i0 & 63;
             i = -1;
             if (wv == 0) {
                 if (ln < reg_npair) i = reg_base + ln * 5 + 4;
@@ -1368,59 +1382,64 @@
         }
     }
     KBA_TICK(5);
-    double cost = 0.0, failf = 0.0, gmax = 0.0, xn2 = 0.0, reg_free = 0.0, reg_fixed = 0.0;
-    for (int i = tid; i < wd.n_lblk * wd.n_view; i += nt) cost += bv.lv_part[wd.lvpart_off + (int64_t)i * kLinPartial];
-    for (int b = wd.lblk0 + tid; b < wd.lblk0 + wd.n_lblk; b += nt)
-        if (bv.lblk_linfail[b] != 0.0) failf = 1.0;
-    if (wd.n_lm_const) {
-        for (int i = tid; i < wd.n_lblk * wd.n_view_fixed0; i += nt)
-            reg_fixed += bv.lv_part[wd.lvpart_off + ((int64_t)(i / wd.n_view_fixed0) * wd.n_view + i % wd.n_view_fixed0) * kLinPartial + kLinFixedCost];
-        for (int g = wd.gp0 + tid; g < wd.gp0 + wd.n_gp; g += nt) {
-            const double v = bv.gp_cost[g];
-            const bool fixed = gp_row_fixed(bv, g);
-            cost += fixed ? 0.0 : v;
-            reg_fixed += fixed ? v : 0.0;
-        }
-    } else {
-        for (int g = wd.gp0 + tid; g < wd.gp0 + wd.n_gp; g += nt) cost += bv.gp_cost[g];
-    }
-    for (int i = tid; i < nrows; i += nt) {
-        if (rows[i].n < 0)
-            reg_fixed += 0.5 * rows[i].r * rows[i].r;
-        else
-            reg_free += 0.5 * rows[i].r * rows[i].r;
-    }
-    for (int b = wd.lblk0 + tid; b < wd.lblk0 + wd.n_lblk; b += nt) {
-        gmax = fmax(gmax, bv.lblk_part[(int64_t)b * 8 + 0]);
-        xn2 += bv.lblk_part[(int64_t)b * 8 + 1];
-    }
-    for (int k = tid; k < wd.n_kf; k += nt) {
-        const int gk = wd.kf0 + k;
-        if (cm[k * kCamSlots + 0]) {
-            const double* x = bv.pose + 7 * (int64_t)gk;
-            gmax = fmax(gmax, block_grad_inf(0, x, gc + k * kCamSlots));
-            for (int i = 0; i < 7; ++i) xn2 += x[i] * x[i];
-        }
-        if (cm[k * kCamSlots + 6]) {
-            const double* x = bv.pdir + 3 * (int64_t)gk;
-            gmax = fmax(gmax, block_grad_inf(1, x, gc + k * kCamSlots + 6));
-            for (int i = 0; i < 3; ++i) xn2 += x[i] * x[i];
-        }
-        if (cm[k * kCamSlots + 9]) {
-            gmax = fmax(gmax, block_grad_inf(2, bv.pdist + gk, gc + k * kCamSlots + 9));
-            xn2 += bv.pdist[gk] * bv.pdist[gk];
-        }
-    }
-    {
-        double v[6] = {reg_free, reg_fixed, cost, xn2, failf, gmax};
-        coop_reduce<6, 4>(v, tid, nt, red);
-        reg_free = v[0];
-        reg_fixed = v[1];
-        cost = v[2] + reg_free;
-        xn2 = v[3];
-        failf = v[4];
-        gmax = v[5];
-    }
+    double v[2 * 6];
+#pragma unroll
+    for (int u = 0; u < 2; ++u) {
+        if (u >= vrep) break;
+        const int vt = tid + u * nt;
+        double cost = 0.0, failf = 0.0, gmax = 0.0, xn2 = 0.0, reg_free = 0.0, reg_fixed = 0.0;
+        for (int i = vt; i < wd.n_lblk * wd.n_view; i += nvl) cost += bv.lv_part[wd.lvpart_off + (int64_t)i * kLinPartial];
+        for (int b = wd.lblk0 + vt; b < wd.lblk0 + wd.n_lblk; b += nvl)
+            if (bv.lblk_linfail[b] != 0.0) failf = 1.0;
+        if (wd.n_lm_const) {
+            for (int i = vt; i < wd.n_lblk * wd.n_view_fixed0; i += nvl)
+                reg_fixed += bv.lv_part[wd.lvpart_off + ((int64_t)(i / wd.n_view_fixed0) * wd.n_view + i % wd.n_view_fixed0) * kLinPartial + kLinFixedCost];
+            for (int g = wd.gp0 + vt; g < wd.gp0 + wd.n_gp; g += nvl) {
+                const double gv = bv.gp_cost[g];
+                const bool fixed = gp_row_fixed(bv, g);
+                cost += fixed ? 0.0 : gv;
+                reg_fixed += fixed ? gv : 0.0;
+            }
+        } else {
+            for (int g = wd.gp0 + vt; g < wd.gp0 + wd.n_gp; g += nvl) cost += bv.gp_cost[g];
+        }
+        for (int i = vt; i < nrows; i += nvl) {
+            if (rows[i].n < 0)
+                reg_fixed += 0.5 * rows[i].r * rows[i].r;
+            else
+                reg_free += 0.5 * rows[i].r * rows[i].r;
+        }
+        for (int b = wd.lblk0 + vt; b < wd.lblk0 + wd.n_lblk; b += nvl) {
+            gmax = fmax(gmax, bv.lblk_part[(int64_t)b * 8 + 0]);
+            xn2 += bv.lblk_part[(int64_t)b * 8 + 1];
+        }
+        for (int k = vt; k < wd.n_kf; k += nvl) {
+            const int gk = wd.kf0 + k;
+            if (cm[k * kCamSlots + 0]) {
+                const double* x = bv.pose + 7 * (int64_t)gk;
+                gmax = fmax(gmax, block_grad_inf(0, x, gc + k * kCamSlots));
+                for (int i = 0; i < 7; ++i) xn2 += x[i] * x[i];
+            }
+            if (cm[k * kCamSlots + 6]) {
+                const double* x = bv.pdir + 3 * (int64_t)gk;
+                gmax = fmax(gmax, block_grad_inf(1, x, gc + k * kCamSlots + 6));
+                for (int i = 0; i < 3; ++i) xn2 += x[i] * x[i];
+            }
+            if (cm[k * kCamSlots + 9]) {
+                gmax = fmax(gmax, block_grad_inf(2, bv.pdist + gk, gc + k * kCamSlots + 9));
+                xn2 += bv.pdist[gk] * bv.pdist[gk];
+            }
+        }
+        double* vu = v + 6 * u;
+        vu[0] = reg_free;
+        vu[1] = reg_fixed;
+        vu[2] = cost;
+        vu[3] = xn2;
+        vu[4] = failf;
+        vu[5] = gmax;
+    }
+    coop_reduce<6, 4>(v, tid, nt, red, vrep);
+    const double reg_free = v[0], reg_fixed = v[1], cost = v[2] + reg_free, xn2 = v[3], failf = v[4], gmax = v[5];
     if (tid == 0) {
         WinRed& r = bv.red[w];
         r.lin_cost = cost;
@@ -1434,14 +1453,17 @@
     KBA_TICK(6);
 }
 
-KBA_HD void cam_solve(const BatchView& bv, const SolveConsts& c, int w, int tid, int nt, double* scratch, int* flag) {
+KBA_HD void cam_solve(const BatchView& bv, const SolveConsts& c, int w, int tid, int nt, double* scratch, int* flag, int nvl = 0) {
     const WinDesc& wd = bv.win[w];
     const int nc = wd.nc, nf = wd.nf, nfp = wd.nf_pad, lda = nf + 1;
+    if (nvl <= 0) nvl = nt;
+    const int vrep = nvl / nt;
     double* A = scratch;
     double* y = A + nf * lda;
     double* dl = y + nf;
     double* red = dl + nc;
-    double* Hs = red + coop_red_doubles(3, nt);
+    double* Hd = red + coop_red_doubles(3, nvl);
+    auto hs_at = [&](int ca, int cb) -> double& { return cb == ca ? Hd[ca] : cb == nf ? Hd[nf + ca] : A[cb * lda + ca]; };
     const double radius = bv.st[w].radius;
     const double* Hg = bv.Hcc + wd.hcc_off;
     const double* sc = bv.scale_c + wd.cam0;
@@ -1475,7 +1497,7 @@
             int ca, cb;
             schur_need_decode(i, nf, ca, cb);
             double s_e = Hg[i];
-            Hs[i] = s_e;
+            hs_at(ca, cb) = s_e;
             if (ca == cb) s_e += fmin(fmax(s_e, c.min_lm_diagonal), c.max_lm_diagonal) / radius;
             off[e] = (c.schur_packed || pk) ? i : (int)schur_need_offset(ca, cb, nf, nfq, nfp);
             if (pk) off_pl[e] = slab_packed_read(false, ca, cb, nf, nfq);
@@ -1513,9 +1535,9 @@
     const int tw = nt >= 16 ? 16 : 1, th = nt / tw, tx = tid % tw;
     const int ty = nt == 256 ? ((tid >> 4) & 3) * 4 + (tid >> 6) : tid / tw;
 #if defined(__HIP_DEVICE_COMPILE__)
-    if (nt == 256) {
+    if (nvl == 256) {
         typedef double v4d_t __attribute__((ext_vector_type(4)));
-        const int lane = tid & 63, wave = tid >> 6, li = lane & 15, kq = lane >> 4;
+        const int lane = tid & 63, wave = tid >> 6, n_wave = nt >> 6, li = lane & 15, kq = lane >> 4;
         double* invd = y;
         if (tid == 0) *flag = 0;
         KBA_SYNC();
@@ -1581,7 +1603,7 @@
                 int t = 0;
                 for (int ti = 0; ti < Ti; ++ti)
                     for (int tj = ti; tj < Tj; ++tj, ++t) {
-                        if ((t & 3) != wave) continue;
+                        if ((t & (n_wave - 1)) != wave) continue;
                         const int i_op = kbe + 16 * ti + li, j_op = kbe + 16 * tj + li;
                         const double wv = kin && i_op < nf ? -(A[kp * lda + i_op] * ivd) : 0.0;
                         const double pv = kin && j_op <= nf ? A[kp * lda + j_op] : 0.0;
@@ -1676,18 +1698,27 @@
         dl[a] = d;
     }
     KBA_SYNC();
-    double part = 0.0;
-    for (int i = tid; i < n_need; i += nt) {
+    double part = 0.0, part_o = 0.0;
+    for (int i = tid; i < n_need; i += nvl) {
         int ca, cb;
         schur_need_decode(i, nf, ca, cb);
         if (cb < nf)
-            part -= (ca == cb ? 0.5 : 1.0) * (Hs[i] * y[ca] * y[cb]);
+            part -= (ca == cb ? 0.5 : 1.0) * (hs_at(ca, cb) * y[ca] * y[cb]);
         else
-            part += Hs[i] * y[ca];
+            part += hs_at(ca, cb) * y[ca];
+    }
+    for (int i = tid + nt; vrep == 2 && i < n_need; i += nvl) {
+        int ca, cb;
+        schur_need_decode(i, nf, ca, cb);
+        if (cb < nf)
+            part_o -= (ca == cb ? 0.5 : 1.0) * (hs_at(ca, cb) * y[ca] * y[cb]);
+        else
+            part_o += hs_at(ca, cb) * y[ca];
     }
     KBA_TICK(14);
     const uint8_t* cm = bv.cmask + (int64_t)wd.cam0;
     double step2 = 0.0, cand2 = 0.0;
+    const double step2_o = 0.0, cand2_o = 0.0;
     for (int k = tid; k < wd.n_kf; k += nt) {
         const int gk = wd.kf0 + k;
         const double* d = dl + k * kCamSlots;
@@ -1753,8 +1784,8 @@
         }
     }
     KBA_TICK(12);
-    double v3[3] = {part, step2, cand2};
-    coop_reduce<3, 3>(v3, tid, nt, red);
+    double v3[2 * 3] = {part, step2, cand2, part_o, step2_o, cand2_o};
+    coop_reduce<3, 3>(v3, tid, nt, red, vrep);
     if (tid == 0) {
         WinRed& r = bv.red[w];
         r.chol_fail = 0;
diff --git a/limo_amd/csrc/kba_kernels.hip b/limo_amd/csrc/kba_kernels.hip
--- a/limo_amd/csrc/kba_kernels.hip
+++ b/limo_amd/csrc/kba_kernels.hip
@@ -1093,7 +1093,9 @@
     }
 }
 
-__global__ __launch_bounds__(kBlock) __attribute__((amdgpu_waves_per_eu(3, 3))) void k_cam_assemble(BatchView bv, SolveConsts c, const int32_t* wl) {
+template <int NT>
+__global__ __launch_bounds__(NT) __attribute__((amdgpu_waves_per_eu(3, 3))) void k_cam_assemble(BatchView bv, SolveConsts c, const int32_t* wl) {
+    const int nt = NT == kBlock ? (int)blockDim.x : NT, nvl = NT == kBlock ? 0 : kBlock;
     const int w = wl_at(bv, wl, blockIdx.x);
     if (w < 0) return;
     WinState& st = bv.st[w];
@@ -1101,9 +1103,9 @@
     if (st.active && st.need_lin) {
         const int64_t so = bv.win[w].cam_scr_off;
         if (so >= 0)
-            cam_assemble(bv, c, w, threadIdx.x, blockDim.x, bv.cam_scratch + so);
+            cam_assemble(bv, c, w, threadIdx.x, nt, bv.cam_scratch + so, nvl);
         else
-            cam_assemble(bv, c, w, threadIdx.x, blockDim.x, smem);
+            cam_assemble(bv, c, w, threadIdx.x, nt, smem, nvl);
         __syncthreads();
 #ifdef KBA_PROFILE_TICKS
         if (w == 0 && threadIdx.x == 0)
@@ -1129,7 +1131,9 @@
     }
 }
 
-__global__ __launch_bounds__(kBlock) void k_cam_solve(BatchView bv, SolveConsts c, const int32_t* wl) {
+template <int NT>
+__global__ __launch_bounds__(NT) void k_cam_solve(BatchView bv, SolveConsts c, const int32_t* wl) {
+    const int nt = NT == kBlock ? (int)blockDim.x : NT, nvl = NT == kBlock ? 0 : kBlock;
     const int w = wl_at(bv, wl, blockIdx.x);
     if (w < 0) return;
     if (!bv.st[w].active) return;
@@ -1137,9 +1141,9 @@
     __shared__ int flag;
     const int64_t so = bv.win[w].cam_scr_off;
     if (so >= 0)
-        cam_solve(bv, c, w, threadIdx.x, blockDim.x, bv.cam_scratch + so, &flag);
+        cam_solve(bv, c, w, threadIdx.x, nt, bv.cam_scratch + so, &flag, nvl);
     else
-        cam_solve(bv, c, w, threadIdx.x, blockDim.x, smem, &flag);
+        cam_solve(bv, c, w, threadIdx.x, nt, smem, &flag, nvl);
 #ifdef KBA_PROFILE_TICKS
     __syncthreads();
     if (w == 0 && threadIdx.x == 0)
diff --git a/limo_amd/csrc/kba_layout.hpp b/limo_amd/csrc/kba_layout.hpp
--- a/limo_amd/csrc/kba_layout.hpp
+++ b/limo_amd/csrc/kba_layout.hpp
@@ -12,6 +12,7 @@
 constexpr int kCamSlots = 10;
 constexpr int kMaxNc = kMaxKf * kCamSlots;
 constexpr int kBlock = 256;
+constexpr int kCamLanesHalf = kBlock / 2;
 constexpr int kObsPerLane = 4;
 constexpr int kObsBlock = kBlock * kObsPerLane;
 constexpr int kSchurLm = 16;
diff --git a/limo_amd/csrc/kba_pack.cpp b/limo_amd/csrc/kba_pack.cpp
--- a/limo_amd/csrc/kba_pack.cpp
+++ b/limo_amd/csrc/kba_pack.cpp
@@ -724,7 +724,7 @@
             d.lvpart_off = P.lvpart_total;
             P.lvpart_total += (int64_t)d.n_lblk * d.n_view * kLinPartial;
             {
-                const int need = std::max(cam_assemble_scratch(d.nc, kBlock, d.n_view), cam_solve_scratch(d.nc, kBlock));
+                const int need = cam_class_doubles(d.nc, d.n_view);
                 d.cam_scr_off = -1;
                 if (need * (int)sizeof(double) > kCamLdsCapBytes) {
                     d.cam_scr_off = P.camscr_total;
diff --git a/limo_amd/csrc/limo_ctx.hpp b/limo_amd/csrc/limo_ctx.hpp
--- a/limo_amd/csrc/limo_ctx.hpp
+++ b/limo_amd/csrc/limo_ctx.hpp
@@ -49,6 +49,7 @@
     int coop_benched = 0;
     long long last_solve_info[8] = {0, 0, 0, 0, 0, 0, 0, 0};
     long long last_schur_gp_info[4] = {0, 0, 0, 0};
+    long long last_cam_lanes_info[9] = {0, 0, 0, 0, 0, 0, 0, 0, 0};
     bool iteration_log = false;
     std::vector<limo_ba_iteration> last_log;
     std::vector<int32_t> last_log_n;
diff --git a/limo_amd/csrc/limo_hip.hip b/limo_amd/csrc/limo_hip.hip
--- a/limo_amd/csrc/limo_hip.hip
+++ b/limo_amd/csrc/limo_hip.hip
@@ -107,6 +107,10 @@
     int64_t n_rounds = 0, n_pair_launches = 0;
     int64_t n_narrow_launches = 0, n_widegp_launches = 0;
     int lin_variant = 1;
+    CamOccupancy cam_occ;
+    CamLanesPlan cam_plan;
+    int cam_lanes_forced = 0;
+    int64_t n_cam_launches[2][2] = {{0, 0}, {0, 0}};
 
     ~limo_ba_batch() override {
         if (holds_pack_arena) ctx->pack_arena_busy = false;
@@ -311,8 +315,18 @@
             schur_fn_gen = schur_kernel(2, plan.wide_npw, 0);
             HIP_TRY(ctx, hipFuncSetAttribute(schur_fn_gen, hipFuncAttributeMaxDynamicSharedMemorySize, plan.wide_lds));
         }
-        HIP_TRY(ctx, hipFuncSetAttribute((const void*)k_cam_assemble, hipFuncAttributeMaxDynamicSharedMemorySize, plan.asm_bytes));
-        HIP_TRY(ctx, hipFuncSetAttribute((const void*)k_cam_solve, hipFuncAttributeMaxDynamicSharedMemorySize, plan.solve_bytes));
+        HIP_TRY(ctx, hipFuncSetAttribute((const void*)k_cam_assemble<kBlock>, hipFuncAttributeMaxDynamicSharedMemorySize, plan.asm_bytes));
+        HIP_TRY(ctx, hipFuncSetAttribute((const void*)k_cam_solve<kBlock>, hipFuncAttributeMaxDynamicSharedMemorySize, plan.solve_bytes));
+        HIP_TRY(ctx, hipFuncSetAttribute((const void*)k_cam_assemble<kCamLanesHalf>, hipFuncAttributeMaxDynamicSharedMemorySize, plan.asm_bytes));
+        HIP_TRY(ctx, hipFuncSetAttribute((const void*)k_cam_solve<kCamLanesHalf>, hipFuncAttributeMaxDynamicSharedMemorySize, plan.solve_bytes));
+        {
+            HIP_TRY(ctx, hipDeviceGetAttribute(&cam_occ.n_cu, hipDeviceAttributeMultiprocessorCount, ctx->device));
+            HIP_TRY(ctx, hipOccupancyMaxActiveBlocksPerMultiprocessor(&cam_occ.asm_full, k_cam_assemble<kBlock>, kBlock, plan.asm_bytes));
+            HIP_TRY(ctx, hipOccupancyMaxActiveBlocksPerMultiprocessor(&cam_occ.asm_half, k_cam_assemble<kCamLanesHalf>, kCamLanesHalf, plan.asm_bytes));
+            HIP_TRY(ctx, hipOccupancyMaxActiveBlocksPerMultiprocessor(&cam_occ.solve_full, k_cam_solve<kBlock>, kBlock, plan.solve_bytes));
+            HIP_TRY(ctx, hipOccupancyMaxActiveBlocksPerMultiprocessor(&cam_occ.solve_half, k_cam_solve<kCamLanesHalf>, kCamLanesHalf, plan.solve_bytes));
+            cam_plan = plan_cam_lanes(P, cam_occ, shard_P == 1 && !pose_batch);
+        }
         HIP_TRY(ctx, hipFuncSetAttribute((const void*)k_trim_select, hipFuncAttributeMaxDynamicSharedMemorySize, plan.trim_bytes));
         for (auto& e : act_ev) HIP_TRY(ctx, hipEventCreateWithFlags(&e, hipEventDisableTiming));
         HIP_TRY(ctx, hipEventCreate(&ev_total_a));
@@ -664,10 +678,22 @@
     }
 
     void launch_cam_assemble(const BatchView& v, const int32_t* list, int grid, hipStream_t s) {
-        if (grid) hipLaunchKernelGGL(k_cam_assemble, dim3(grid), dim3(kBlock), plan.asm_bytes, s, v, c, list);
+        if (!grid) return;
+        const bool half = cam_lanes_for_launch(cam_plan.asm_half_ok, cam_plan.asm_resident, grid, cam_lanes_forced) == kCamLanesHalf;
+        if (half)
+            hipLaunchKernelGGL(k_cam_assemble<kCamLanesHalf>, dim3(grid), dim3(kCamLanesHalf), plan.asm_bytes, s, v, c, list);
+        else
+            hipLaunchKernelGGL(k_cam_assemble<kBlock>, dim3(grid), dim3(kBlock), plan.asm_bytes, s, v, c, list);
+        ++n_cam_launches[0][half ? 0 : 1];
     }
     void launch_cam_solve(const BatchView& v, const int32_t* list, int grid, hipStream_t s) {
-        if (grid) hipLaunchKernelGGL(k_cam_solve, dim3(grid), dim3(kBlock), plan.solve_bytes, s, v, c, list);
+        if (!grid) return;
+        const bool half = cam_lanes_for_launch(cam_plan.solve_half_ok, cam_plan.solve_resident, grid, cam_lanes_forced) == kCamLanesHalf;
+        if (half)
+            hipLaunchKernelGGL(k_cam_solve<kCamLanesHalf>, dim3(grid), dim3(kCamLanesHalf), plan.solve_bytes, s, v, c, list);
+        else
+            hipLaunchKernelGGL(k_cam_solve<kBlock>, dim3(grid), dim3(kBlock), plan.solve_bytes, s, v, c, list);
+        ++n_cam_launches[1][half ? 0 : 1];
     }
     void launch_backsub(const BatchView& v, const int32_t* list, int grid, hipStream_t s) {
         if (grid) hipLaunchKernelGGL(k_backsub, dim3(grid), dim3(kBlock), 0, s, v, c, list);
@@ -1212,6 +1238,8 @@
     if (ch.benched) ++ctx->coop_benched;
     b->n_rounds = b->n_pair_launches = b->n_narrow_launches = b->n_widegp_launches = 0;
     b->gp_wide = sw.gp_wide;
+    b->cam_lanes_forced = sw.cam_lanes;
+    b->n_cam_launches[0][0] = b->n_cam_launches[0][1] = b->n_cam_launches[1][0] = b->n_cam_launches[1][1] = 0;
     b->lin_variant = 1;
     long long* info = ctx->last_solve_info;
     std::fill(info, info + 8, 0ll);
@@ -1279,6 +1307,19 @@
     ctx->last_schur_gp_info[1] = b->P.n_sgrp_wide;
     ctx->last_schur_gp_info[2] = b->n_narrow_launches;
     ctx->last_schur_gp_info[3] = b->n_widegp_launches;
+    {
+        long long* ci = ctx->last_cam_lanes_info;
+        ci[0] = b->n_cam_launches[0][0];
+        ci[1] = b->n_cam_launches[0][1];
+        ci[2] = b->n_cam_launches[1][0];
+        ci[3] = b->n_cam_launches[1][1];
+        ci[4] = b->cam_occ.asm_half;
+        ci[5] = b->cam_occ.asm_full;
+        ci[6] = b->cam_occ.solve_half;
+        ci[7] = b->cam_occ.solve_full;
+        ci[8] = 0;
+        for (const WinDesc& d : b->P.win) ci[8] += d.cam_scr_off >= 0 ? 1 : 0;
+    }
     HIP_TRY(ctx, hipEventRecord(b->ev_total_b, ctx->stream));
     HIP_TRY(ctx, hipStreamSynchronize(ctx->stream));
     float ms = 0.f;
@@ -1558,6 +1599,12 @@
 int limo_ctx_last_solve_info(const limo_ctx* ctx, int64_t info[8]) {
     if (!ctx || !info) return LIMO_ERR_INVALID;
     for (int i = 0; i < 8; ++i) info[i] = ctx->last_solve_info[i];
+    return LIMO_OK;
+}
+
+int limo_ctx_last_cam_lanes_info(const limo_ctx* ctx, int64_t info[9]) {
+    if (!ctx || !info) return LIMO_ERR_INVALID;
+    for (int i = 0; i < 9; ++i) info[i] = ctx->last_cam_lanes_info[i];
     return LIMO_OK;
 }
 
```

After: 42050 windows/s, median of 6. 1.04x the previous value.
